# jjery2243542/semi-supervised-ASR

Measured on AMD Instinct MI355X. Metric: utterances/sec (train step), higher is better.
Workload: dtype f32 (fp32-equivalent bf16x6 products)

## Files before the change

include/asr_hip.h:

```cpp
#ifndef ASR_HIP_H
#define ASR_HIP_H

#include <stdint.h>

#ifdef __cplusplus
extern "C" {
#endif

#define ASR_ABI_VERSION 6

#define ASR_E_ARG    (-1)
#define ASR_E_SHAPE  (-2)
#define ASR_E_ALIGN  (-3)

typedef void* asr_stream_t;

int asr_abi_version(void);

#define ASR_ARITH_F32        0
#define ASR_ARITH_BF16X6     1
#define ASR_ARITH_BF16X3     2
#define ASR_ARITH_MASK       0xff
#define ASR_GEMM_TILE_NARROW 0x100
#define ASR_GEMM_TILE_WIDE   0x200
#define ASR_GEMM_TILE_SP     0x800
#define ASR_GEMM_TILE_SMALL  0x1000
#define ASR_GEMM_C_ZEROED    0x2000
#define ASR_LSTM_BWD_GATHER  0x400
#define ASR_DEBUG_FAULT      0x10000

void* asr_graphs_create(int max_entries);
void asr_graphs_destroy(void* graphs);
int asr_graphs_stats(void* graphs, int64_t* hits, int64_t* captures, int64_t* eager);

int asr_gemm_f32(int transA, int transB, int64_t M, int64_t N, int64_t K,
                 const float* A, int64_t lda, const float* B, int64_t ldb,
                 float* C, int64_t ldc, const float* bias, int relu, int accumulate,
                 int batch, int64_t sA, int64_t sB, int64_t sC, int split_k, int arith,
                 asr_stream_t stream);
int asr_gemm_drop_f32(int transA, int transB, int64_t M, int64_t N, int64_t K, const float* A, int64_t lda,
                      const float* B, int64_t ldb, float* C, int64_t ldc, const float* bias, int relu, int split_k,
                      int arith, uint64_t seed, float p, asr_stream_t stream);

int asr_gemm_side_f32(int transA, int transB, int64_t M, int64_t N, int64_t K, const float* A, int64_t lda,
                      const float* B, int64_t ldb, float* C, int64_t ldc, int batch, int64_t sA, int64_t sB, int64_t sC,
                      int arith, unsigned xcd_mask, unsigned* queue, asr_stream_t stream);

int asr_gemm_skinny_f32(int64_t M, int64_t N, int64_t K,
                        const float* A, int64_t lda, const float* Bt, int64_t ldb,
                        float* C, int64_t ldc, const float* bias, int accumulate,
                        const float* mask, int64_t ldmask, int64_t mask_from,
                        asr_stream_t stream);

int asr_colsum_f32(int64_t M, int64_t N, const float* X, int64_t ldx, float* out,
                   int accumulate, asr_stream_t stream);

int asr_lstm_seq_fwd(int T, int B, int nb, int H, int ndir, float* gates, const float* w_hh,
                     const int32_t* lens, const int32_t* rowbase, const int32_t* rowext, float* y, float* c,
                     void* graphs, asr_stream_t stream);

int asr_persist_scratch_bytes(int64_t* xch_bytes, int64_t* ctrl_bytes);
int asr_lstm_seq_fwd_persist(int T, int B, int nb, int H, int ndir, float* gates, const float* w_hh,
                             const int32_t* lens, const int32_t* rowbase, const int32_t* rowext,
                             const int32_t* lens_host, float* y, float* c, void* xch, void* ctrl, int arith,
                             asr_stream_t stream);

int asr_lstm_seq_bwd(int T, int B, int nb, int H, int ndir, float* gates, const float* w_hhT,
                     const int32_t* lens, const int32_t* rowbase, const int32_t* rowext, const float* dy, const float* c,
                     float* dcarry, void* graphs, asr_stream_t stream);
int asr_lstm_seq_bwd_persist(int T, int B, int nb, int H, int ndir, float* gates, const float* w_hhT,
                             const int32_t* lens, const int32_t* rowbase, const int32_t* rowext,
                             const int32_t* lens_host, const float* dy, const float* c, const float* y,
                             float* dw_hh, float* db, void* xch, void* ctrl, int arith, asr_stream_t stream);
int asr_lstm_bwd_persist_fuses_dw(int H, int arith);
int asr_lstm_seq_bwd_persist_w(int T, int B, int nb, int H, int ndir, float* gates, const float* w_hh_il,
                               const int32_t* lens, const int32_t* rowbase, const int32_t* rowext,
                               const int32_t* lens_host, const float* dy, const float* c, const float* y, float* dw_hh,
                               float* db, void* xch, void* ctrl, int arith, asr_stream_t stream);

int asr_rows_pack_f32(int B, int T, int C, const float* x, const int32_t* lens, const int32_t* rowbase,
                      const int32_t* rowext, int ext_max, float* rows, asr_stream_t stream);
int asr_rows_unpack_fwd_f32(int B, int T, int C, const float* rows, const int32_t* lens, const int32_t* rowbase,
                            const float* fill, int fill_relu, const float* mask, uint64_t seed, float p, float* out,
                            asr_stream_t stream);
int asr_rows_unpack_bwd_f32(int B, int T, int C, const float* dout, const int32_t* lens, const int32_t* rowbase,
                            const int32_t* rowext, int ext_max, const float* mask, uint64_t seed, float p, float* drows,
                            float* dfill, const float* relu_of, asr_stream_t stream);

int asr_pyramid_concat_fwd(int T, int B, int C, const float* in, const float* mask,
                           float* out, asr_stream_t stream);
int asr_pyramid_concat_bwd(int T, int B, int C, const float* dout, const float* mask,
                           float* din, asr_stream_t stream);

int asr_dropout_seeded_f32(int64_t n, float* x, uint64_t seed, float p, asr_stream_t stream);
int asr_relu_dropout_bwd_f32(int64_t n, const float* grad, const float* y, uint64_t seed, float p, float* out,
                             asr_stream_t stream);
int asr_dropout_mask_f32(int64_t n, float* mask, uint64_t seed, float p, asr_stream_t stream);
int asr_pyramid_concat_fwd_seeded(int T, int B, int C, const float* in, uint64_t seed, float p, float* out,
                                  asr_stream_t stream);
int asr_pyramid_concat_bwd_seeded(int T, int B, int C, const float* dout, uint64_t seed, float p, float* din,
                                  asr_stream_t stream);

typedef struct {
  int B, nb, Tp, A, D, O, E, C, K;
  int L;
  float scaling;
  const float* P;
  const float* Q;
  const float* bo;
  const float* wcat;
  const float* bcat;
  const float* wdec;
  const float* convw;
  const float* watt;
  const float* wattT;
  const float* gvec;
  const float* w0;
  const float* xmask;
  float* X;
  float* Xd;
  float* gates;
  float* cstate;
  float* Dproj;
  float* fconv;
  float* S;
  float* energy;
  float* ws;
} asr_dec_fwd_t;

int asr_dec_step_fwd(const asr_dec_fwd_t* p, int s, asr_stream_t stream);
int asr_att_step_fwd(const asr_dec_fwd_t* p, int s, asr_stream_t stream);
int asr_dec_seq_fwd(const asr_dec_fwd_t* p, int s_begin, int s_end, void* graphs, asr_stream_t stream);
int asr_dec_seq_fwd_persist(const asr_dec_fwd_t* p, void* xch, void* ctrl, asr_stream_t stream);
int asr_dec_seq_fwd_persist_fault(const asr_dec_fwd_t* p, void* xch, void* ctrl, asr_stream_t stream);
typedef struct {
  int mode;
  int V;
  int eos;
  float scaling;
  const float* w_out;
  const float* b_out;
  const float* emb;
  float* logits;
  float* probs;
  int64_t* pred;
  int64_t* fed;
  const int64_t* tokens;
  int64_t ld_tokens;
  const unsigned char* teacher;
} asr_dec_feedback_t;
int asr_dec_seq_fwd_persist_free(const asr_dec_fwd_t* p, const asr_dec_feedback_t* f, void* xch, void* ctrl,
                                 asr_stream_t stream);

typedef struct {
  asr_dec_fwd_t f;
  const float* wcatT;
  const float* wdecT;
  const float* dws;
  float* G;
  float* dwext;
  float* dwraw;
  float* dfpart;
  float* dP;
  float* dgates;
  float* dD;
  float* dcell;
  float* dgvec_part;
  float* dwatt_part;
  float* dconv_part;
} asr_dec_bwd_t;

int asr_dec_step_bwd(const asr_dec_bwd_t* p, int s, asr_stream_t stream);
int asr_dec_seq_bwd(const asr_dec_bwd_t* p, int s_begin, int s_end, void* graphs, asr_stream_t stream);
int asr_dec_seq_bwd_persist(const asr_dec_bwd_t* p, float* mbuf, void* xch, void* ctrl, asr_stream_t stream);

typedef struct {
  int V;
  float scaling;
  const float* w_out;
  const float* emb;
  const float* probs;
  float* dlfb;
} asr_dec_feedback_bwd_t;
int asr_dec_seq_bwd_persist_free(const asr_dec_bwd_t* p, const asr_dec_feedback_bwd_t* fb, float* mbuf, void* xch,
                                 void* ctrl, asr_stream_t stream);

#define ASR_PACK_MAX_LAYERS 4
typedef struct {
  int H, I, ndir;
  const float* w_ih[2];
  const float* w_hh[2];
  const float* b_ih[2];
  const float* b_hh[2];
  float* w_ih_cat;
  float* w_hh_il;
  float* bias;
} asr_lstm_pack_job_t;
typedef struct {
  int H, I, ndir;
// ... 117 lines not shown
```

semi-supervised-asr_amd/csrc/gemm.hip:

```cpp
#include <cstdlib>
#include <type_traits>
#include "common.h"

#ifndef ASR_GEMM_BF3_TOUCH
#define ASR_GEMM_BF3_TOUCH 2
#endif
#ifndef ASR_GB_ABL
#define ASR_GB_ABL 0
#endif
#ifndef ASR_GLDS_CLOBBER_M0
#define ASR_GLDS_CLOBBER_M0 0
#endif
#ifndef ASR_GEMM_SETPRIO
#define ASR_GEMM_SETPRIO 1
#endif
namespace {

constexpr int BM = 128, BN = 128, BK = 32;
#ifndef ASR_GEMM_SMALL_OCC
#define ASR_GEMM_SMALL_OCC 1
#endif
#ifndef ASR_GEMM_TOUCH
#define ASR_GEMM_TOUCH 2
#endif

struct MatView {
  const float* p;
  int64_t ld, R, Cn;
  bool vec;
};

__device__ __forceinline__ float4 load4_guard(const MatView& m, int64_t r, int64_t c) {
  float4 v = make_float4(0.f, 0.f, 0.f, 0.f);
  if (r >= m.R) return v;
  const float* q = m.p + r * m.ld + c;
  if (m.vec && c + 3 < m.Cn) return *reinterpret_cast<const float4*>(q);
  if (c < m.Cn) v.x = q[0];
  if (c + 1 < m.Cn) v.y = q[1];
  if (c + 2 < m.Cn) v.z = q[2];
  if (c + 3 < m.Cn) v.w = q[3];
  return v;
}

template <bool KC>
struct TileCfg {
  static constexpr int S = KC ? 129 : 128;
};

template <bool KC>
__device__ __forceinline__ void tile_fetch(const MatView& m, int64_t row0, int64_t k0, float4 (&v)[4]) {
  const int t = threadIdx.x;
#pragma unroll
  for (int i = 0; i < 4; ++i) {
    const int f = t + 256 * i;
    if (KC) {
      const int row = f >> 3, kc4 = f & 7;
      v[i] = load4_guard(m, row0 + row, k0 + 4 * kc4);
    } else {
      const int k = f >> 5, m4 = f & 31;
      v[i] = load4_guard(m, k0 + k, row0 + 4 * m4);
    }
  }
}

template <bool KC>
__device__ __forceinline__ void tile_store(float* lds, const float4 (&v)[4]) {
  constexpr int S = TileCfg<KC>::S;
  const int t = threadIdx.x;
#pragma unroll
  for (int i = 0; i < 4; ++i) {
    const int f = t + 256 * i;
    if (KC) {
      const int row = f >> 3, kc4 = f & 7;
      float* d = lds + (4 * kc4) * S + row;
      d[0] = v[i].x; d[S] = v[i].y; d[2 * S] = v[i].z; d[3 * S] = v[i].w;
    } else {
      const int k = f >> 5, m4 = f & 31;
      *reinterpret_cast<float4*>(lds + k * S + 4 * m4) = v[i];
    }
  }
}

struct GemmArgs {
  MatView A, B;
  float* C;
  int64_t ldc, M, N, K;
  const float* bias;
  int relu, accumulate, split_k;
  int64_t sA, sB, sC;
  int tiles_m, tiles_n;
  unsigned* queue;
  unsigned xcd_mask;
};


#ifndef ASR_GEMM_GM
#define ASR_GEMM_GM 4
#endif
__device__ __forceinline__ void tile_coords(int tid, int tiles_m, int tiles_n, int gm_, int& tm, int& tn) {
  const int per = gm_ * tiles_n;
  const int grp = tid / per, in = tid - grp * per;
  const int first = grp * gm_;
  const int rows = tiles_m - first < gm_ ? tiles_m - first : gm_;
  tm = first + in % rows;
  tn = in / rows;
}

template <bool AKC, bool BKC>
__global__ __launch_bounds__(256) void gemm_f32_kernel(GemmArgs g) {
  constexpr int SA = TileCfg<AKC>::S, SB = TileCfg<BKC>::S;
  __shared__ __attribute__((aligned(16))) float smem[BK * SA + BK * SB];
  float* As = smem;
  float* Bs = smem + BK * SA;

  const int ntile = g.tiles_m * g.tiles_n;
  int tid = blockIdx.x;
  {
    const int q = ntile >> 3, rmd = ntile & 7, xcd = tid & 7, idx = tid >> 3;
    tid = (xcd < rmd ? xcd * (q + 1) : rmd * (q + 1) + (xcd - rmd) * q) + idx;
  }
  const int tm = tid / g.tiles_n, tn = tid % g.tiles_n;
  const int z = blockIdx.y;
  const int bz = z / g.split_k, kz = z % g.split_k;

  MatView A = g.A, B = g.B;
  A.p += bz * g.sA;
  B.p += bz * g.sB;
  float* C = g.C + bz * g.sC;

  const int64_t m0 = (int64_t)tm * BM, n0 = (int64_t)tn * BN;
  const int64_t ktiles = (g.K + BK - 1) / BK;
  const int64_t per = (ktiles + g.split_k - 1) / g.split_k;
  const int64_t kt_begin = kz * per;
  const int64_t kt_end = kt_begin + per < ktiles ? kt_begin + per : ktiles;

  const int lane = threadIdx.x & 63, wave = threadIdx.x >> 6;
  const int wm = wave >> 1, wn = wave & 1;
  const int l31 = lane & 31, kh = lane >> 5;

  f32x16 acc[2][2];
#pragma unroll
  for (int i = 0; i < 2; ++i)
#pragma unroll
    for (int j = 0; j < 2; ++j)
#pragma unroll
      for (int e = 0; e < 16; ++e) acc[i][j][e] = 0.f;

  const bool fast_a = A.vec && (AKC ? (m0 + BM <= A.R) : (m0 + BM <= A.Cn)) && A.R * A.ld < (int64_t)1 << 30;
  const bool fast_b = B.vec && (BKC ? (n0 + BN <= B.R) : (n0 + BN <= B.Cn)) && B.R * B.ld < (int64_t)1 << 30;
  const bool fast = fast_a && fast_b;
  unsigned offa[4], offb[4];
#pragma unroll
  for (int i = 0; i < 4; ++i) {
    const int f = threadIdx.x + 256 * i;
    offa[i] = AKC ? (unsigned)((f >> 3) * A.ld + 4 * (f & 7)) : (unsigned)((f >> 5) * A.ld + 4 * (f & 31));
    offb[i] = BKC ? (unsigned)((f >> 3) * B.ld + 4 * (f & 7)) : (unsigned)((f >> 5) * B.ld + 4 * (f & 31));
  }
  const float* basea = AKC ? A.p + m0 * A.ld : A.p + m0;
  const float* baseb = BKC ? B.p + n0 * B.ld : B.p + n0;
  float4 ra[4], rb[4];
  auto fetch = [&](int64_t kt2) {
    const int64_t k0 = kt2 * BK;
    if (fast && k0 + BK <= g.K) {
      const float* pa = basea + (AKC ? k0 : k0 * A.ld);
      const float* pb = baseb + (BKC ? k0 : k0 * B.ld);
#pragma unroll
      for (int i = 0; i < 4; ++i) ra[i] = *reinterpret_cast<const float4*>(pa + offa[i]);
#pragma unroll
      for (int i = 0; i < 4; ++i) rb[i] = *reinterpret_cast<const float4*>(pb + offb[i]);
    } else {
      tile_fetch<AKC>(A, m0, k0, ra);
      tile_fetch<BKC>(B, n0, k0, rb);
    }
  };
  if (kt_begin < kt_end) fetch(kt_begin);
  const int tt = threadIdx.x & 127;
  const bool touch_a = threadIdx.x < 128;
  float touched = 0.f;
  const bool do_touch = kt_end - kt_begin > 16;
  auto touch_tile = [&](int64_t ktt) {
    const MatView& m = touch_a ? A : B;
    const bool kc = touch_a ? AKC : BKC;
    const int64_t r0t = touch_a ? m0 : n0;
    int64_t rr, cc;
    if (kc) { rr = r0t + tt; cc = ktt * BK; }
    else { rr = ktt * BK + (tt >> 2); cc = r0t + 32 * (tt & 3); }
    rr = rr < m.R ? rr : m.R - 1;
    cc = cc < m.Cn ? cc : m.Cn - 1;
    touched = m.p[rr * m.ld + cc];
  };
  for (int64_t kt = kt_begin; kt < kt_end; ++kt) {
    tile_store<AKC>(As, ra);
    tile_store<BKC>(Bs, rb);
    __syncthreads();
    if (kt + 1 < kt_end) fetch(kt + 1);
#if ASR_GEMM_TOUCH
    asm volatile("" ::"v"(touched));
    if (do_touch && kt + ASR_GEMM_TOUCH < kt_end) touch_tile(kt + ASR_GEMM_TOUCH);
#endif
    const float* ap = As + kh * SA + wm * 64 + l31;
    const float* bp = Bs + kh * SB + wn * 64 + l31;
    if (ASR_GEMM_SETPRIO && !AKC) __builtin_amdgcn_s_setprio(1);
#pragma unroll
    for (int kk = 0; kk < BK / 2; ++kk) {
      const float a0 = ap[(2 * kk) * SA], a1 = ap[(2 * kk) * SA + 32];
      const float b0 = bp[(2 * kk) * SB], b1 = bp[(2 * kk) * SB + 32];
      acc[0][0] = __builtin_amdgcn_mfma_f32_32x32x2f32(a0, b0, acc[0][0], 0, 0, 0);
      acc[0][1] = __builtin_amdgcn_mfma_f32_32x32x2f32(a0, b1, acc[0][1], 0, 0, 0);
      acc[1][0] = __builtin_amdgcn_mfma_f32_32x32x2f32(a1, b0, acc[1][0], 0, 0, 0);
      acc[1][1] = __builtin_amdgcn_mfma_f32_32x32x2f32(a1, b1, acc[1][1], 0, 0, 0);
    }
    if (ASR_GEMM_SETPRIO && !AKC) __builtin_amdgcn_s_setprio(0);
    __syncthreads();
  }

  if (m0 + BM <= g.M && n0 + BN <= g.N) {
    const unsigned ldc = (unsigned)g.ldc;
    const bool split = g.split_k > 1, accum = g.accumulate != 0, relu = g.relu != 0;
#pragma unroll
    for (int j = 0; j < 2; ++j) {
      const int64_t n = n0 + wn * 64 + j * 32 + l31;
      const float bv = g.bias ? g.bias[n] : 0.f;
#pragma unroll
      for (int i = 0; i < 2; ++i) {
        float* base = C + (m0 + wm * 64 + i * 32 + 4 * kh) * g.ldc + n;
        if (split) {
#pragma unroll
          for (int e = 0; e < 16; ++e) atomicAdd(base + (unsigned)((e & 3) + 8 * (e >> 2)) * ldc, acc[i][j][e]);
        } else if (accum) {
          float old[16];
#pragma unroll
          for (int e = 0; e < 16; ++e) old[e] = base[(unsigned)((e & 3) + 8 * (e >> 2)) * ldc];
#pragma unroll
          for (int e = 0; e < 16; ++e) {
            float v = acc[i][j][e] + bv + old[e];
            if (relu) v = fmaxf(v, 0.f);
            base[(unsigned)((e & 3) + 8 * (e >> 2)) * ldc] = v;
          }
        } else {
#pragma unroll
          for (int e = 0; e < 16; ++e) {
            float v = acc[i][j][e] + bv;
            if (relu) v = fmaxf(v, 0.f);
            base[(unsigned)((e & 3) + 8 * (e >> 2)) * ldc] = v;
          }
        }
      }
    }
    return;
  }
#pragma unroll
  for (int j = 0; j < 2; ++j) {
    const int64_t n = n0 + wn * 64 + j * 32 + l31;
    if (n >= g.N) continue;
    const float bv = g.bias ? g.bias[n] : 0.f;
#pragma unroll
    for (int i = 0; i < 2; ++i) {
#pragma unroll
      for (int e = 0; e < 16; ++e) {
        const int64_t m = m0 + wm * 64 + i * 32 + (e & 3) + 8 * (e >> 2) + 4 * kh;
        if (m >= g.M) continue;
        float v = acc[i][j][e];
        float* dst = C + m * g.ldc + n;
        if (g.split_k > 1) {
          atomicAdd(dst, v);
        } else {
          v += bv;
          if (g.accumulate) v += *dst;
          if (g.relu) v = fmaxf(v, 0.f);
          *dst = v;
        }
      }
    }
  }
}

typedef __bf16 gbf16x8 __attribute__((ext_vector_type(8)));
typedef __bf16 gbf16x2 __attribute__((ext_vector_type(2)));
typedef unsigned gu32x4 __attribute__((ext_vector_type(4)));
constexpr int BS = 40;

__device__ __forceinline__ unsigned bf3g_hi2(float a, float b) {
  return __builtin_amdgcn_perm(__float_as_uint(b), __float_as_uint(a), 0x07060302u);
}
__device__ __forceinline__ unsigned bf3g_lo2(float a, float b) {
  const float la = a - __uint_as_float(__float_as_uint(a) & 0xffff0000u);
  const float lb = b - __uint_as_float(__float_as_uint(b) & 0xffff0000u);
  const gbf16x2 p = {(__bf16)la, (__bf16)lb};
  return __builtin_bit_cast(unsigned, p);
}

template <int NT>
__device__ __forceinline__ void bfn_split2(float x, float y, unsigned (&t)[NT]) {
  if constexpr (NT == 2) {
    t[0] = bf3g_hi2(x, y);
    t[1] = bf3g_lo2(x, y);
  } else {
    const gbf16x2 pa = {(__bf16)x, (__bf16)y};
    const unsigned ua = __builtin_bit_cast(unsigned, pa);
    const float rx = x - __uint_as_float(ua << 16), ry = y - __uint_as_float(ua & 0xffff0000u);
    const gbf16x2 pb = {(__bf16)rx, (__bf16)ry};
    const unsigned ub = __builtin_bit_cast(unsigned, pb);
    const float sx = rx - __uint_as_float(ub << 16), sy = ry - __uint_as_float(ub & 0xffff0000u);
    t[0] = ua;
    t[1] = ub;
    t[2] = bf3g_hi2(sx, sy);
  }
}

template <bool KC, int TS>
__device__ __forceinline__ void tile_fetch_bf3(const MatView& m, int64_t row0, int64_t k0, float4 (&v)[TS / 32]) {
  const int t = threadIdx.x;
#pragma unroll
  for (int i = 0; i < TS / 32; ++i) {
    if (KC) {
      const int f = t + 256 * i;
      v[i] = load4_guard(m, row0 + (f >> 3), k0 + 4 * (f & 7));
    } else if (TS == 128) {
      v[i] = load4_guard(m, k0 + 4 * (t & 7) + i, row0 + 4 * (t >> 3));
    } else {
      v[i] = load4_guard(m, k0 + 4 * (t & 7) + 2 * (t >> 7) + i, row0 + 4 * ((t >> 3) & 15));
    }
  }
}

template <bool KC, int NT, int TS>
__device__ __forceinline__ void tile_store_bf3(unsigned short* img, const float4 (&v)[TS / 32]) {
  const int t = threadIdx.x;
  if (KC) {
#pragma unroll
    for (int i = 0; i < TS / 32; ++i) {
      const int f = t + 256 * i;
      const int o = (f >> 3) * BS + 4 * (f & 7);
      unsigned p0[NT], p1[NT];
      bfn_split2<NT>(v[i].x, v[i].y, p0);
      bfn_split2<NT>(v[i].z, v[i].w, p1);
#pragma unroll
      for (int k = 0; k < NT; ++k) *reinterpret_cast<uint2*>(img + k * TS * BS + o) = make_uint2(p0[k], p1[k]);
    }
  } else if constexpr (TS == 64) {
    const int o = 4 * ((t >> 3) & 15) * BS + 4 * (t & 7) + 2 * (t >> 7);
    const float r[4][2] = {{v[0].x, v[1].x}, {v[0].y, v[1].y}, {v[0].z, v[1].z}, {v[0].w, v[1].w}};
#pragma unroll
    for (int j = 0; j < 4; ++j) {
      unsigned p0[NT];
      bfn_split2<NT>(r[j][0], r[j][1], p0);
#pragma unroll
      for (int k = 0; k < NT; ++k) *reinterpret_cast<unsigned*>(img + k * TS * BS + o + j * BS) = p0[k];
    }
  } else {
    const int o = 4 * (t >> 3) * BS + 4 * (t & 7);
    const float r[4][4] = {{v[0].x, v[1].x, v[2].x, v[3].x}, {v[0].y, v[1].y, v[2].y, v[3].y},
                           {v[0].z, v[1].z, v[2].z, v[3].z}, {v[0].w, v[1].w, v[2].w, v[3].w}};
#pragma unroll
    for (int j = 0; j < 4; ++j) {
      unsigned p0[NT], p1[NT];
      bfn_split2<NT>(r[j][0], r[j][1], p0);
      bfn_split2<NT>(r[j][2], r[j][3], p1);
#pragma unroll
      for (int k = 0; k < NT; ++k) *reinterpret_cast<uint2*>(img + k * TS * BS + o + j * BS) = make_uint2(p0[k], p1[k]);
    }
  }
}

template <bool AKC, bool BKC, int NT, int TS = 128, bool QUEUE = false>
__global__ __launch_bounds__(256, QUEUE ? 4 : (TS == 64 ? ASR_GEMM_SMALL_OCC : 1)) void gemm_bf3_kernel(GemmArgs g) {
  static_assert(!QUEUE || TS == 64, "the queue instantiation is the 64 x 64 tile");
  constexpr int BM = TS, BN = TS, NP = TS / 32, NB = TS / 64;
  __shared__ __attribute__((aligned(16))) unsigned short smem[2 * NT * BM * BS];
  unsigned short* Ai = smem;
  unsigned short* Bi = smem + NT * BM * BS;

  const int ntile = g.tiles_m * g.tiles_n;
  int tid = blockIdx.x;
  int z = blockIdx.y;
  if constexpr (QUEUE) {
    const unsigned xcc = __builtin_amdgcn_s_getreg(20 | (0 << 6) | (3 << 11)) & 7u;
    if (!((g.xcd_mask >> xcc) & 1u)) return;
    __shared__ unsigned ticket;
    if (threadIdx.x == 0) ticket = atomicAdd(g.queue, 1u);
    __syncthreads();
    const unsigned tk = ticket;
    if (tk >= (unsigned)ntile * gridDim.y) return;
    tid = (int)(tk % (unsigned)ntile);
    z = (int)(tk / (unsigned)ntile);
  } else {
    const int q = ntile >> 3, rmd = ntile & 7, xcd = tid & 7, idx = tid >> 3;
    tid = (xcd < rmd ? xcd * (q + 1) : rmd * (q + 1) + (xcd - rmd) * q) + idx;
  }
  const int tm = tid / g.tiles_n, tn = tid % g.tiles_n;
  const int bz = z / g.split_k, kz = z % g.split_k;

  MatView A = g.A, B = g.B;
  A.p += bz * g.sA;
  B.p += bz * g.sB;
  float* C = g.C + bz * g.sC;

  const int64_t m0 = (int64_t)tm * BM, n0 = (int64_t)tn * BN;
  const int64_t ktiles = (g.K + BK - 1) / BK;
  const int64_t per = (ktiles + g.split_k - 1) / g.split_k;
  const int64_t kt_begin = kz * per;
  const int64_t kt_end = kt_begin + per < ktiles ? kt_begin + per : ktiles;

  const int lane = threadIdx.x & 63, wave = threadIdx.x >> 6;
  const int wm = wave >> 1, wn = wave & 1;
  const int l31 = lane & 31, kh = lane >> 5;

  f32x16 acc[NB][NB];
#pragma unroll
  for (int i = 0; i < NB; ++i)
#pragma unroll
    for (int j = 0; j < NB; ++j)
#pragma unroll
      for (int e = 0; e < 16; ++e) acc[i][j][e] = 0.f;

  const bool fast_a = A.vec && (AKC ? (m0 + BM <= A.R) : (m0 + BM <= A.Cn)) && A.R * A.ld < (int64_t)1 << 30;
  const bool fast_b = B.vec && (BKC ? (n0 + BN <= B.R) : (n0 + BN <= B.Cn)) && B.R * B.ld < (int64_t)1 << 30;
  const bool fast = fast_a && fast_b;
  unsigned offa[NP], offb[NP];
#pragma unroll
  for (int i = 0; i < NP; ++i) {
    const int f = threadIdx.x + 256 * i;
    const int t = threadIdx.x;
    const int krow = TS == 128 ? 4 * (t & 7) + i : 4 * (t & 7) + 2 * (t >> 7) + i, rq = TS == 128 ? (t >> 3) : ((t >> 3) & 15);
    offa[i] = AKC ? (unsigned)((f >> 3) * A.ld + 4 * (f & 7)) : (unsigned)(krow * A.ld + 4 * rq);
    offb[i] = BKC ? (unsigned)((f >> 3) * B.ld + 4 * (f & 7)) : (unsigned)(krow * B.ld + 4 * rq);
  }
  const float* basea = AKC ? A.p + m0 * A.ld : A.p + m0;
  const float* baseb = BKC ? B.p + n0 * B.ld : B.p + n0;
  float4 ra[NP], rb[NP];
  auto fetch_fast = [&](int64_t kt2) {
    const int64_t k0 = kt2 * BK;
    const float* pa = basea + (AKC ? k0 : k0 * A.ld);
    const float* pb = baseb + (BKC ? k0 : k0 * B.ld);
#pragma unroll
    for (int i = 0; i < NP; ++i) ra[i] = *reinterpret_cast<const float4*>(pa + offa[i]);
#pragma unroll
    for (int i = 0; i < NP; ++i) rb[i] = *reinterpret_cast<const float4*>(pb + offb[i]);
  };
  auto fetch_guard = [&](int64_t kt2) {
    const int64_t k0 = kt2 * BK;
    tile_fetch_bf3<AKC, TS>(A, m0, k0, ra);
    tile_fetch_bf3<BKC, TS>(B, n0, k0, rb);
  };
  const int tt = threadIdx.x & 127;
  const bool touch_a = threadIdx.x < 128;
  float touched = 0.f;
  const bool do_touch = TS == 128 && kt_end - kt_begin > 2 * ASR_GEMM_BF3_TOUCH;
  auto touch_tile = [&](int64_t ktt) {
    const MatView& m = touch_a ? A : B;
    const bool kc = touch_a ? AKC : BKC;
    const int64_t r0t = touch_a ? m0 : n0;
    int64_t rr, cc;
    if (kc) { rr = r0t + tt; cc = ktt * BK; }
    else { rr = ktt * BK + (tt >> 2); cc = r0t + 32 * (tt & 3); }
    rr = rr < m.R ? rr : m.R - 1;
    cc = cc < m.Cn ? cc : m.Cn - 1;
    touched = m.p[rr * m.ld + cc];
  };
  const int ao = (wm * (TS / 2) + l31) * BS + 8 * kh, bo = (wn * (TS / 2) + l31) * BS + 8 * kh;
  auto multiply = [&]() {
#pragma unroll
    for (int ks = 0; ks < ((ASR_GB_ABL & 1) ? 0 : BK / 16); ++ks) {
      gu32x4 af[NB][NT], bf[NB][NT];
#pragma unroll
      for (int i = 0; i < NB; ++i)
#pragma unroll
        for (int k = 0; k < NT; ++k) {
          af[i][k] = *reinterpret_cast<const gu32x4*>(Ai + k * BM * BS + ao + 32 * i * BS + 16 * ks);
          bf[i][k] = *reinterpret_cast<const gu32x4*>(Bi + k * BM * BS + bo + 32 * i * BS + 16 * ks);
        }
#define BF3G(a_, b_, c_) c_ = __builtin_amdgcn_mfma_f32_32x32x16_bf16(__builtin_bit_cast(gbf16x8, a_), __builtin_bit_cast(gbf16x8, b_), c_, 0, 0, 0)
#pragma unroll
      for (int o = 0; o < NT; ++o)
#pragma unroll
        for (int p = 0; p <= o; ++p)
#pragma unroll
          for (int i = 0; i < NB; ++i)
#pragma unroll
            for (int j = 0; j < NB; ++j) BF3G(af[i][p], bf[j][o - p], acc[i][j]);
#undef BF3G
    }
  };
  const int64_t kt_full = g.K / BK < kt_end ? g.K / BK : kt_end;
  const int64_t kt_fast_end = (fast && kt_full > kt_begin) ? kt_full : kt_begin;
  if constexpr (TS == 64) {
    constexpr int PD = QUEUE ? 1 : 3;
    float4 qa[PD][NP], qb[PD][NP];
    auto fetch_set = [&](int64_t kt2, float4 (&xa)[NP], float4 (&xb)[NP]) __attribute__((always_inline)) {
      const int64_t k0 = kt2 * BK;
      const float* pa = basea + (AKC ? k0 : k0 * A.ld);
      const float* pb = baseb + (BKC ? k0 : k0 * B.ld);
#pragma unroll
      for (int i = 0; i < NP; ++i) xa[i] = *reinterpret_cast<const float4*>(pa + offa[i]);
#pragma unroll
      for (int i = 0; i < NP; ++i) xb[i] = *reinterpret_cast<const float4*>(pb + offb[i]);
    };
    int64_t kt = kt_begin;
    if (kt < kt_fast_end) {
#pragma unroll
      for (int d = 0; d < PD; ++d)
        if (kt + d < kt_fast_end) fetch_set(kt + d, qa[d], qb[d]);
      for (; kt + 2 * PD <= kt_fast_end; kt += PD) {
#pragma unroll
        for (int d = 0; d < PD; ++d) {
          __builtin_amdgcn_sched_barrier(0);
          tile_store_bf3<AKC, NT, TS>(Ai, qa[d]);
          tile_store_bf3<BKC, NT, TS>(Bi, qb[d]);
          __syncthreads();
          fetch_set(kt + d + PD, qa[d], qb[d]);
          multiply();
          __syncthreads();
          __builtin_amdgcn_sched_barrier(0);
        }
      }
#pragma unroll
      for (int d = 0; d < 2 * PD - 1; ++d) {
        if (kt + d < kt_fast_end) {
          tile_store_bf3<AKC, NT, TS>(Ai, qa[d % PD]);
          tile_store_bf3<BKC, NT, TS>(Bi, qb[d % PD]);
          __syncthreads();
          if (kt + d + PD < kt_fast_end) fetch_set(kt + d + PD, qa[d % PD], qb[d % PD]);
          multiply();
          __syncthreads();
        }
      }
    }
  } else if (kt_begin < kt_fast_end) {
    fetch_fast(kt_begin);
    for (int64_t kt = kt_begin; kt < kt_fast_end; ++kt) {
#if ASR_GB_ABL & 4
      if (kt == kt_begin) {
        tile_store_bf3<AKC, NT, TS>(Ai, ra);
        tile_store_bf3<BKC, NT, TS>(Bi, rb);
      } else {
#pragma unroll
        for (int i = 0; i < NP; ++i) asm volatile("" ::"v"(ra[i].x), "v"(ra[i].y), "v"(ra[i].z), "v"(ra[i].w), "v"(rb[i].x), "v"(rb[i].y), "v"(rb[i].z), "v"(rb[i].w));
      }
#else
      tile_store_bf3<AKC, NT, TS>(Ai, ra);
      tile_store_bf3<BKC, NT, TS>(Bi, rb);
#endif
      __syncthreads();
      if (kt + 1 < kt_fast_end && !(ASR_GB_ABL & 2)) fetch_fast(kt + 1);
#if ASR_GEMM_TOUCH
      asm volatile("" ::"v"(touched));
      if (do_touch && kt + ASR_GEMM_BF3_TOUCH < kt_end) touch_tile(kt + ASR_GEMM_BF3_TOUCH);
#endif
      multiply();
      __syncthreads();
    }
  }
  if (kt_fast_end < kt_end) {
    fetch_guard(kt_fast_end);
    for (int64_t kt = kt_fast_end; kt < kt_end; ++kt) {
      tile_store_bf3<AKC, NT, TS>(Ai, ra);
      tile_store_bf3<BKC, NT, TS>(Bi, rb);
      __syncthreads();
      if (kt + 1 < kt_end) fetch_guard(kt + 1);
#if ASR_GEMM_TOUCH
      asm volatile("" ::"v"(touched));
      if (do_touch && kt + ASR_GEMM_BF3_TOUCH < kt_end) touch_tile(kt + ASR_GEMM_BF3_TOUCH);
#endif
      multiply();
      __syncthreads();
    }
  }

#if ASR_GB_ABL & 8
  if (threadIdx.x + blockIdx.x + blockIdx.y != 0 || g.M != 1) {
#pragma unroll
    for (int i = 0; i < NB; ++i)
#pragma unroll
      for (int j = 0; j < NB; ++j)
#pragma unroll
        for (int e = 0; e < 16; ++e) asm volatile("" ::"v"(acc[i][j][e]));
    return;
  }
#endif
  if (m0 + BM <= g.M && n0 + BN <= g.N) {
    const unsigned ldc = (unsigned)g.ldc;
    const bool split = QUEUE || g.split_k > 1, accum = g.accumulate != 0, relu = g.relu != 0;
#pragma unroll
    for (int j = 0; j < NB; ++j) {
      const int64_t n = n0 + wn * (TS / 2) + j * 32 + l31;
      const float bv = g.bias ? g.bias[n] : 0.f;
#pragma unroll
      for (int i = 0; i < NB; ++i) {
        float* base = C + (m0 + wm * (TS / 2) + i * 32 + 4 * kh) * g.ldc + n;
        if (split) {
#pragma unroll
          for (int e = 0; e < 16; ++e) atomicAdd(base + (unsigned)((e & 3) + 8 * (e >> 2)) * ldc, acc[i][j][e]);
        } else if (accum) {
          float old[16];
#pragma unroll
          for (int e = 0; e < 16; ++e) old[e] = base[(unsigned)((e & 3) + 8 * (e >> 2)) * ldc];
#pragma unroll
          for (int e = 0; e < 16; ++e) {
            float v = acc[i][j][e] + bv + old[e];
            if (relu) v = fmaxf(v, 0.f);
            base[(unsigned)((e & 3) + 8 * (e >> 2)) * ldc] = v;
          }
        } else {
#pragma unroll
          for (int e = 0; e < 16; ++e) {
            float v = acc[i][j][e] + bv;
            if (relu) v = fmaxf(v, 0.f);
            base[(unsigned)((e & 3) + 8 * (e >> 2)) * ldc] = v;
          }
        }
      }
    }
    return;
  }
#pragma unroll
  for (int j = 0; j < NB; ++j) {
    const int64_t n = n0 + wn * (TS / 2) + j * 32 + l31;
    if (n >= g.N) continue;
    const float bv = g.bias ? g.bias[n] : 0.f;
#pragma unroll
    for (int i = 0; i < NB; ++i) {
#pragma unroll
      for (int e = 0; e < 16; ++e) {
        const int64_t m = m0 + wm * (TS / 2) + i * 32 + (e & 3) + 8 * (e >> 2) + 4 * kh;
        if (m >= g.M) continue;
        float v = acc[i][j][e];
        float* dst = C + m * g.ldc + n;
        if (QUEUE || g.split_k > 1) {
          atomicAdd(dst, v);
        } else {
          v += bv;
          if (g.accumulate) v += *dst;
          if (g.relu) v = fmaxf(v, 0.f);
          *dst = v;
        }
      }
    }
  }
}

constexpr int WM = 256, WN = 128, WK = 32;
constexpr int W_A_FLOATS = WM * WK, W_B_FLOATS = WN * WK, W_STAGE_FLOATS = W_A_FLOATS + W_B_FLOATS, W_STAGES = 3;
typedef __attribute__((address_space(3))) void* lds_vptr;

__device__ __forceinline__ void glds16(const float* src, float* lds_dst) {
  const unsigned dst = (unsigned)(uintptr_t)(lds_vptr)lds_dst;
#if ASR_GLDS_CLOBBER_M0
  asm volatile("s_mov_b32 m0, %1\n\ts_nop 0\n\tglobal_load_lds_dwordx4 %0, off" ::"v"(src), "s"(dst) : "memory", "m0");
#else
  unsigned keep;
  asm volatile("s_mov_b32 %0, m0\n\ts_mov_b32 m0, %2\n\ts_nop 0\n\tglobal_load_lds_dwordx4 %1, off\n\ts_mov_b32 m0, %0"
               : "=&s"(keep) : "v"(src), "s"(dst) : "memory");
#endif
}

#ifndef ASR_GW_ABL
#define ASR_GW_ABL 0
#endif
__device__ __forceinline__ void bf3w_split(const float (&v)[8], gu32x4& hi, gu32x4& lo) {
#if ASR_GW_ABL & 2
#pragma unroll
  for (int p = 0; p < 4; ++p) { hi[p] = __float_as_uint(v[p]); lo[p] = __float_as_uint(v[4 + p]); }
  return;
#endif
#pragma unroll
  for (int p = 0; p < 4; ++p) {
    hi[p] = bf3g_hi2(v[2 * p], v[2 * p + 1]);
    lo[p] = bf3g_lo2(v[2 * p], v[2 * p + 1]);
  }
}

template <bool KC, int ROWS>
__device__ __forceinline__ void bf3w_frag(const float* st, int row, int kq0s, int kq1s, int k0, gu32x4& hi, gu32x4& lo) {
  float v[8];
  if (KC) {
    const float4 x = *reinterpret_cast<const float4*>(st + row * WK + kq0s);
    const float4 y = *reinterpret_cast<const float4*>(st + row * WK + kq1s);
    v[0] = x.x; v[1] = x.y; v[2] = x.z; v[3] = x.w; v[4] = y.x; v[5] = y.y; v[6] = y.z; v[7] = y.w;
  } else {
#pragma unroll
    for (int e = 0; e < 8; ++e) v[e] = st[(k0 + e) * ROWS + row];
  }
  bf3w_split(v, hi, lo);
}

template <int I0>
__device__ __forceinline__ void bf3w_send(float* xs, const f32x16 (&acc)[4][2], int lane) {
#pragma unroll
  for (int b = 0; b < 2; ++b)
#pragma unroll
    for (int j = 0; j < 2; ++j)
#pragma unroll
      for (int e = 0; e < 16; ++e) xs[((b * 2 + j) * 16 + e) * 64 + lane] = acc[I0 + b][j][e];
}

template <int I0, bool EDGE>
__device__ __forceinline__ void bf3w_finish(const float* xr, f32x16 (&acc)[4][2], const GemmArgs& g, float* C, int64_t mrow0,
                                            int64_t ncol0, int lane) {
  const int l31 = lane & 31, kh = lane >> 5;
  const unsigned ldc = (unsigned)g.ldc;
  const bool split = g.split_k > 1, accum = g.accumulate != 0, relu = g.relu != 0;
#pragma unroll
  for (int b = 0; b < 2; ++b)
#pragma unroll
    for (int j = 0; j < 2; ++j) {
      const int64_t n = ncol0 + j * 32 + l31;
      const int64_t mb = mrow0 + (I0 + b) * 32 + 4 * kh;
      const bool nok = !EDGE || n < g.N;
      const float bv = (g.bias && nok) ? g.bias[n] : 0.f;
      float* base = C + mb * g.ldc + n;
      float v[16];
#pragma unroll
      for (int e = 0; e < 16; ++e) v[e] = acc[I0 + b][j][e] + xr[((b * 2 + j) * 16 + e) * 64 + lane];
#pragma unroll
      for (int e = 0; e < 16; ++e) {
        const int r = (e & 3) + 8 * (e >> 2);
        if (EDGE && !(nok && mb + r < g.M)) continue;
        float* dst = base + (unsigned)r * ldc;
        if (split) {
          atomicAdd(dst, v[e]);
        } else {
          float o = v[e] + bv;
          if (accum) o += *dst;
          if (relu) o = fmaxf(o, 0.f);
          *dst = o;
        }
      }
    }
}

#ifdef ASR_GW_TRACE
__device__ unsigned long long asr_gw_trace_buf[2 * 64 * 8];
#define GW_MARK(m) do { if (blockIdx.x == 0 && blockIdx.y == 0 && lane == 0 && (wave & 3) == 0 && st < 63) \
    asr_gw_trace_buf[((wave >> 2) * 64 + st) * 8 + (m)] = clock64(); } while (0)
#define GW_COARSE(m) do { if (blockIdx.x == 0 && blockIdx.y == 0 && threadIdx.x == 0) asr_gw_trace_buf[63 * 8 + (m)] = clock64(); } while (0)
#else
#define GW_MARK(m) do {} while (0)
#define GW_COARSE(m) do {} while (0)
#endif

template <bool AKC, bool BKC>
__global__ __launch_bounds__(512) void gemm_bf3w_kernel(GemmArgs g) {
  __shared__ __attribute__((aligned(1024))) float smem[W_STAGES * W_STAGE_FLOATS];

  const int ntile = g.tiles_m * g.tiles_n;
  int tid = blockIdx.x;
  {
    const int q = ntile >> 3, rmd = ntile & 7, xcd = tid & 7, idx = tid >> 3;
    tid = (xcd < rmd ? xcd * (q + 1) : rmd * (q + 1) + (xcd - rmd) * q) + idx;
  }
  const int tm = tid / g.tiles_n, tn = tid % g.tiles_n;
  const int z = blockIdx.y;
  const int bz = z / g.split_k, kz = z % g.split_k;
  const float* Ap = g.A.p + bz * g.sA;
  const float* Bp = g.B.p + bz * g.sB;
  float* C = g.C + bz * g.sC;
  const int64_t m0 = (int64_t)tm * WM, n0 = (int64_t)tn * WN;
  const int64_t ktiles = g.K / WK;
  const int64_t per = (ktiles + g.split_k - 1) / g.split_k;
  const int64_t kt_begin = kz * per;
  const int64_t kt_end = kt_begin + per < ktiles ? kt_begin + per : ktiles;
  const int S = (int)(kt_end - kt_begin);
  if (S <= 0) return;

  const int lane = threadIdx.x & 63;
  const int wave = __builtin_amdgcn_readfirstlane(threadIdx.x >> 6);
  const int kg = wave >> 2, wm = (wave >> 1) & 1, wn = wave & 1;
  const int l31 = lane & 31, kh = lane >> 5;

  const int64_t lda = g.A.ld, ldb = g.B.ld;
  unsigned offa[4], offb[2];
#pragma unroll
  for (int q = 0; q < 4; ++q) {
    const int p = 4 * wave + q;
    if (AKC) {
      const int r = 8 * p + (lane >> 3);
      const int64_t row = m0 + r < g.M ? m0 + r : g.M - 1;
      offa[q] = (unsigned)(row * lda + 4 * ((lane & 7) ^ ((r >> 1) & 7)));
    } else {
      const int64_t col = m0 + 4 * lane + 4 <= g.M ? m0 + 4 * lane : g.M - 4;
      offa[q] = (unsigned)(p * lda + col);
    }
  }
#pragma unroll
  for (int q = 0; q < 2; ++q) {
    const int p = 2 * wave + q;
    if (BKC) {
      const int r = 8 * p + (lane >> 3);
      const int64_t row = n0 + r < g.N ? n0 + r : g.N - 1;
      offb[q] = (unsigned)(row * ldb + 4 * ((lane & 7) ^ ((r >> 1) & 7)));
    } else {
// ... 885 lines not shown
#define X_LDA0(u_) load_a(I0(), std::integral_constant<int, u_>(), grp)
  BFK_FOR_PIECES(X_LDA0);
#undef X_LDA0
  barrier();
  {
    const unsigned bbase = lds0 + BUFB + (wn * 32 + l31) * ROWB + 16 * kh;
#pragma unroll
    for (int ks = 0; ks < KS; ++ks) {
      const unsigned a = bbase + 32 * ks;
      FB[ks][0] = *lds_at<lds_q4ptr>(a);
      FB[ks][1] = *lds_at<lds_q4ptr>(a + PLANE);
      if constexpr (NT > 2) FB[ks][2] = *lds_at<lds_q4ptr>(a + 2 * PLANE);
    }
  }
#define X_UNA0(u_) unit(I0(), std::integral_constant<int, u_>(), I0())
  BFK_FOR_PIECES(X_UNA0);
#undef X_UNA0
  if (ntile > 1) {
#define X_LDA1(u_) load_a(I1(), std::integral_constant<int, u_>(), grp + groups)
    BFK_FOR_PIECES(X_LDA1);
#undef X_LDA1
  }
  barrier();
  read_fa(I0(), I0(), I0());
#pragma unroll
  for (int p = 0; p < 2; ++p)
#pragma unroll
    for (int i = 0; i < 2; ++i)
#pragma unroll
      for (int e = 0; e < 16; ++e) acc[p][i][e] = 0.f;

  auto mtile = [&](int k, auto ptag) __attribute__((always_inline)) {
    constexpr int P = decltype(ptag)::value;
    typedef std::integral_constant<int, P> PT;
    typedef std::integral_constant<int, 1 - P> PN;
    const int mt = grp + k * groups;
    const bool has_prev = k > 0, has_next = k + 1 < ntile, has_next2 = k + 2 < ntile;
    if (has_next2 && !(ASR_GK_ABL & 2)) {
#define X_LDA2(u_) load_a(PT(), std::integral_constant<int, u_>(), mt + 2 * groups)
      BFK_FOR_PIECES(X_LDA2);
#undef X_LDA2
    }
#define BFK_UNIT(u_) { unit(PN(), std::integral_constant<int, u_>(), PN()); }
#define BFK_STEP(ks_)                                                                                                   \
    {                                                                                                                   \
      typedef std::integral_constant<int, ((ks_) + P * KS) & 1> SL;       \
      typedef std::integral_constant<int, ((ks_) + 1 + P * KS) & 1> SN;                                                 \
      if ((ks_) == KS - 1 && has_next) barrier();                                                                       \
      products(SL(), std::integral_constant<int, ks_>(), PT());                                                         \
      if ((ks_) + 1 < KS) read_fa(SN(), std::integral_constant<int, ((ks_) + 1 < KS ? (ks_) + 1 : 0)>(), PT());        \
      else if (has_next) read_fa(SN(), I0(), PN());                                                                     \
      if constexpr ((ks_) < KS - 1) {                   \
        if (has_next && !(ASR_GK_ABL & 2)) {                                                                            \
          constexpr int u0 = (ks_) * HP / (KS - 1), u1 = ((ks_) + 1) * HP / (KS - 1);                                   \
          if constexpr (u0 < u1) BFK_UNIT(u0)                                                                           \
          if constexpr (u0 + 1 < u1) BFK_UNIT(u0 + 1)                                                                   \
          if constexpr (u0 + 2 < u1) BFK_UNIT(u0 + 2)                                                                   \
        }                                                                                                               \
      }                                                                                                                 \
      if constexpr ((ks_) < 4) {                                                                                        \
        if (has_prev) store_half(PN(), std::integral_constant<int, ((ks_) / 2)>(), std::integral_constant<int, (ks_) & 1>(), mt - groups); \
      }                                                                                                                 \
      __builtin_amdgcn_sched_barrier(0);                                                                                \
    }
    BFK_STEP(0) BFK_STEP(1) BFK_STEP(2) BFK_STEP(3)
    if constexpr (KS > 4) BFK_STEP(4)
    if constexpr (KS > 5) BFK_STEP(5)
#undef BFK_STEP
#undef BFK_UNIT
  };
  int k = 0;
  for (; k + 1 < ntile; k += 2) {
    mtile(k, I0());
    mtile(k + 1, I1());
  }
  if (k < ntile) mtile(k, I0());
  {
    const int klast = ntile - 1, mt = grp + klast * groups;
    if (klast & 1) {
      store_half(I1(), I0(), I0(), mt); store_half(I1(), I0(), I1(), mt); store_half(I1(), I1(), I0(), mt); store_half(I1(), I1(), I1(), mt);
    } else {
      store_half(I0(), I0(), I0(), mt); store_half(I0(), I0(), I1(), mt); store_half(I0(), I1(), I0(), mt); store_half(I0(), I1(), I1(), mt);
    }
  }
#undef BFK_FOR_PIECES
}

struct DropEpi {
  unsigned long long seed;
  unsigned thresh;
  float scale;
};
__global__ void bias_act_kernel(float* C, int64_t ldc, int64_t M, int64_t N, int64_t sC, const float* __restrict__ bias,
                                int relu, DropEpi drop) {
  float* p = C + blockIdx.z * sC;
  for (int64_t i = blockIdx.x * (int64_t)blockDim.x + threadIdx.x; i < M * N; i += (int64_t)gridDim.x * blockDim.x) {
    const int64_t m = i / N, n = i % N;
    float v = p[m * ldc + n] + (bias ? bias[n] : 0.f);
    if (relu) v = fmaxf(v, 0.f);
    if (drop.thresh) v = asr_drop_keep(drop.seed, i, drop.thresh) ? v * drop.scale : 0.f;
    p[m * ldc + n] = v;
  }
}

__global__ void zero_rows_kernel(float* C, int64_t ldc, int64_t M, int64_t N, int64_t sC) {
  float* p = C + blockIdx.z * sC;
  for (int64_t i = blockIdx.x * (int64_t)blockDim.x + threadIdx.x; i < M * N; i += (int64_t)gridDim.x * blockDim.x) {
    const int64_t m = i / N, n = i % N;
    p[m * ldc + n] = 0.f;
  }
}

template <int MT>
__global__ __launch_bounds__(256) void skinny_kernel(int64_t M, int64_t N, int K, const float* A, int64_t lda,
                                                     const float* Bt, int64_t ldb, float* C, int64_t ldc,
                                                     const float* bias, int accumulate, const float* mask,
                                                     int64_t ldmask, int64_t mask_from, int ksplit) {
  __shared__ float red[4 * MT * 16 * SK_LDS_STRIDE];
  const int64_t n0 = (int64_t)blockIdx.x * 16;
  const int64_t row0 = (int64_t)blockIdx.y * (MT * 16);
  const int kper = K / ksplit;
  A += (int64_t)blockIdx.z * kper;
  Bt += (int64_t)blockIdx.z * kper;
  K = kper;
  constexpr int NE = MT;
  float bv[NE], mv[NE], cv[NE];
#pragma unroll
  for (int i = 0; i < NE; ++i) {
    const int e = threadIdx.x + 256 * i;
    const int row = e >> 4, col = e & 15;
    const int64_t m = row0 + row, n = n0 + col;
    const bool ok = m < M && n < N;
    const int64_t mc = ok ? m : 0, nc = ok ? n : 0;
    bv[i] = bias ? bias[nc] : 0.f;
    mv[i] = (mask && nc >= mask_from) ? mask[mc * ldmask + (nc - mask_from)] : 1.f;
    cv[i] = (accumulate && ksplit == 1) ? C[mc * ldc + nc] : 0.f;
  }
  skinny_partial<MT>(A, lda, row0, M, Bt, ldb, n0, N, K, red);
  __syncthreads();
#pragma unroll
  for (int i = 0; i < NE; ++i) {
    const int e = threadIdx.x + 256 * i;
    const int row = e >> 4, col = e & 15;
    const int64_t m = row0 + row, n = n0 + col;
    if (m >= M || n >= N) continue;
    const float v = (skinny_reduced<MT>(red, row, col) + bv[i]) * mv[i];
    if (ksplit > 1) atomicAdd(C + m * ldc + n, v);
    else C[m * ldc + n] = v + cv[i];
  }
}

__global__ void colsum_kernel(int64_t M, int64_t N, const float* X, int64_t ldx, float* out) {
  __shared__ float part[4][64];
  const int cx = threadIdx.x & 63, ry = threadIdx.x >> 6;
  const int64_t n = (int64_t)blockIdx.x * 64 + cx;
  const int64_t mbeg = (int64_t)blockIdx.y * 512;
  const int64_t mend = mbeg + 512 < M ? mbeg + 512 : M;
  float s = 0.f;
  if (n < N)
    for (int64_t m = mbeg + ry; m < mend; m += 4) s += X[m * ldx + n];
  part[ry][cx] = s;
  __syncthreads();
  if (ry == 0 && n < N) atomicAdd(out + n, (part[0][cx] + part[1][cx]) + (part[2][cx] + part[3][cx]));
}

__global__ __launch_bounds__(256) void colsum4_kernel(int64_t M, int64_t N, const float* __restrict__ X, int64_t ldx,
                                                      float* out) {
  __shared__ float4 part[16][16];
  const int cq = threadIdx.x & 15, ry = threadIdx.x >> 4;
  const int64_t n = (int64_t)blockIdx.x * 64 + 4 * cq;
  const int64_t mbeg = (int64_t)blockIdx.y * 256;
  const int64_t mend = mbeg + 256 < M ? mbeg + 256 : M;
  float4 s = make_float4(0.f, 0.f, 0.f, 0.f);
  if (n < N) {
    const float* p = X + n;
#pragma unroll 4
    for (int64_t m = mbeg + ry; m < mend; m += 16) {
      const float4 v = *reinterpret_cast<const float4*>(p + m * ldx);
      s.x += v.x; s.y += v.y; s.z += v.z; s.w += v.w;
    }
  }
  part[ry][cq] = s;
  __syncthreads();
  if (threadIdx.x < 64) {
    const int q = threadIdx.x >> 2, e = threadIdx.x & 3;
    float t = 0.f;
#pragma unroll
    for (int r = 0; r < 16; ++r) t += reinterpret_cast<const float*>(&part[r][q])[e];
    const int64_t col = (int64_t)blockIdx.x * 64 + threadIdx.x;
    if (col < N) atomicAdd(out + col, t);
  }
}

}

extern "C" int asr_abi_version(void) { return ASR_ABI_VERSION; }

#ifdef ASR_GW_TRACE
extern "C" int asr_gw_trace_read(void* dst) {
  return (int)hipMemcpyFromSymbol(dst, HIP_SYMBOL(asr_gw_trace_buf), sizeof(unsigned long long) * 2 * 64 * 8);
}
#endif

static int narrow_split_k(int64_t M, int64_t N, int64_t K, int batch, bool epilogue, int ts = 128) {
  const int64_t tiles = ((M + ts - 1) / ts) * ((N + ts - 1) / ts) * batch;
  const int64_t target = 512;
  if (tiles >= target || K < 512) return 1;
  int64_t sk = tiles <= 32 ? 16 : 8;
  if (target / tiles < sk) sk = target / tiles;
  if (K / 256 < sk) sk = K / 256;
  if (sk < 1) sk = 1;
  if (epilogue && sk > 1 && tiles > 64 && K < 2048) return 1;
  return (int)sk;
}

template <int NT, int TS = 128>
static void launch_narrow_split(bool akc, bool bkc, dim3 grid, hipStream_t stream, const GemmArgs& g) {
  const dim3 block(256);
  if (akc && bkc) hipLaunchKernelGGL((gemm_bf3_kernel<true, true, NT, TS>), grid, block, 0, stream, g);
  else if (akc && !bkc) hipLaunchKernelGGL((gemm_bf3_kernel<true, false, NT, TS>), grid, block, 0, stream, g);
  else if (!akc && bkc) hipLaunchKernelGGL((gemm_bf3_kernel<false, true, NT, TS>), grid, block, 0, stream, g);
  else hipLaunchKernelGGL((gemm_bf3_kernel<false, false, NT, TS>), grid, block, 0, stream, g);
}

static int gemm_impl(int transA, int transB, int64_t M, int64_t N, int64_t K, const float* A, int64_t lda,
                     const float* B, int64_t ldb, float* C, int64_t ldc, const float* bias, int relu,
                     int accumulate, int batch, int64_t sA, int64_t sB, int64_t sC, int split_k, int arith,
                     DropEpi drop, hipStream_t stream) {
  if (!A || !B || !C || M <= 0 || N <= 0 || K <= 0 || batch <= 0) return ASR_E_ARG;
  if (drop.thresh && (batch != 1 || accumulate)) return ASR_E_ARG;
  const DropEpi no_drop = {0ull, 0u, 1.f};
  auto pass_behind = [&](bool late) {
    if (!late && !drop.thresh) return;
    dim3 eg((unsigned)((M * N + 255) / 256 > 2048 ? 2048 : (M * N + 255) / 256), 1, batch);
    hipLaunchKernelGGL(bias_act_kernel, eg, dim3(256), 0, stream, C, ldc, M, N, sC, late ? bias : nullptr, late ? relu : 0,
                       drop.thresh ? drop : no_drop);
  };
  const int ar = arith & ASR_ARITH_MASK;
  if (ar != ASR_ARITH_F32 && ar != ASR_ARITH_BF16X6 && ar != ASR_ARITH_BF16X3) return ASR_E_ARG;
  const bool auto_split = split_k <= 0;
  GemmArgs g;
  const bool akc = !transA, bkc = transB != 0;
  g.A.p = A; g.A.ld = lda;
  if (akc) { g.A.R = M; g.A.Cn = K; } else { g.A.R = K; g.A.Cn = M; }
  g.A.vec = (lda % 4 == 0) && asr_aligned16(A) && (sA % 4 == 0);
  g.B.p = B; g.B.ld = ldb;
  if (bkc) { g.B.R = N; g.B.Cn = K; } else { g.B.R = K; g.B.Cn = N; }
  g.B.vec = (ldb % 4 == 0) && asr_aligned16(B) && (sB % 4 == 0);
  g.C = C; g.ldc = ldc; g.M = M; g.N = N; g.K = K;
  g.accumulate = accumulate;
  g.sA = sA; g.sB = sB; g.sC = sC;
  g.queue = nullptr; g.xcd_mask = 0xffu;
  const bool epi = bias || relu;
  const bool base_shape = g.A.vec && g.B.vec && (akc ? M : K) * lda < ((int64_t)1 << 31) &&
                          (bkc ? N : K) * ldb < ((int64_t)1 << 31) && (akc || (M % 4 == 0 && M >= 4)) &&
                          (bkc || (N % 4 == 0 && N >= 4)) && M >= 64 && N >= 64;
  const bool wide_shape = K % WK == 0 && base_shape;
  const int64_t wtiles = ((M + WM - 1) / WM) * ((N + WN - 1) / WN) * batch;
  const bool may_split = auto_split && !(epi && accumulate);
  const bool wide_pays = (!akc && !bkc && K >= 1024) || (K >= 2048 && ((may_split && !epi) || wtiles >= 150));
  if (ar != ASR_ARITH_F32 && akc && bkc && K == 80 && g.A.vec && g.B.vec && M * lda < ((int64_t)1 << 29) && N * ldb < ((int64_t)1 << 29) &&
      M >= 1024 && N >= 128 && (auto_split || split_k == 1) && !(arith & (ASR_GEMM_TILE_NARROW | ASR_GEMM_TILE_WIDE | ASR_GEMM_TILE_SP | ASR_GEMM_TILE_SMALL))) {
    const int tiles_n = (int)((N + 127) / 128);
    if (tiles_n <= 256) {
      const int groups = 8 * (tiles_n >= 32 ? 1 : 32 / tiles_n);
      g.bias = bias; g.relu = relu; g.split_k = 1;
      dim3 grid(tiles_n * groups, batch, 1), b4(512);
      const bool plain = M % 128 == 0 && N % 128 == 0 && !relu && !accumulate && M * ldc < ((int64_t)1 << 29);
      if (ar == ASR_ARITH_BF16X6) {
        if (plain) hipLaunchKernelGGL((gemm_bfk_kernel<3, 5, true>), grid, b4, 0, stream, g, groups);
        else hipLaunchKernelGGL((gemm_bfk_kernel<3, 5, false>), grid, b4, 0, stream, g, groups);
      } else {
        if (plain) hipLaunchKernelGGL((gemm_bfk_kernel<2, 5, true>), grid, b4, 0, stream, g, groups);
        else hipLaunchKernelGGL((gemm_bfk_kernel<2, 5, false>), grid, b4, 0, stream, g, groups);
      }
      pass_behind(false);
      ASR_CHECK_LAUNCH();
      return 0;
    }
  }
  static const int64_t small_max = [] { const char* f = getenv("ASR_GEMM_SMALL_MAX"); return f ? (int64_t)atoll(f) : (int64_t)256; }();
  const int64_t tiles128 = ((M + BM - 1) / BM) * ((N + BN - 1) / BN) * batch;
  const int64_t wgs128 = tiles128 * (auto_split ? ((epi && accumulate) ? 1 : narrow_split_k(M, N, K, batch, epi, 128)) : (split_k > 0 ? split_k : 1));
  const bool small = ar != ASR_ARITH_F32 && ((arith & ASR_GEMM_TILE_SMALL) || (wgs128 <= small_max && !(arith & ASR_GEMM_TILE_NARROW)));
  const bool sp_shape = base_shape && (K % WK == 0 || (K % 4 == 0 && K > WK)) &&
                        (akc ? M : K) * lda < ((int64_t)1 << 29) && (bkc ? N : K) * ldb < ((int64_t)1 << 29);
  static const int64_t sp_min_units = [] { const char* f = getenv("ASR_GEMM_SP_MIN"); return f ? (int64_t)atoll(f) : (int64_t)5000; }();
  const bool sp_pays = (K % WK == 0 || K >= 64 * WK) && wtiles * (K / WK) >= sp_min_units;
  const bool use_sp = ar != ASR_ARITH_F32 && sp_shape && (auto_split || split_k == 1) && (!small || (arith & ASR_GEMM_TILE_SP)) &&
                      ((arith & ASR_GEMM_TILE_SP) || (sp_pays && !(arith & (ASR_GEMM_TILE_NARROW | ASR_GEMM_TILE_WIDE | ASR_GEMM_TILE_SMALL))));
  const bool wide = use_sp || (ar != ASR_ARITH_F32 && !(arith & (ASR_GEMM_TILE_NARROW | ASR_GEMM_TILE_SP | ASR_GEMM_TILE_SMALL)) && wide_shape &&
                               ((wide_pays && !small) || (arith & ASR_GEMM_TILE_WIDE)) && (auto_split || split_k == 1));
  if (wide) {
    const int64_t tiles = wtiles, stages = (K + WK - 1) / WK;
    int best = 1;
    if (may_split) {
      double best_cost = 1e30;
      for (int sk = 1; sk <= 16 && stages / sk >= 8; ++sk) {
        const int64_t wgs = tiles * sk, rounds = (wgs + 255) / 256;
        const double out_mb = (double)M * N * batch * 4.0 / 1048576.0;
        const double cost = (double)rounds * ((double)((stages + sk - 1) / sk) + 6.0) +
                            (sk > 1 ? 0.47 * sk * out_mb + (epi ? 3.0 + 0.6 * out_mb : 0.0) : 0.0);
        if (cost < best_cost) { best_cost = cost; best = sk; }
      }
    }
    static const int forced_sk = [] { const char* f = getenv("ASR_GEMM_WIDE_SK"); return f ? atoi(f) : 0; }();
    if (forced_sk >= 1 && forced_sk <= stages && may_split) best = forced_sk;
    const bool late_epi = best > 1 && epi;
    g.bias = late_epi ? nullptr : bias; g.relu = late_epi ? 0 : relu;
    g.split_k = best;
    g.tiles_m = (int)((M + WM - 1) / WM);
    g.tiles_n = (int)((N + WN - 1) / WN);
    if (best > 1 && !accumulate && !(arith & ASR_GEMM_C_ZEROED)) {
      dim3 zg((unsigned)((M * N + 255) / 256 > 2048 ? 2048 : (M * N + 255) / 256), 1, batch);
      hipLaunchKernelGGL(zero_rows_kernel, zg, dim3(256), 0, stream, C, ldc, M, N, sC);
    }
    dim3 grid(g.tiles_m * g.tiles_n, batch * best, 1), block(512);
    if (use_sp) {
      const dim3 b4(256);
#define SP_LAUNCH(nt_, kt_)                                                                                             \
      do {                                                                                                              \
        if (akc && bkc) hipLaunchKernelGGL((gemm_bfs_kernel<true, true, nt_, kt_>), grid, b4, 0, stream, g);            \
        else if (akc && !bkc) hipLaunchKernelGGL((gemm_bfs_kernel<true, false, nt_, kt_>), grid, b4, 0, stream, g);     \
        else if (!akc && bkc) hipLaunchKernelGGL((gemm_bfs_kernel<false, true, nt_, kt_>), grid, b4, 0, stream, g);     \
        else hipLaunchKernelGGL((gemm_bfs_kernel<false, false, nt_, kt_>), grid, b4, 0, stream, g);                     \
      } while (0)
      if (ar == ASR_ARITH_BF16X6) { if (K % WK) SP_LAUNCH(3, true); else SP_LAUNCH(3, false); }
      else { if (K % WK) SP_LAUNCH(2, true); else SP_LAUNCH(2, false); }
#undef SP_LAUNCH
    } else if (ar == ASR_ARITH_BF16X6) {
      if (akc && bkc) hipLaunchKernelGGL((gemm_bf6w_kernel<true, true>), grid, block, 0, stream, g);
      else if (akc && !bkc) hipLaunchKernelGGL((gemm_bf6w_kernel<true, false>), grid, block, 0, stream, g);
      else if (!akc && bkc) hipLaunchKernelGGL((gemm_bf6w_kernel<false, true>), grid, block, 0, stream, g);
      else hipLaunchKernelGGL((gemm_bf6w_kernel<false, false>), grid, block, 0, stream, g);
    } else {
      if (akc && bkc) hipLaunchKernelGGL((gemm_bf3w_kernel<true, true>), grid, block, 0, stream, g);
      else if (akc && !bkc) hipLaunchKernelGGL((gemm_bf3w_kernel<true, false>), grid, block, 0, stream, g);
      else if (!akc && bkc) hipLaunchKernelGGL((gemm_bf3w_kernel<false, true>), grid, block, 0, stream, g);
      else hipLaunchKernelGGL((gemm_bf3w_kernel<false, false>), grid, block, 0, stream, g);
    }
    pass_behind(late_epi);
    ASR_CHECK_LAUNCH();
    return 0;
  }
  const int ts = small ? 64 : 128;
  if (auto_split) split_k = (epi && accumulate) ? 1 : narrow_split_k(M, N, K, batch, epi, ts);
  const bool late_epilogue = split_k > 1 && epi;
  if (late_epilogue && accumulate) return ASR_E_SHAPE;
  g.bias = late_epilogue ? nullptr : bias;
  g.relu = late_epilogue ? 0 : relu;
  g.tiles_m = (int)((M + ts - 1) / ts);
  g.tiles_n = (int)((N + ts - 1) / ts);
  const int64_t ktiles = (K + BK - 1) / BK;
  if (split_k > ktiles) split_k = (int)ktiles;
  g.split_k = split_k;
  if (split_k > 1 && !accumulate && !(arith & ASR_GEMM_C_ZEROED)) {
    dim3 zg((unsigned)((M * N + 255) / 256 > 2048 ? 2048 : (M * N + 255) / 256), 1, batch);
    hipLaunchKernelGGL(zero_rows_kernel, zg, dim3(256), 0, stream, C, ldc, M, N, sC);
  }
  dim3 grid(g.tiles_m * g.tiles_n, batch * split_k, 1), block(256);
  if (ar == ASR_ARITH_BF16X6 && small) launch_narrow_split<3, 64>(akc, bkc, grid, stream, g);
  else if (ar == ASR_ARITH_BF16X3 && small) launch_narrow_split<2, 64>(akc, bkc, grid, stream, g);
  else if (ar == ASR_ARITH_BF16X6) launch_narrow_split<3>(akc, bkc, grid, stream, g);
  else if (ar == ASR_ARITH_BF16X3) launch_narrow_split<2>(akc, bkc, grid, stream, g);
  else if (akc && bkc) hipLaunchKernelGGL((gemm_f32_kernel<true, true>), grid, block, 0, stream, g);
  else if (akc && !bkc) hipLaunchKernelGGL((gemm_f32_kernel<true, false>), grid, block, 0, stream, g);
  else if (!akc && bkc) hipLaunchKernelGGL((gemm_f32_kernel<false, true>), grid, block, 0, stream, g);
  else hipLaunchKernelGGL((gemm_f32_kernel<false, false>), grid, block, 0, stream, g);
  pass_behind(late_epilogue);
  ASR_CHECK_LAUNCH();
  return 0;
}

extern "C" int asr_gemm_f32(int transA, int transB, int64_t M, int64_t N, int64_t K, const float* A, int64_t lda,
                            const float* B, int64_t ldb, float* C, int64_t ldc, const float* bias, int relu,
                            int accumulate, int batch, int64_t sA, int64_t sB, int64_t sC, int split_k, int arith,
                            asr_stream_t stream) {
  const DropEpi none = {0ull, 0u, 1.f};
  return gemm_impl(transA, transB, M, N, K, A, lda, B, ldb, C, ldc, bias, relu, accumulate, batch, sA, sB, sC, split_k, arith,
                   none, (hipStream_t)stream);
}

extern "C" int asr_gemm_drop_f32(int transA, int transB, int64_t M, int64_t N, int64_t K, const float* A, int64_t lda,
                                 const float* B, int64_t ldb, float* C, int64_t ldc, const float* bias, int relu,
                                 int split_k, int arith, uint64_t seed, float p, asr_stream_t stream) {
  if (p < 0.f || p >= 1.f) return ASR_E_ARG;
  const DropEpi d = {(unsigned long long)seed, asr_drop_thresh(p), 1.0f / (1.0f - p)};
  return gemm_impl(transA, transB, M, N, K, A, lda, B, ldb, C, ldc, bias, relu, 0, 1, 0, 0, 0, split_k, arith, d,
                   (hipStream_t)stream);
}

extern "C" int asr_gemm_side_f32(int transA, int transB, int64_t M, int64_t N, int64_t K, const float* A, int64_t lda,
                                 const float* B, int64_t ldb, float* C, int64_t ldc, int batch, int64_t sA, int64_t sB,
                                 int64_t sC, int arith, unsigned xcd_mask, unsigned* queue, asr_stream_t stream_) {
  if (!A || !B || !C || !queue || M <= 0 || N <= 0 || K <= 0 || batch <= 0 || !(xcd_mask & 0xffu)) return ASR_E_ARG;
  const int ar = arith & ASR_ARITH_MASK;
  if (ar != ASR_ARITH_BF16X6 && ar != ASR_ARITH_BF16X3) return ASR_E_SHAPE;
  hipStream_t stream = (hipStream_t)stream_;
  GemmArgs g;
  const bool akc = !transA, bkc = transB != 0;
  g.A.p = A; g.A.ld = lda;
  if (akc) { g.A.R = M; g.A.Cn = K; } else { g.A.R = K; g.A.Cn = M; }
  g.A.vec = (lda % 4 == 0) && asr_aligned16(A) && (sA % 4 == 0);
  g.B.p = B; g.B.ld = ldb;
  if (bkc) { g.B.R = N; g.B.Cn = K; } else { g.B.R = K; g.B.Cn = N; }
  g.B.vec = (ldb % 4 == 0) && asr_aligned16(B) && (sB % 4 == 0);
  g.C = C; g.ldc = ldc; g.M = M; g.N = N; g.K = K;
  g.bias = nullptr; g.relu = 0; g.accumulate = 1;
  g.sA = sA; g.sB = sB; g.sC = sC;
  g.tiles_m = (int)((M + 63) / 64);
  g.tiles_n = (int)((N + 63) / 64);
  g.queue = queue; g.xcd_mask = xcd_mask & 0xffu;
  const int nx = __builtin_popcount(g.xcd_mask);
  const int64_t tiles = (int64_t)g.tiles_m * g.tiles_n * batch, ktiles = (K + BK - 1) / BK;
  int64_t sk = (4 * 32 * nx + tiles - 1) / tiles;
  if (sk > ktiles / 8) sk = ktiles / 8;
  if (sk < 1) sk = 1;
  if (sk > 64) sk = 64;
  g.split_k = (int)sk;
  const int64_t tickets = (int64_t)g.tiles_m * g.tiles_n * batch * sk;
  if (tickets > 0x3fffffff) return ASR_E_SHAPE;
  const unsigned gy = (unsigned)(batch * sk);
  const int64_t per_y = (int64_t)g.tiles_m * g.tiles_n;
  const unsigned gx = (unsigned)((per_y * 8 + nx - 1) / nx + 8);
  auto launch = [&](dim3 grid) {
    const dim3 block(256);
#define SIDE_LAUNCH(nt_)                                                                                                     \
    do {                                                                                                                     \
      if (akc && bkc) hipLaunchKernelGGL((gemm_bf3_kernel<true, true, nt_, 64, true>), grid, block, 0, stream, g);           \
      else if (akc && !bkc) hipLaunchKernelGGL((gemm_bf3_kernel<true, false, nt_, 64, true>), grid, block, 0, stream, g);    \
      else if (!akc && bkc) hipLaunchKernelGGL((gemm_bf3_kernel<false, true, nt_, 64, true>), grid, block, 0, stream, g);    \
      else hipLaunchKernelGGL((gemm_bf3_kernel<false, false, nt_, 64, true>), grid, block, 0, stream, g);                    \
    } while (0)
    if (ar == ASR_ARITH_BF16X6) SIDE_LAUNCH(3); else SIDE_LAUNCH(2);
#undef SIDE_LAUNCH
  };
  launch(dim3(gx, gy, 1));
  g.xcd_mask = 0xffu;
  launch(dim3((unsigned)per_y, gy, 1));
  ASR_CHECK_LAUNCH();
  return 0;
}

int asr_skinny_launch(int64_t M, int64_t N, int64_t K, const float* A, int64_t lda, const float* Bt, int64_t ldb,
                      float* C, int64_t ldc, const float* bias, int accumulate, const float* mask, int64_t ldmask,
                      int64_t mask_from, hipStream_t stream) {
  if (!A || !Bt || !C || M <= 0 || N <= 0 || K <= 0) return ASR_E_ARG;
  if (K % 16 || lda % 4 || ldb % 4) return ASR_E_SHAPE;
  if (!asr_aligned16(A) || !asr_aligned16(Bt)) return ASR_E_ALIGN;
  const unsigned nb = (unsigned)((N + 15) / 16);
  int ksplit = 1;
  if (accumulate && !bias && K >= 1024 && K % 64 == 0) {
    ksplit = (int)(K / 512);
    while ((K / 16) % ksplit) --ksplit;
  }
  if (M <= 32) {
    hipLaunchKernelGGL((skinny_kernel<1>), dim3(nb, (unsigned)((M + 15) / 16), ksplit), dim3(256), 0, stream, M, N,
                       (int)K, A, lda, Bt, ldb, C, ldc, bias, accumulate, mask, ldmask, mask_from, ksplit);
  } else {
    hipLaunchKernelGGL((skinny_kernel<2>), dim3(nb, (unsigned)((M + 31) / 32), ksplit), dim3(256), 0, stream, M, N,
                       (int)K, A, lda, Bt, ldb, C, ldc, bias, accumulate, mask, ldmask, mask_from, ksplit);
  }
  ASR_CHECK_LAUNCH();
  return 0;
}

extern "C" int asr_gemm_skinny_f32(int64_t M, int64_t N, int64_t K, const float* A, int64_t lda, const float* Bt,
                                   int64_t ldb, float* C, int64_t ldc, const float* bias, int accumulate,
                                   const float* mask, int64_t ldmask, int64_t mask_from, asr_stream_t stream) {
  return asr_skinny_launch(M, N, K, A, lda, Bt, ldb, C, ldc, bias, accumulate, mask, ldmask, mask_from,
                           (hipStream_t)stream);
}

extern "C" int asr_colsum_f32(int64_t M, int64_t N, const float* X, int64_t ldx, float* out, int accumulate,
                              asr_stream_t stream) {
  if (!X || !out || M <= 0 || N <= 0) return ASR_E_ARG;
  if (!accumulate) {
    hipError_t e = hipMemsetAsync(out, 0, (size_t)N * sizeof(float), (hipStream_t)stream);
    if (e != hipSuccess) return (int)e;
  }
  if (N % 4 == 0 && ldx % 4 == 0 && asr_aligned16(X))
    hipLaunchKernelGGL(colsum4_kernel, dim3((unsigned)((N + 63) / 64), (unsigned)((M + 255) / 256)), dim3(256), 0,
                       (hipStream_t)stream, M, N, X, ldx, out);
  else
    hipLaunchKernelGGL(colsum_kernel, dim3((unsigned)((N + 63) / 64), (unsigned)((M + 511) / 512)), dim3(256), 0,
                       (hipStream_t)stream, M, N, X, ldx, out);
  ASR_CHECK_LAUNCH();
  return 0;
}
```

semi-supervised-asr_amd/hip_backend.py:

```python
import ctypes
import os

import torch

_HERE = os.path.dirname(os.path.abspath(__file__))
LIB_PATH = os.path.join(_HERE, "lib", "libasr_hip.so")
ABI_VERSION = 6

EXPORTS = (
    "asr_abi_version", "asr_persist_scratch_bytes", "asr_gemm_f32", "asr_gemm_skinny_f32", "asr_colsum_f32",
    "asr_lstm_seq_fwd", "asr_lstm_seq_fwd_persist", "asr_lstm_seq_bwd", "asr_lstm_seq_bwd_persist", "asr_lstm_seq_bwd_persist_w", "asr_lstm_bwd_persist_fuses_dw", "asr_pyramid_concat_fwd", "asr_pyramid_concat_bwd",
    "asr_pyramid_concat_fwd_seeded", "asr_pyramid_concat_bwd_seeded", "asr_rows_pack_f32", "asr_rows_unpack_fwd_f32", "asr_rows_unpack_bwd_f32", "asr_dropout_seeded_f32", "asr_relu_dropout_bwd_f32",
    "asr_dropout_mask_f32",
    "asr_dec_step_fwd", "asr_att_step_fwd", "asr_dec_seq_fwd", "asr_dec_seq_fwd_persist", "asr_dec_seq_fwd_persist_fault", "asr_dec_seq_fwd_persist_free", "asr_dec_step_bwd", "asr_dec_seq_bwd", "asr_dec_seq_bwd_persist", "asr_dec_seq_bwd_persist_free",
    "asr_lstm_pack_f32", "asr_lstm_unpack_f32", "asr_lstm_unpack2_f32", "asr_dec_prepare_f32", "asr_cell_pack_f32", "asr_cell_unpack_f32",
    "asr_lstm_pack_multi_f32", "asr_lstm_unpack_multi_f32", "asr_dec_pack_f32", "asr_colsum_parts_f32", "asr_gemm_drop_f32", "asr_gemm_side_f32", "asr_embedding_grad_f32",
    "asr_label_logprob_fwd", "asr_label_logprob_bwd", "asr_dec_feedback_fwd", "asr_dec_feedback_bwd",
    "asr_adam_clip_f32", "asr_sumsq_f32", "asr_gather_sumsq_f32", "asr_graphs_create", "asr_graphs_destroy", "asr_graphs_stats",
    "asr_beam_select_f32", "asr_beam_reorder_f32", "asr_beam_backtrack",
    "asr_lm_step_f32", "asr_beam_select_lm_f32", "asr_beam_reorder_lm_f32",
    "asr_edit_distance_i32",
)

_lib = None

c_i, c_i64, c_f, c_p = ctypes.c_int, ctypes.c_int64, ctypes.c_float, ctypes.c_void_p


PACK_MAX_LAYERS = 4


class LstmPackJob(ctypes.Structure):
    _fields_ = [("H", c_i), ("I", c_i), ("ndir", c_i), ("w_ih", c_p * 2), ("w_hh", c_p * 2), ("b_ih", c_p * 2),
                ("b_hh", c_p * 2), ("w_ih_cat", c_p), ("w_hh_il", c_p), ("bias", c_p)]


class LstmUnpackJob(ctypes.Structure):
    _fields_ = [("H", c_i), ("I", c_i), ("ndir", c_i), ("dw_ih_cat", c_p), ("dw_hh_il", c_p), ("db_il", c_p),
                ("dw_ih", c_p * 2), ("dw_hh", c_p * 2), ("db", c_p * 2), ("db2", c_p * 2)]


class DecFeedback(ctypes.Structure):
    _fields_ = [("mode", c_i), ("V", c_i), ("eos", c_i), ("scaling", c_f), ("w_out", c_p), ("b_out", c_p), ("emb", c_p), ("logits", c_p),
                ("probs", c_p), ("pred", c_p), ("fed", c_p), ("tokens", c_p), ("ld_tokens", ctypes.c_int64), ("teacher", c_p)]


class DecFeedbackBwd(ctypes.Structure):
    _fields_ = [("V", c_i), ("scaling", c_f), ("w_out", c_p), ("emb", c_p), ("probs", c_p), ("dlfb", c_p)]


_DEC_DIMS = ("B", "nb", "Tp", "A", "D", "O", "E", "C", "K", "L")
_DEC_FWD_PTRS = ("P", "Q", "bo", "wcat", "bcat", "wdec", "convw", "watt", "wattT", "gvec", "w0", "xmask",
                 "X", "Xd", "gates", "cstate", "Dproj", "fconv", "S", "energy", "ws")
_DEC_BWD_PTRS = ("wcatT", "wdecT", "dws", "G", "dwext", "dwraw", "dfpart", "dP", "dgates", "dD",
                 "dcell", "dgvec_part", "dwatt_part", "dconv_part")


class DecFwd(ctypes.Structure):
    _fields_ = [(n, c_i) for n in _DEC_DIMS] + [("scaling", c_f)] + [(n, c_p) for n in _DEC_FWD_PTRS]


class Beam(ctypes.Structure):
    _fields_ = [(n, c_i) for n in ("B", "K", "V", "L", "eos")] + \
               [(n, c_p) for n in ("logits", "scores", "tok_hist", "bp_hist", "fin", "fin_score", "nfin", "done", "ndone")]


class BeamState(ctypes.Structure):
    _fields_ = [(n, c_i) for n in ("D", "O", "E", "Tp")] + [("ldx", ctypes.c_int64)] + \
               [(n, c_p) for n in ("x_src", "x_dst", "c_src", "c_dst", "w_src", "w_dst", "emb")]


BEAM_KMAX, BEAM_FCAP = 16, 48
LM_MAX_LAYERS, LM_MAX_ROWS, LM_MAX_WIDTH = 4, 512, 1024


class BeamLmState(ctypes.Structure):
    _fields_ = [("n_layers", c_i), ("H", c_i), ("in_dim", c_i * LM_MAX_LAYERS)] + \
               [(n, c_p * LM_MAX_LAYERS) for n in ("x_src", "x_dst", "c_src", "c_dst")] + [("emb", c_p)]


class DecBwd(ctypes.Structure):
    _fields_ = [("f", DecFwd)] + [(n, c_p) for n in _DEC_BWD_PTRS]


def _fptr(t, off=0):
    return None if t is None else c_p(t.data_ptr() + 4 * int(off))


class DecBuffers(object):

    _ACC = ("G", "dwext", "dP", "dcell", "dgvec_part", "dwatt_part", "dconv_part")

    def __init__(self, B, Tp, A, D, O, E, C, K, L, drop, dev, with_bwd):
        f32 = dict(device=dev, dtype=torch.float32)
        KX = D + O + E
        self.dims = dict(B=B, Tp=Tp, A=A, D=D, O=O, E=E, C=C, K=K, L=L)
        self.B, self.L, self.KX, self.scaling = B, L, KX, 2.0
        self.bo = self.wdec = self.watt = None
        self.P, self.Q, self.w0 = torch.empty(B, Tp, A, **f32), torch.empty(B, Tp, O, **f32), torch.empty(B, Tp, **f32)
        self.wcat, self.bcat, self.wattT = torch.empty(4 * D, KX, **f32), torch.empty(4 * D, **f32), torch.empty(C, A, **f32)
        self.convw, self.gvec = torch.empty(C, 2 * K + 1, **f32), torch.empty(A, **f32)
        self.X = torch.empty(L + 1, B, KX, **f32)
        self.Xd = torch.empty(L + 1, B, KX, **f32) if drop else None
        self.xmask = torch.empty(L, B, O + E, **f32) if drop else None
        self.gates, self.cstate = torch.empty(L, B, 4 * D, **f32), torch.empty(L, B, D, **f32)
        self.Dproj, self.fconv = torch.empty(L, B, A, **f32), torch.empty(L, B, C, Tp, **f32)
        self.S, self.energy, self.ws = torch.empty(L, B, Tp, A, **f32), torch.empty(L, B, Tp, **f32), torch.empty(L, B, Tp, **f32)
        self._row = dict(P=Tp * A, Q=Tp * O, w0=Tp, xmask=O + E, X=KX, Xd=KX, gates=4 * D, cstate=D, Dproj=A, fconv=C * Tp,
                         S=Tp * A, energy=Tp, ws=Tp, dws=Tp, G=KX, dwext=Tp, dwraw=Tp, dfpart=C * Tp, dP=Tp * A, dgates=4 * D,
                         dD=A, dcell=D, dgvec_part=A, dwatt_part=A * C, dconv_part=C * (2 * K + 1))
        self.zbuf = self.acc = None
        if with_bwd:
            ntile = (A + 63) // 64
            shapes = dict(G=(L + 1, B, KX), dwext=(C, B, Tp), dP=(B, Tp, A), dcell=(B, D), dgvec_part=(B, A),
                          dwatt_part=(B, A, C), dconv_part=(B, C, 2 * K + 1))
            self._acc_layout, off = [], 0
            for name in self._ACC:
                strides = torch.empty(shapes[name], device="meta").stride()
                self._acc_layout.append((name, shapes[name], strides, off))
                off += (strides[0] * shapes[name][0] + 3) // 4 * 4
            self.zbuf = torch.empty(off, **f32)
            self.acc = self.accumulators(self.zbuf)
            self.wcatT, self.wdecT = torch.empty(KX, 4 * D, **f32), torch.empty(D, A, **f32)
            self.dwraw, self.dfpart = torch.empty(B, Tp, **f32), torch.empty(ntile, B, C, Tp, **f32)
            self.dgates, self.dD = torch.empty(L, B, 4 * D, **f32), torch.empty(L, B, A, **f32)
            self.dws, self.Mf = torch.empty(L, B, Tp, **f32), torch.empty(L, B, C, Tp, **f32)
        else:
            self.wcatT = self.wdecT = None

    def bind(self, P=None, Q=None, w0=None, convw=None, gvec=None, bo=None, wdec=None, watt=None, xmask=None, scaling=None):
        given = dict(P=P, Q=Q, w0=w0, bo=bo, wdec=wdec, watt=watt, xmask=xmask,
                     convw=None if convw is None else convw.reshape(self.convw.shape),
                     gvec=None if gvec is None else gvec.reshape(self.gvec.shape))
        for name, t in given.items():
            if t is not None:
                setattr(self, name, t.contiguous())
        if scaling is not None:
            self.scaling = float(scaling)

    def accumulators(self, base):
        first = base.storage_offset()
        return {name: base.as_strided(shape, strides, first + off) for name, shape, strides, off in self._acc_layout}

    def fwd_struct(self, b0=0, nb=None):
        row = self._row
        return DecFwd(nb=self.B if nb is None else nb, scaling=self.scaling,
                      **{n: _fptr(getattr(self, n), b0 * row.get(n, 0)) for n in _DEC_FWD_PTRS}, **self.dims)

    def bwd_struct(self, b0=0, nb=None, acc=None, with_dws=True):
        acc, own, row = self.acc if acc is None else acc, self.__dict__, self._row
        ptrs = {n: _fptr(acc[n] if n in acc else own[n], b0 * row.get(n, 0)) for n in _DEC_BWD_PTRS}
        if not with_dws:
            ptrs["dws"] = None
        return DecBwd(f=self.fwd_struct(b0, nb), **ptrs)


def load():
    global _lib
    if _lib is not None:
        return _lib
    if not os.path.exists(LIB_PATH):
        raise RuntimeError(
            "libasr_hip.so not found at %s — build it with `python -c 'import __graft_entry__ as g; g.build()'` "
            "(hipcc --offload-arch=gfx950). This package has no CPU fallback." % LIB_PATH)
    lib = ctypes.CDLL(LIB_PATH)
    for name in EXPORTS:
        getattr(lib, name).restype = c_i
    lib.asr_graphs_create.restype = c_p
    lib.asr_graphs_create.argtypes = [c_i]
    lib.asr_graphs_destroy.restype = None
    lib.asr_graphs_destroy.argtypes = [c_p]
    lib.asr_graphs_stats.argtypes = [c_p, ctypes.POINTER(c_i64), ctypes.POINTER(c_i64), ctypes.POINTER(c_i64)]
    lib.asr_persist_scratch_bytes.argtypes = [ctypes.POINTER(c_i64), ctypes.POINTER(c_i64)]
    lib.asr_gemm_f32.argtypes = [c_i, c_i, c_i64, c_i64, c_i64, c_p, c_i64, c_p, c_i64, c_p, c_i64, c_p, c_i, c_i,
                                 c_i, c_i64, c_i64, c_i64, c_i, c_i, c_p]
    lib.asr_gemm_skinny_f32.argtypes = [c_i64, c_i64, c_i64, c_p, c_i64, c_p, c_i64, c_p, c_i64, c_p, c_i, c_p,
                                        c_i64, c_i64, c_p]
    lib.asr_colsum_f32.argtypes = [c_i64, c_i64, c_p, c_i64, c_p, c_i, c_p]
    lib.asr_lstm_seq_fwd.argtypes = [c_i, c_i, c_i, c_i, c_i, c_p, c_p, c_p, c_p, c_p, c_p, c_p, c_p, c_p]
    lib.asr_lstm_seq_fwd_persist.argtypes = [c_i, c_i, c_i, c_i, c_i, c_p, c_p, c_p, c_p, c_p, c_p, c_p, c_p, c_p, c_p, c_i, c_p]
    lib.asr_lstm_seq_bwd_persist.argtypes = [c_i, c_i, c_i, c_i, c_i, c_p, c_p, c_p, c_p, c_p, c_p, c_p, c_p, c_p, c_p, c_p, c_p, c_p,
                                             c_i, c_p]
    lib.asr_lstm_seq_bwd_persist_w.argtypes = lib.asr_lstm_seq_bwd_persist.argtypes
    lib.asr_lstm_bwd_persist_fuses_dw.argtypes = [c_i, c_i]
    lib.asr_lstm_seq_bwd.argtypes = [c_i, c_i, c_i, c_i, c_i, c_p, c_p, c_p, c_p, c_p, c_p, c_p, c_p, c_p, c_p]
    lib.asr_rows_pack_f32.argtypes = [c_i, c_i, c_i, c_p, c_p, c_p, c_p, c_i, c_p, c_p]
    lib.asr_rows_unpack_fwd_f32.argtypes = [c_i, c_i, c_i, c_p, c_p, c_p, c_p, c_i, c_p, ctypes.c_uint64, c_f, c_p, c_p]
    lib.asr_rows_unpack_bwd_f32.argtypes = [c_i, c_i, c_i, c_p, c_p, c_p, c_p, c_i, c_p, ctypes.c_uint64, c_f, c_p, c_p, c_p, c_p]
    lib.asr_pyramid_concat_fwd.argtypes = [c_i, c_i, c_i, c_p, c_p, c_p, c_p]
    lib.asr_pyramid_concat_bwd.argtypes = [c_i, c_i, c_i, c_p, c_p, c_p, c_p]
    c_u64 = ctypes.c_uint64
    lib.asr_pyramid_concat_fwd_seeded.argtypes = [c_i, c_i, c_i, c_p, c_u64, c_f, c_p, c_p]
    lib.asr_pyramid_concat_bwd_seeded.argtypes = [c_i, c_i, c_i, c_p, c_u64, c_f, c_p, c_p]
    lib.asr_dropout_seeded_f32.argtypes = [c_i64, c_p, c_u64, c_f, c_p]
    lib.asr_relu_dropout_bwd_f32.argtypes = [c_i64, c_p, c_p, c_u64, c_f, c_p, c_p]
    lib.asr_dropout_mask_f32.argtypes = [c_i64, c_p, c_u64, c_f, c_p]
    lib.asr_dec_step_fwd.argtypes = [ctypes.POINTER(DecFwd), c_i, c_p]
    lib.asr_beam_select_f32.argtypes = [ctypes.POINTER(Beam), c_i, c_p]
    lib.asr_beam_reorder_f32.argtypes = [ctypes.POINTER(Beam), c_i, ctypes.POINTER(BeamState), c_p]
    lib.asr_beam_backtrack.argtypes = [ctypes.POINTER(Beam), c_f, c_p, c_p, c_p, c_p]
    lib.asr_lm_step_f32.argtypes = [c_i, c_i, c_i, c_p, c_i64, c_p, c_p, c_p, c_p, c_p, c_i64, c_p, c_i64, c_p]
    lib.asr_beam_select_lm_f32.argtypes = [ctypes.POINTER(Beam), c_p, c_f, c_i, c_p]
    lib.asr_beam_reorder_lm_f32.argtypes = [ctypes.POINTER(Beam), c_i, ctypes.POINTER(BeamState),
                                            ctypes.POINTER(BeamLmState), c_p]
    lib.asr_edit_distance_i32.argtypes = [c_i, c_p, c_i, c_i64, c_i, c_p, c_p, c_i64, c_p, c_p, c_i, c_p, c_i, c_p, c_p, c_p,
                                          c_p, c_p]
    lib.asr_att_step_fwd.argtypes = [ctypes.POINTER(DecFwd), c_i, c_p]
    lib.asr_dec_seq_fwd.argtypes = [ctypes.POINTER(DecFwd), c_i, c_i, c_p, c_p]
    lib.asr_dec_seq_fwd_persist.argtypes = [ctypes.POINTER(DecFwd), c_p, c_p, c_p]
    lib.asr_dec_seq_fwd_persist_fault.argtypes = lib.asr_dec_seq_fwd_persist.argtypes
    lib.asr_dec_seq_fwd_persist_free.argtypes = [ctypes.POINTER(DecFwd), ctypes.POINTER(DecFeedback), c_p, c_p, c_p]
    lib.asr_dec_step_bwd.argtypes = [ctypes.POINTER(DecBwd), c_i, c_p]
    lib.asr_dec_seq_bwd.argtypes = [ctypes.POINTER(DecBwd), c_i, c_i, c_p, c_p]
    lib.asr_dec_seq_bwd_persist.argtypes = [ctypes.POINTER(DecBwd), c_p, c_p, c_p, c_p]
    lib.asr_dec_seq_bwd_persist_free.argtypes = [ctypes.POINTER(DecBwd), ctypes.POINTER(DecFeedbackBwd), c_p, c_p, c_p, c_p]
    lib.asr_adam_clip_f32.argtypes = [c_i64, c_p, c_p, c_p, c_p, c_p, c_p, c_f, c_f, c_f, c_f, c_f, c_f, c_f, c_f, c_p, c_p, c_p]
    lib.asr_sumsq_f32.argtypes = [c_i64, c_p, c_p, c_p]
    lib.asr_gather_sumsq_f32.argtypes = [c_i, ctypes.POINTER(c_p), ctypes.POINTER(c_i64), ctypes.POINTER(c_i64), c_p, c_p, c_p]
    lib.asr_label_logprob_fwd.argtypes = [c_i64, c_i, c_p, c_i64, c_p, c_p, c_f, c_p, c_p, c_f, c_p, c_p]
    lib.asr_label_logprob_bwd.argtypes = [c_i64, c_i, c_p, c_i64, c_p, c_p, c_f, c_p, c_i64, c_f, c_p, c_i64, c_p]
    lib.asr_dec_feedback_fwd.argtypes = [c_i, c_i, c_i, c_i, c_p, c_i64, c_p, c_p, c_p, c_p, c_p, c_i, c_f, c_p, c_i64,
                                         c_p, c_p, c_p, c_p, c_p, c_i64, c_p]
    lib.asr_dec_feedback_bwd.argtypes = [c_i, c_i, c_i, c_i, c_p, c_p, c_i64, c_p, c_p, c_p, c_f, c_p, c_p]
    pp = ctypes.POINTER(c_p)
    lib.asr_lstm_pack_f32.argtypes = [c_i, c_i, c_i, pp, pp, pp, pp, c_p, c_p, c_p, c_p]
    lib.asr_lstm_unpack_f32.argtypes = [c_i, c_i, c_i, c_p, c_p, c_p, pp, pp, pp, c_p]
    lib.asr_lstm_unpack2_f32.argtypes = [c_i, c_i, c_i, c_p, c_p, c_p, pp, pp, pp, pp, c_p]
    lib.asr_dec_prepare_f32.argtypes = [c_i, c_i, c_i, c_i, c_i, c_p, c_i64, c_p, c_p, c_p, c_p, c_p, c_p]
    lib.asr_cell_pack_f32.argtypes = [c_i, c_i, c_i, c_p, c_p, c_p, c_p, c_p, c_p, c_p]
    lib.asr_cell_unpack_f32.argtypes = [c_i, c_i, c_i, c_p, c_p, c_p, c_p, c_p, c_p, c_p]
    lib.asr_lstm_pack_multi_f32.argtypes = [c_i, ctypes.POINTER(LstmPackJob), c_p]
    lib.asr_lstm_unpack_multi_f32.argtypes = [c_i, ctypes.POINTER(LstmUnpackJob), c_p]
    lib.asr_dec_pack_f32.argtypes = [c_i, c_i, c_i, c_i, c_i] + [c_p] * 12
    lib.asr_colsum_parts_f32.argtypes = [c_i, c_i, pp, ctypes.POINTER(ctypes.c_int32), pp, c_p]
    lib.asr_embedding_grad_f32.argtypes = [c_i64, c_i, c_i, c_p, c_p, c_i64, c_p, c_p]
    lib.asr_gemm_drop_f32.argtypes = [c_i, c_i, c_i64, c_i64, c_i64, c_p, c_i64, c_p, c_i64, c_p, c_i64, c_p, c_i, c_i, c_i,
                                      ctypes.c_uint64, c_f, c_p]
    lib.asr_gemm_side_f32.argtypes = [c_i, c_i, c_i64, c_i64, c_i64, c_p, c_i64, c_p, c_i64, c_p, c_i64, c_i, c_i64, c_i64, c_i64,
                                      c_i, ctypes.c_uint, c_p, c_p]
    if lib.asr_abi_version() != ABI_VERSION:
        raise RuntimeError("libasr_hip.so ABI %d != expected %d" % (lib.asr_abi_version(), ABI_VERSION))
    _lib = lib
    return lib


ARITH_F32, ARITH_BF16X6, ARITH_BF16X3 = 0, 1, 2
GEMM_TILE_NARROW, GEMM_TILE_WIDE, LSTM_BWD_GATHER, GEMM_TILE_SP, GEMM_TILE_SMALL = 0x100, 0x200, 0x400, 0x800, 0x1000
DEBUG_FAULT = 0x10000
DEC_FAULT = [False]
ARITH_NAMES = {"f32": ARITH_F32, "bf16x6": ARITH_BF16X6, "bf16x3": ARITH_BF16X3}
ARITH_LABEL = {ARITH_F32: "f32", ARITH_BF16X6: "bf16x6", ARITH_BF16X3: "bf16x3"}


def _arith_code(a):
    if isinstance(a, str):
        code = 0
        for part in a.lower().split("+"):
            code |= {"narrow": GEMM_TILE_NARROW, "wide": GEMM_TILE_WIDE, "gather": LSTM_BWD_GATHER, "sp": GEMM_TILE_SP,
                     "small": GEMM_TILE_SMALL, "fault": DEBUG_FAULT}.get(part, 0) or \
                    ARITH_NAMES[part]
        return code
    return int(a)


ARITH = [_arith_code(os.environ.get("ASR_ARITH", "bf16x6"))]


def current_arith():
    return ARITH[0]


def arith_name(a=None):
    return ARITH_LABEL[(ARITH[0] if a is None else _arith_code(a)) & 0xff]


class arith(object):

    def __init__(self, a):
        self.code = _arith_code(a)

    def __enter__(self):
        self.old = ARITH[0]
        ARITH[0] = self.code
        return self

    def __exit__(self, *exc):
        ARITH[0] = self.old
        return False


def _dev(t, name="tensor"):
    if not t.is_cuda:
        raise RuntimeError("%s must live on the GPU: the HIP path has no CPU fallback" % name)
    if t.dtype not in (torch.float32, torch.int32):
        raise RuntimeError("%s must be float32/int32, got %s" % (name, t.dtype))
    return t


def ptr(t):
    return None if t is None else c_p(_dev(t).data_ptr())


_raw_stream = getattr(torch._C, "_cuda_getCurrentRawStream", None)
_raw_device = getattr(torch._C, "_cuda_getDevice", None)


def stream():
    if _raw_stream is not None and _raw_device is not None:
        return c_p(_raw_stream(_raw_device()))
    return c_p(torch.cuda.current_stream().cuda_stream)


def check(rc, what):
    if rc != 0:
        raise RuntimeError("%s failed with code %d (negative: ASR_E_*; positive: hipError_t)" % (what, rc))


def _rowmajor(t):
    assert t.dim() == 2 and (t.stride(1) == 1 or t.shape[1] == 1), "need row-major 2-D view"
    return t, (t.stride(0) if t.shape[0] > 1 else max(t.shape[1], 1))


C_ZEROED = 0x2000


def gemm(A, B, trans_a=False, trans_b=False, bias=None, relu=False, out=None, accumulate=False, split_k=None, arith=None,
         drop=None, out_zeroed=False):
    A, lda = _rowmajor(_dev(A, "A"))
    B, ldb = _rowmajor(_dev(B, "B"))
    M, K = (A.shape[1], A.shape[0]) if trans_a else A.shape
    K2, N = (B.shape[1], B.shape[0]) if trans_b else B.shape
    assert K == K2, "inner dimensions differ: %d vs %d" % (K, K2)
    if out is None:
        out = torch.empty(M, N, device=A.device, dtype=torch.float32)
    out, ldc = _rowmajor(out)
    assert out.shape == (M, N)
    code = (ARITH[0] if arith is None else _arith_code(arith)) | (C_ZEROED if out_zeroed else 0)
    if drop is not None:
        assert not accumulate and ldc == N
        check(load().asr_gemm_drop_f32(int(trans_a), int(trans_b), M, N, K, ptr(A), lda, ptr(B), ldb, ptr(out), ldc,
                                       ptr(bias), int(relu), 0 if split_k is None else int(split_k), code, drop.seed,
                                       float(drop.p), stream()), "asr_gemm_drop_f32")
        return out
    check(load().asr_gemm_f32(int(trans_a), int(trans_b), M, N, K, ptr(A), lda, ptr(B), ldb, ptr(out), ldc,
                              ptr(bias), int(relu), int(accumulate), 1, 0, 0, 0, 0 if split_k is None else int(split_k),
                              code, stream()), "asr_gemm_f32")
    return out


def gemm_batched(A, B, out, trans_a, trans_b, M, N, K, lda, ldb, ldc, batch, sA, sB, sC, accumulate=False, arith=None,
                 split_k=None, a_off=0, b_off=0):
    check(load().asr_gemm_f32(int(trans_a), int(trans_b), M, N, K, _off(A, a_off), lda, _off(B, b_off), ldb, ptr(out), ldc,
                              None, 0, int(accumulate), batch, sA, sB, sC, 0 if split_k is None else int(split_k),
                              ARITH[0] if arith is None else _arith_code(arith), stream()), "asr_gemm_f32(batched)")
    return out


def gemm_side(A, B, out, queue, xcd_mask, trans_a=False, trans_b=False, arith=None):
    code = ARITH[0] if arith is None else _arith_code(arith)
    if (code & 0xff) == ARITH_F32:
        return False
    A, lda = _rowmajor(_dev(A, "A"))
    B, ldb = _rowmajor(_dev(B, "B"))
    M, K = (A.shape[1], A.shape[0]) if trans_a else A.shape
    K2, N = (B.shape[1], B.shape[0]) if trans_b else B.shape
    assert K == K2 and out.shape == (M, N)
    out, ldc = _rowmajor(out)
    check(load().asr_gemm_side_f32(int(trans_a), int(trans_b), M, N, K, ptr(A), lda, ptr(B), ldb, ptr(out), ldc, 1, 0, 0, 0,
                                   code, int(xcd_mask) & 0xff, c_p(queue.data_ptr()), stream()), "asr_gemm_side_f32")
    return True


def gemm_side_batched(A, B, out, queue, xcd_mask, trans_a, trans_b, M, N, K, lda, ldb, ldc, batch, sA, sB, sC, arith=None,
                      a_off=0, b_off=0):
    code = ARITH[0] if arith is None else _arith_code(arith)
    if (code & 0xff) == ARITH_F32:
        return False
    check(load().asr_gemm_side_f32(int(trans_a), int(trans_b), M, N, K, _off(A, a_off), lda, _off(B, b_off), ldb, ptr(out), ldc,
                                   batch, sA, sB, sC, code, int(xcd_mask) & 0xff, c_p(queue.data_ptr()), stream()),
          "asr_gemm_side_f32(batched)")
    return True


def gemm_skinny(A, Bt, bias=None, out=None, accumulate=False):
    A, lda = _rowmajor(_dev(A, "A"))
    Bt, ldb = _rowmajor(_dev(Bt, "Bt"))
    M, K = A.shape
    N = Bt.shape[0]
    if out is None:
        out = torch.empty(M, N, device=A.device, dtype=torch.float32)
    out, ldc = _rowmajor(out)
    check(load().asr_gemm_skinny_f32(M, N, K, ptr(A), lda, ptr(Bt), ldb, ptr(out), ldc, ptr(bias), int(accumulate),
                                     None, 0, 0, stream()), "asr_gemm_skinny_f32")
    return out


class BeamSearch:

    def __init__(self, B, K, V, L, eos, device):
        if not 1 <= K <= BEAM_KMAX:
            raise ValueError("beam width %d outside 1..%d" % (K, BEAM_KMAX))
        i32 = dict(dtype=torch.int32, device=device)
        self.B, self.K, self.V, self.L, self.eos = B, K, V, L, eos
        self.scores = torch.full((B, K), float("-inf"), dtype=torch.float32, device=device)
        self.scores[:, 0] = 0.0
        self.tok_hist = torch.empty(L, B, K, **i32)
        self.bp_hist = torch.empty(L, B, K, **i32)
        self.fin = torch.empty(B, BEAM_FCAP, 4, **i32)
        self.fin_score = torch.empty(B, BEAM_FCAP, dtype=torch.float32, device=device)
        counters = torch.zeros(2 * B + 1, **i32)
        self.nfin, self.done, self.ndone = counters[:B], counters[B:2 * B], counters[2 * B:]
        self._counters = counters
        self.struct = Beam(B=B, K=K, V=V, L=L, eos=eos, logits=None, scores=ptr(self.scores),
                           tok_hist=ptr(self.tok_hist), bp_hist=ptr(self.bp_hist), fin=ptr(self.fin),
                           fin_score=ptr(self.fin_score), nfin=ptr(self.nfin), done=ptr(self.done), ndone=ptr(self.ndone))

    def select(self, logits, t):
        assert logits.is_contiguous() and tuple(logits.shape) == (self.B * self.K, self.V)
        self.struct.logits = ptr(logits)
        check(load().asr_beam_select_f32(ctypes.byref(self.struct), int(t), stream()), "asr_beam_select_f32")

    def select_lm(self, logits, lm_logits, lm_weight, t):
        assert logits.is_contiguous() and tuple(logits.shape) == (self.B * self.K, self.V)
        assert lm_logits.is_contiguous() and lm_logits.shape == logits.shape
        self.struct.logits = ptr(logits)
        check(load().asr_beam_select_lm_f32(ctypes.byref(self.struct), ptr(lm_logits), float(lm_weight), int(t), stream()),
              "asr_beam_select_lm_f32")

    @staticmethod
    def _state(x_src, x_dst, c_src, c_dst, w_src, w_dst, emb, D, O):
        assert x_dst.stride(0) == x_src.stride(0) and emb.is_contiguous()
        return BeamState(D=D, O=O, E=emb.shape[1], Tp=w_src.shape[1], ldx=x_src.stride(0), x_src=ptr(x_src),
                         x_dst=ptr(x_dst), c_src=ptr(c_src), c_dst=ptr(c_dst), w_src=ptr(w_src), w_dst=ptr(w_dst),
                         emb=ptr(emb))

    def reorder(self, t, x_src, x_dst, c_src, c_dst, w_src, w_dst, emb, D, O):
        st = self._state(x_src, x_dst, c_src, c_dst, w_src, w_dst, emb, D, O)
        check(load().asr_beam_reorder_f32(ctypes.byref(self.struct), int(t), ctypes.byref(st), stream()),
              "asr_beam_reorder_f32")

    def reorder_lm(self, t, lm_state, dec=None):
        st = self._state(*dec) if dec is not None else None
        check(load().asr_beam_reorder_lm_f32(ctypes.byref(self.struct), int(t), ctypes.byref(st) if st is not None else None,
                                             ctypes.byref(lm_state.reorder_struct()), stream()), "asr_beam_reorder_lm_f32")

    def backtrack(self, length_penalty=0.0):
        dev = self.scores.device
        tokens = torch.empty(self.B, self.K, self.L, dtype=torch.int32, device=dev)
        scores = torch.empty(self.B, self.K, dtype=torch.float32, device=dev)
        lengths = torch.empty(self.B, self.K, dtype=torch.int32, device=dev)
        check(load().asr_beam_backtrack(ctypes.byref(self.struct), float(length_penalty), ptr(tokens), ptr(scores),
                                        ptr(lengths), stream()), "asr_beam_backtrack")
        return tokens, scores, lengths


ED_MAX_COLS = 4096


class UnsupportedShape(RuntimeError):
    """A launcher answered ASR_E_SHAPE: its kernel does not cover these sizes (the caller may have another route)."""


def _ints(t, name, dtypes, dim):
    if t is None:
        return None
    if not t.is_cuda:
        raise RuntimeError("%s must live on the GPU: the HIP path has no CPU fallback" % name)
    if t.dtype not in dtypes:
        raise RuntimeError("%s must be %s, got %s" % (name, " or ".join(str(d) for d in dtypes), t.dtype))
    if t.dim() != dim or (t.shape[-1] > 1 and t.stride(-1) != 1):
        raise RuntimeError("%s must be %d-D with unit stride in its last dimension" % (name, dim))
    return c_p(t.data_ptr())


def edit_distance(hyp, ref, ref_len, *, hyp_len=None, ref_index=None, eos=-1, skip=None, totals=None, out=None):
    N = hyp.shape[0]
    hp = _ints(hyp, "hyp", (torch.int32, torch.int64), 2)
    rp, rlp = _ints(ref, "ref", (torch.int32,), 2), _ints(ref_len, "ref_len", (torch.int32,), 1)
    hlp, rip = _ints(hyp_len, "hyp_len", (torch.int32,), 1), _ints(ref_index, "ref_index", (torch.int32,), 1)
    sp, tp = _ints(skip, "skip", (torch.uint8,), 1), _ints(totals, "totals", (torch.int64,), 1)
    if ref_len.shape[0] != ref.shape[0] or (ref_index is None and ref.shape[0] < N):
        raise RuntimeError("ref has %d rows, ref_len %d, for %d pairs" % (ref.shape[0], ref_len.shape[0], N))
    for t, n, name in ((hyp_len, N, "hyp_len"), (ref_index, N, "ref_index"), (totals, 2, "totals")):
        if t is not None and t.shape[0] != n:
            raise RuntimeError("%s must have %d entries, got %d" % (name, n, t.shape[0]))
    if out is None:
        out = torch.empty(3, N, dtype=torch.int32, device=hyp.device)
    op = _ints(out, "out", (torch.int32,), 2)
    if tuple(out.shape) != (3, N) or not out.is_contiguous():
        raise RuntimeError("out must be a contiguous int32 [3, %d]" % N)
    rc = load().asr_edit_distance_i32(
        N, hp, hyp.element_size(), hyp.stride(0) if N > 1 else max(hyp.shape[1], 1), hyp.shape[1], hlp, rp,
        ref.stride(0) if ref.shape[0] > 1 else max(ref.shape[1], 1), rlp, rip, int(eos), sp,
        0 if skip is None else skip.shape[0], op, c_p(out[1].data_ptr()), c_p(out[2].data_ptr()), tp, stream())
    if rc == ASR_E_SHAPE:
        raise UnsupportedShape("asr_edit_distance_i32: more than %d columns (hyp %d, ref %d)"
                               % (ED_MAX_COLS, hyp.shape[1], ref.shape[1]))
    check(rc, "asr_edit_distance_i32")
    return out[0], out[1], out[2]


def lm_step(R, H, In, xin, wcat, bcat, c_prev, c_out, h_out, h_out2=None):
    check(load().asr_lm_step_f32(int(R), int(H), int(In), ptr(xin), xin.stride(0), ptr(wcat), ptr(bcat), ptr(c_prev),
                                 ptr(c_out), ptr(h_out), h_out.stride(0), ptr(h_out2),
                                 0 if h_out2 is None else h_out2.stride(0), stream()), "asr_lm_step_f32")


class LmStepState:

    def __init__(self, R, emb, layers, device=None):
        device = emb.device if device is None else device
        n = len(layers)
        if not 1 <= n <= LM_MAX_LAYERS:
            raise ValueError("%d LM layers outside 1..%d" % (n, LM_MAX_LAYERS))
        if not 1 <= R <= LM_MAX_ROWS:
            raise ValueError("%d beam rows outside 1..%d: the LM step kernel does not serve them" % (R, LM_MAX_ROWS))
        f32 = dict(device=device, dtype=torch.float32)
        self.R, self.n, self.H = R, n, layers[0][1].shape[1]
        self.emb = emb.detach().contiguous()
        self.in_dim, self.xin, self.cell, self.wcat, self.bcat = [], [], [], [], []
        with torch.no_grad():
            for l, (w_ih, w_hh, b_ih, b_hh) in enumerate(layers):
                H, In = self.H, w_ih.shape[1]
                want = self.emb.shape[1] if l == 0 else H
                if tuple(w_hh.shape) != (4 * H, H) or w_ih.shape[0] != 4 * H or In != want:
                    raise ValueError("LM layer %d: weights %s / %s do not stack on input width %d, hidden width %d"
                                     % (l, tuple(w_ih.shape), tuple(w_hh.shape), want, H))
                self.in_dim.append(In)
                self.xin.append(torch.zeros(2, R, In + H, **f32))
                self.cell.append(torch.zeros(2, R, H, **f32))
                w = torch.cat([w_ih.detach(), w_hh.detach()], dim=1).view(4, H, In + H)
                self.wcat.append(w.transpose(0, 1).reshape(4 * H, In + H).contiguous())
                self.bcat.append((b_ih.detach() + b_hh.detach()).view(4, H).t().contiguous().view(-1))
        self._reorder = None

    def prime(self, token):
# ... 805 lines not shown
```

semi-supervised-asr_amd/ops.py:

```python
import ctypes
import os
import weakref

import torch

import hip_backend as hb


def gate_perm(H, device):
    return torch.arange(4 * H, device=device).view(4, H).t().reshape(-1)


def gate_unperm(H, device):
    return torch.arange(4 * H, device=device).view(H, 4).t().reshape(-1)


class _Lease(object):

    def __init__(self, free_list, ws):
        self._free, self.ws = free_list, ws

    def release(self):
        if self.ws is not None:
            self._free.append(self.ws)
# ... 18 lines not shown

    def __init__(self):
        self.buf, self.cursor, self.want, self.active = None, 0, 0, False

    def begin(self, device):
        device = torch.device(device)
        if self.buf is None or self.buf.device != device or self.buf.numel() < self.want:
            self.buf = torch.zeros(int(self.want * 1.25) + 4096, device=device, dtype=torch.float32) if self.want > 0 else None
        elif self.cursor > 0:
            self.buf[:self.cursor].zero_()
        if _ARENA_DEBUG and self.buf is not None:
            assert float(self.buf.abs().max()) == 0.0, "step arena: a value survived behind the cursor"
        self.cursor, self.want, self.active = 0, 0, True

    def end(self):
        self.active = False

    def take(self, shape, device):
        if not self.active:
            return None
        n = 1
        for v in shape:
            n *= int(v)
        n4 = (n + 63) // 64 * 64
        self.want += n4
        if self.buf is None or self.buf.device != torch.device(device) or self.cursor + n4 > self.buf.numel():
            return None
        shape = tuple(int(v) for v in shape)
        strides, acc = [], 1
        for v in reversed(shape):
            strides.append(acc)
            acc *= v
        out = torch.empty(0, device=self.buf.device, dtype=torch.float32).set_(
            self.buf.untyped_storage(), self.buf.storage_offset() + self.cursor, shape, tuple(reversed(strides)))
        self.cursor += n4
        return out


_ARENA_DEBUG = os.environ.get("ASR_ARENA_DEBUG", "0") == "1"
_ARENA = _Arena()
_LINEAR_ARENA = os.environ.get("ASR_LINEAR_ARENA", "1") != "0"


class step_arena(object):

    def __init__(self, device):
        self.device = device

    def __enter__(self):
        if torch.device(self.device).type == "cuda":
            _ARENA.begin(self.device)
        return _ARENA

    def __exit__(self, *exc):
        _ARENA.end()
        return False


def zeros_acc(shape, device):
    t = _ARENA.take(shape, device)
    return t if t is not None else torch.zeros(*shape, device=device, dtype=torch.float32)


class _SideStream(object):

    def __init__(self):
        self.enabled = os.environ.get("ASR_SIDE_GEMM", "1") != "0"
        self.streams, self.active, self.mask_hint = {}, None, 0
        self.uses = {}
        self.deferred = []
        self.task = -1
        self.launches = 0

    def mask_for(self, nbatch):
        return hb.idle_xcd_mask(nbatch) if self.enabled else 0

    def usable(self, mask):
        return bool(mask) and self.enabled and (hb.current_arith() & 0xff) != hb.ARITH_F32

    def count_use(self, ctx, weight):
        key = weight.data_ptr()
        self.uses[key] = self.uses.get(key, 0) + 1
        weakref.finalize(ctx, self._drop_use, key)

    def _drop_use(self, key):
        n = self.uses.get(key, 0) - 1
        if n > 0:
            self.uses[key] = n
        else:
            self.uses.pop(key, None)

    def may_defer(self, ctx, weight):
        return (ctx.side_mask and ctx.needs_input_grad[0] and weight.is_leaf and weight.grad is None
                and not weight._backward_hooks and not getattr(weight, "_post_accumulate_grad_hooks", None)
                and self.uses.get(weight.data_ptr(), 0) == 1 and self.usable(ctx.side_mask))

    def defer(self, dev, launch, keep):
        main = torch.cuda.current_stream(dev)
        st = self.streams.get(dev.index)
        if st is None:
            st = self.streams[dev.index] = torch.cuda.Stream(device=dev)
        task = torch._C._current_graph_task_id()
        if self.active is not None and task != self.task:
            self.active[0].wait_stream(self.active[1])
            del self.deferred[:]
            self.active = None
        if self.active is None:
            self.active, self.task = (main, st), task
            torch.autograd.Variable._execution_engine.queue_callback(self.join)
        self.deferred.append((launch, keep))
        self.launches += 1

    def flush(self):
        if self.active is None or not self.deferred:
            return
        if self.task != torch._C._current_graph_task_id() and torch._C._current_graph_task_id() != -1:
            return
        main, st = self.active
        ev = torch.cuda.Event()
        ev.record(main)
        st.wait_event(ev)
        with torch.cuda.stream(st):
            for launch, keep in self.deferred:
                launch()
                for t in keep:
                    t.record_stream(st)
        del self.deferred[:]

    def join_now(self):
        if self.active is not None:
            self.flush()
            self.active[0].wait_stream(self.active[1])

    def join(self):
        self.join_now()
        self.active = None


_SIDE = _SideStream()


def _side_product(a, b, out, queue, mask):
    code = hb.current_arith()
    return lambda: hb.gemm_side(a, b, out, queue, mask, trans_a=True, arith=code)


def _gemm_acc(A, B, trans_a=False, trans_b=False, shape=None):
    out = _ARENA.take(shape, A.device) if shape is not None else None
    if out is None:
        return hb.gemm(A, B, trans_a=trans_a, trans_b=trans_b)
    return hb.gemm(A, B, trans_a=trans_a, trans_b=trans_b, out=out, accumulate=True)


def _colsum_acc(X):
    out = _ARENA.take((X.shape[1],), X.device)
    return hb.colsum(X) if out is None else hb.colsum(X, out=out, accumulate=True)


def _with_saved_arith(bwd):
    import functools

    @functools.wraps(bwd)
    def wrapped(ctx, *grads):
        with hb.arith(ctx.arith):
            return bwd(ctx, *grads)
    return wrapped


class _Linear(torch.autograd.Function):
    @staticmethod
    def forward(ctx, x, weight, bias, relu, drop):
        ctx.arith = hb.current_arith()
        x2 = x.reshape(-1, x.shape[-1])
        seeded = isinstance(drop, hb.SeededMask)
        if seeded:
            assert relu and (x2.shape[0] * weight.shape[0]) % 4 == 0
        out = _ARENA.take((x2.shape[0], weight.shape[0]), x2.device) if _LINEAR_ARENA else None
        y = hb.gemm(x2, weight, trans_b=True, bias=bias, relu=relu, drop=drop if seeded else None, out=out,
                    out_zeroed=out is not None)
        ctx.save_for_backward(x2, weight, y if relu else None)
        ctx.side_mask = 0
        if ctx.needs_input_grad[1]:
            _SIDE.count_use(ctx, weight)
            ctx.side_mask = _SIDE.mask_hint if x2.shape[0] >= 512 else 0
        ctx.relu = relu
        ctx.drop = (drop.seed, drop.p) if seeded else None
        ctx.has_bias = bias is not None
        ctx.in_shape = x.shape
        return y.view(*x.shape[:-1], weight.shape[0])

    @staticmethod
    @_with_saved_arith
    def backward(ctx, dy):
        x2, weight, y = ctx.saved_tensors
        dy2 = dy.reshape(-1, dy.shape[-1])
        if not dy2.is_contiguous():
            dy2 = dy2.contiguous()
        if ctx.relu and y.numel() % 4 == 0:
            seed, p = ctx.drop if ctx.drop is not None else (0, 0.0)
            dy2 = hb.relu_dropout_bwd(dy2, y, seed, p)
        elif ctx.relu:
            dy2 = dy2 * (y > 0).to(dy2.dtype)
        dx = hb.gemm(dy2, weight).view(ctx.in_shape) if ctx.needs_input_grad[0] else None
        if _SIDE.may_defer(ctx, weight):
            dw = zeros_acc((dy2.shape[1], x2.shape[1]), dy2.device)
            queue = zeros_acc((1,), dy2.device)
            _SIDE.defer(dy2.device, _side_product(dy2, x2, dw.detach(), queue, ctx.side_mask), (dy2, x2, queue))
        else:
            dw = _gemm_acc(dy2, x2, trans_a=True, shape=(dy2.shape[1], x2.shape[1]))
        db = _colsum_acc(dy2) if ctx.has_bias else None
        return dx, dw, db, None, None


def linear(x, weight, bias=None, relu=False, drop=None):
    return _Linear.apply(x, weight, bias, relu, drop)


def _row_capacity(n):
    n = max(int(n), 1)
    q = max(256, 1 << max(n.bit_length() - 3, 0))
    return (n + q - 1) // q * q


def _lstm_workspace(rows, nbatch, H, ndir, dev, with_bwd):
    f32 = dict(device=dev, dtype=torch.float32)
    alloc = torch.zeros if with_bwd else torch.empty
    ws = dict(gates_buf=alloc(rows + 1, ndir, 4 * H, **f32), y_buf=alloc(rows + 1, ndir * H, **f32),
              c_buf=torch.empty(rows, ndir * H, **f32))
    if with_bwd:
        n1, n2, n3 = nbatch * ndir * H, ndir * 4 * H * H, ndir * 4 * H
        zbuf = torch.empty(n1 + n2 + n3, **f32)
        ws.update(w_hhT=torch.empty(ndir, H, 4 * H, **f32), dy_buf=torch.empty(rows, ndir * H, **f32), zbuf=zbuf,
                  dcarry=zbuf[:n1].view(nbatch, ndir * H), dw_hh=zbuf[n1:n1 + n2].view(ndir, 4 * H, H),
                  db=zbuf[n1 + n2:].view(ndir * 4 * H))
    return ws


def _lstm_views(ws, T, B, H, ndir):
    n = T * B
    ws["gates"] = ws["gates_buf"][:n].view(T, B, ndir, 4 * H)
    ws["y"] = ws["y_buf"][:n].view(T, B, ndir * H)
    ws["c"] = ws["c_buf"][:n].view(T, B, ndir * H)
    if "dy_buf" in ws:
        ws["dy"] = ws["dy_buf"][:n].view(T, B, ndir * H)
    return ws


class _LstmPack(torch.autograd.Function):

    @staticmethod
    def forward(ctx, ndir, nlayers, *params):
        per = 4 * ndir
        layers = [params[per * j:per * (j + 1)] for j in range(nlayers)]
        ctx.ndir, ctx.dims = ndir, [(lp[1].shape[1], lp[0].shape[1]) for lp in layers]
        ctx.set_materialize_grads(False)
        outs = hb.lstm_pack_multi(layers, ndir)
        return tuple(t for out in outs for t in out)

    @staticmethod
    def backward(ctx, *grads):
        _SIDE.join_now()
        n = len(ctx.dims)
        per_layer = [grads[3 * j:3 * j + 3] for j in range(n)]
        for j, g in enumerate(per_layer):
            if any(t is None for t in g) and not all(t is None for t in g):
                H, I = ctx.dims[j]
                ref = next(t for t in g if t is not None)
                shp = ((ctx.ndir * 4 * H, I), (ctx.ndir, 4 * H, H), (ctx.ndir * 4 * H,))
                per_layer[j] = [t if t is not None else torch.zeros(shp[k], device=ref.device) for k, t in enumerate(g)]
        outs = hb.lstm_unpack_multi(per_layer, ctx.dims, ctx.ndir)
        flat = []
        for j in range(n):
            flat += outs[j] if outs[j] is not None else [None] * (4 * ctx.ndir)
        return (None, None) + tuple(flat)


def lstm_pack(layers, ndir):
    flat = [p for lp in layers for p in lp]
    out = _LstmPack.apply(ndir, len(layers), *flat)
    return [out[3 * j:3 * j + 3] for j in range(len(layers))]


class _LstmLayer(torch.autograd.Function):

    @staticmethod
    def forward(ctx, x, lens, ndir, pooled, rows, w_ih, w_hh, bias):
        ctx.arith = hb.current_arith()
        T, B, I = x.shape
        H = w_hh.shape[2]
        dev = x.device
        x2 = x.reshape(T * B, I)
        nbatch = rows.B if rows is not None else B
        if pooled:
            cap = _row_capacity(T * B)
            lease = _POOL.acquire(("lstm", dev.index, cap, nbatch, H, ndir),
                                  lambda: _lstm_workspace(cap, nbatch, H, ndir, dev, True))
            ws = lease.ws
        else:
            lease, ws = None, _lstm_workspace(T * B, nbatch, H, ndir, dev, False)
        _lstm_views(ws, T, B, H, ndir)
        ws["rows_written"] = max(ws.get("rows_written", 0), T * B)
        ctx.side_mask = _SIDE.mask_hint = _SIDE.mask_for(nbatch) if pooled else 0
        ws["lens"] = lens
        hb.gemm(x2, w_ih, trans_b=True, bias=bias, out=ws["gates"].view(T * B, ndir * 4 * H))
        hb.lstm_seq_fwd(ws["gates"], w_hh, ws["lens"], ws["y"], ws["c"], use_graphs=pooled, rows=rows)
        ctx.save_for_backward(x2, w_ih, w_hh)
        ctx.lease = lease
        ctx.rows = rows
        ctx.dims = (T, B, I, H, ndir)
        return ws["y"].detach()

    @staticmethod
    @_with_saved_arith
    def backward(ctx, dy):
        x2, w_ih, w_hh = ctx.saved_tensors
        T, B, I, H, ndir = ctx.dims
        lease = ctx.lease
        assert lease is not None and lease.ws is not None, "lstm_layer backward needs the leased workspace " \
            "(autograd was off in forward, or backward ran twice)"
        ws = _lstm_views(lease.ws, T, B, H, ndir)
        dev = dy.device
        dyc = dy if dy.is_contiguous() else ws["dy"].copy_(dy)
        zb = _ARENA.take((ws["zbuf"].numel(),), dev)
        if zb is None:
            ws["zbuf"].zero_()
        else:
            nb_, n2 = ws["dcarry"].numel(), ws["dw_hh"].numel()
            ws = dict(ws, dcarry=zb[:nb_].view_as(ws["dcarry"]), dw_hh=zb[nb_:nb_ + n2].view_as(ws["dw_hh"]),
                      db=zb[nb_ + n2:].view_as(ws["db"]))
        gates, y = ws["gates"], ws["y"]
        _SIDE.flush()
        fused_dw, fused_db = hb.lstm_seq_bwd(gates, lambda: ws["w_hhT"].copy_(w_hh.transpose(1, 2)), ws["lens"], dyc,
                                             ws["c"], ws["dcarry"], y=y, dw_hh=ws["dw_hh"], db=ws["db"],
                                             w_hh=w_hh, rows=ctx.rows)
        dG = gates.view(T * B, ndir * 4 * H)
        with_hh = not fused_dw and T > 1
        ldg, ldy = ndir * 4 * H, ndir * H
        kk = T * B if ctx.rows is not None else (T - 1) * B
        hh_shape = (True, False, 4 * H, H, kk, ldg, ldy, H, ndir, 4 * H - B * ldg, B * ldy + H, 4 * H * H)
        side = bool(ctx.side_mask and ctx.needs_input_grad[0] and _SIDE.usable(ctx.side_mask))
        if side:
            dw_ih = zeros_acc((ndir * 4 * H, I), dev)
            queue = zeros_acc((2,), dev)
            dw_hh_side = ws["dw_hh"] if zb is not None else torch.zeros_like(ws["dw_hh"])
        if with_hh and ctx.rows is not None and ws.get("rows_written", 0) > T * B:
            ws["gates_buf"][T * B].zero_()
            ws["y_buf"][T * B].zero_()
        dx = hb.gemm(dG, w_ih).view(T, B, I) if ctx.needs_input_grad[0] else None
        if side:
            mask, code = ctx.side_mask, hb.current_arith()

            def launch():
                hb.gemm_side(dG, x2, dw_ih, queue[0:1], mask, trans_a=True, arith=code)
                if with_hh:
                    hb.gemm_side_batched(dG, y, dw_hh_side, queue[1:2], mask, *hh_shape, arith=code, a_off=B * ldg)
            _SIDE.defer(dev, launch, (x2, queue))
        else:
            dw_ih = _gemm_acc(dG, x2, trans_a=True, shape=(ndir * 4 * H, I))
        db = ws["db"] if fused_db else _colsum_acc(dG)
        if with_hh and not side:
            hb.gemm_batched(dG, y, ws["dw_hh"], *hh_shape, accumulate=True, a_off=B * ldg)
        dw_hh, db = (ws["dw_hh"], db) if zb is not None else (ws["dw_hh"].clone(), db.clone() if fused_db else db)
        if side and with_hh:
# ... 80 lines not shown
        hb.dec_prepare(tokens, emb_w.contiguous(), xmask, X, Xd, fed, L, B, D, O, E)
    else:
        fed = _dec_clear(buf)
        fed.copy_(tokens.t())
        X[:L, :, D + O:] = emb_w[fed]
        if Xd is not None:
            Xd[:L, :, D + O:] = X[:L, :, D + O:] * xmask[:, :, O:]
    hb.dec_seq_fwd(buf, use_graphs)
    logits = hb.gemm(X[1:].view(L * B, buf.KX)[:, :D + O], w_out, trans_b=True, bias=b_out).view(L, B, w_out.shape[0])
    return fed, logits, (None if skip_pred else logits.argmax(-1))


def _dec_free_kernels(buf, emb_w, tokens, tf_flags, smooth, opts, w_out, b_out):
    B, L, D, O = (buf.dims[k] for k in "BLDO")
    X, Xd, dev, V = buf.X, buf.Xd, buf.X.device, w_out.shape[0]
    fed = _dec_clear(buf)
    logits = torch.empty(L, B, V, device=dev, dtype=torch.float32)
    pred = torch.empty(L, B, dtype=torch.long, device=dev)
    emb_c = emb_w.contiguous()
    probs_saved = torch.empty(max(L - 1, 1), B, V, device=dev, dtype=torch.float32) if smooth and tokens is None else []
    tok_c = tokens.contiguous() if tokens is not None else None
    fed[0] = tok_c[:, 0] if tok_c is not None else opts["bos"]
    X[0, :, D + O:] = emb_c[fed[0]]
    if Xd is not None:
        Xd[0, :, D + O:] = X[0, :, D + O:] * buf.xmask[0, :, O:]
    done = hb.dec_free_fwd(buf, w_out, b_out, emb_c, logits, pred, fed, probs_saved, tok_c, tf_flags, smooth,
                           float(opts.get("smooth_scaling", 1.0)), int(opts.get("eos", -1)))
    return fed, logits, pred, probs_saved, done


def _dec_free_torch(buf, emb_w, tokens, tf_flags, smooth, sample, opts, w_out, b_out):
    B, L, D, O = (buf.dims[k] for k in "BLDO")
    X, Xd, dev, V = buf.X, buf.Xd, buf.X.device, w_out.shape[0]
    fed = _dec_clear(buf)
    fs = buf.fwd_struct()
    logits = torch.empty(L, B, V, device=dev, dtype=torch.float32)
    pred = torch.empty(L, B, dtype=torch.long, device=dev)
    probs_saved = []
    for s in range(L):
        if s == 0:
            tok = tokens[:, 0] if tokens is not None else torch.full((B,), opts["bos"], dtype=torch.long, device=dev)
            fed[0] = tok
            X[0, :, D + O:] = emb_w[tok]
        elif tokens is not None:
            tok = tokens[:, s] if tf_flags[s] else pred[s - 1]
            fed[s] = tok
            X[s, :, D + O:] = emb_w[tok]
        elif not smooth:
            fed[s] = pred[s - 1]
            X[s, :, D + O:] = emb_w[pred[s - 1]]
        else:
            pr = torch.softmax(logits[s - 1] * opts["smooth_scaling"], dim=-1)
            probs_saved.append(pr)
            fed[s] = -1
            hb.gemm(pr, emb_w, out=X[s][:, D + O:])
        if Xd is not None:
            Xd[s, :, D + O:] = X[s, :, D + O:] * buf.xmask[s, :, O:]
        hb.dec_step_fwd(fs, s)
        hb.gemm_skinny(X[s + 1][:, :D + O], w_out, bias=b_out, out=logits[s])
        pred[s] = torch.distributions.Categorical(logits=logits[s]).sample() if sample else logits[s].argmax(-1)
    return fed, logits, pred, probs_saved


def _dec_smooth_bwd_torch(buf, acc, with_dws, w_out, emb_w, probs_saved, k, dw_out, db_out, demb_w):
    D, O = buf.dims["D"], buf.dims["O"]
    hb.count_path("dec_bwd", False, "free-running smooth: %s L=%d fused-feedback=False" % (hb.dec_shape(buf), buf.L))
    bs = buf.bwd_struct(0, None, acc, with_dws)
    G, X = acc["G"], buf.X
    for s in range(buf.L - 1, -1, -1):
        hb.dec_step_bwd(bs, s)
        if s >= 1:
            demb = G[s][:, D + O:]
            pr = probs_saved[s - 1]
            hb.gemm(pr, demb, trans_a=True, out=demb_w, accumulate=True, split_k=1)
            dp = hb.gemm(demb, emb_w, trans_b=True)
            dl = (k * pr * (dp - (pr * dp).sum(-1, keepdim=True))).contiguous()
            hb.gemm(dl, w_out, out=G[s][:, :D + O], accumulate=True, split_k=1)
            hb.gemm(dl, X[s][:, :D + O], trans_a=True, out=dw_out, accumulate=True, split_k=1)
            hb.colsum(dl, out=db_out, accumulate=True)


class _DecoderSeq(torch.autograd.Function):

    @staticmethod
    def forward(ctx, P, Q, emb_w, w_ih, w_hh, b_ih, b_hh, wdec, convw, watt, gvec, bo, w_out, b_out, w0, opts):
        ctx.arith = hb.current_arith()
        dev = P.device
        B, Tp, A = P.shape
        O = Q.shape[2]
        D = w_hh.shape[1]
        E = emb_w.shape[1]
        V = w_out.shape[0]
        C = convw.shape[0]
        K = (convw.shape[-1] - 1) // 2
        L = int(opts["L"])
        KX = D + O + E
        xmask_in = opts.get("xmask")
        drop = xmask_in is not None
        pooled = bool(opts.get("pooled", False))
        if pooled:
            lease = _POOL.acquire(("dec", dev.index, B, Tp, A, D, O, E, C, K, L, drop),
                                  lambda: hb.DecBuffers(B, Tp, A, D, O, E, C, K, L, drop, dev, True))
            buf = lease.ws
        else:
            lease, buf = None, hb.DecBuffers(B, Tp, A, D, O, E, C, K, L, drop, dev, False)
        hb.dec_pack(w_ih, w_hh, b_ih, b_hh, wdec, watt, D, O, E, A, C, buf.wcat, buf.bcat, buf.wcatT, buf.wdecT, buf.wattT)
        buf.bind(P, Q, w0, convw, gvec, bo, wdec, watt, xmask_in, opts.get("scaling", 2.0))
        w_out_c = w_out.contiguous()
        tokens = opts.get("tokens")
        tf_flags = opts.get("tf_flags")
        smooth = bool(opts.get("smooth", False))
        sample = bool(opts.get("sample", False))
        all_teacher = tokens is not None and (tf_flags is None or all(tf_flags)) and not sample
        probs_saved, done = [], False
        if all_teacher:
            fed, logits, pred = _dec_teacher_forced(buf, emb_w, tokens, w_out_c, b_out, pooled, opts.get("skip_pred"))
        elif hb.USE_FEEDBACK_KERNEL and not sample and V <= 128:
            fed, logits, pred, probs_saved, done = _dec_free_kernels(buf, emb_w, tokens, tf_flags, smooth, opts, w_out_c, b_out)
        else:
            fed, logits, pred, probs_saved = _dec_free_torch(buf, emb_w, tokens, tf_flags, smooth, sample, opts, w_out_c, b_out)
        ctx.lease = lease
        ctx.keep = (fed, probs_saved, w_out_c, emb_w)
        ctx.dims = (B, Tp, A, O, D, E, V, C, K, L, KX)
        ctx.smooth = smooth and tokens is None
        ctx.all_teacher = all_teacher
        ctx.free_persist = (not all_teacher) and done and not ctx.smooth
        ctx.smooth_scaling = float(opts.get("smooth_scaling", 1.0))
        if pred is not None:
            ctx.mark_non_differentiable(pred)
        ctx.set_materialize_grads(False)
        return logits, (buf.ws.detach() if pooled else buf.ws.clone()), pred

    @staticmethod
    @_with_saved_arith
    def backward(ctx, dlogits, dws, _dpred):
        fed, probs_saved, w_out, emb_w = ctx.keep
        B, Tp, A, O, D, E, V, C, K, L, KX = ctx.dims
        lease = ctx.lease
        assert lease is not None and lease.ws is not None, "decoder_sequence backward needs the leased workspace"
        buf = lease.ws
        X, Xd = buf.X, buf.Xd
        dev = X.device
        if dlogits is None:
            dlogits = torch.zeros(L, B, V, device=dev, dtype=torch.float32)
        dlog2 = dlogits.contiguous().view(L * B, V)
        zb = _ARENA.take((buf.zbuf.numel(),), dev)
        if zb is None:
            buf.zbuf.zero_()
            acc = buf.acc
        else:
            acc = buf.accumulators(zb)
        G = acc["G"]
        XO = X[1:].view(L * B, KX)[:, :D + O]
        hb.gemm(dlog2, w_out, out=G[1:].view(L * B, KX)[:, :D + O])
        dw_out = _gemm_acc(dlog2, XO, trans_a=True, shape=(V, D + O))
        db_out = _colsum_acc(dlog2)
        if dws is not None:
            buf.dws.copy_(dws)
        demb_w = zeros_acc(tuple(emb_w.shape), dev)
        if not ctx.smooth:
            hb.dec_seq_bwd(buf, acc, dws is not None, ctx.all_teacher or ctx.free_persist, ctx.all_teacher)
        elif torch.is_tensor(probs_saved):
            dtot = hb.dec_smooth_bwd(buf, acc, dws is not None, w_out.contiguous(), emb_w.contiguous(), probs_saved,
                                     ctx.smooth_scaling, dlog2)
            dw_out = hb.gemm(dtot.view(L * B, V), XO, trans_a=True)
            db_out = hb.colsum(dtot.view(L * B, V))
            if L > 1:
                hb.gemm(probs_saved[:L - 1].view((L - 1) * B, V), G[1:L].view((L - 1) * B, KX)[:, D + O:], trans_a=True,
                        out=demb_w, accumulate=True, split_k=1)
        else:
            _dec_smooth_bwd_torch(buf, acc, dws is not None, w_out, emb_w, probs_saved, ctx.smooth_scaling, dw_out, db_out,
                                  demb_w)
        dg2 = buf.dgates.view(L * B, 4 * D)
        Xin = X[:L] if Xd is None else Xd[:L]
        dwcat = _gemm_acc(dg2, Xin.reshape(L * B, KX), trans_a=True, shape=(4 * D, KX))
        dw_ih, dw_hh, dbias, dbias2 = hb.cell_unpack(dwcat, _colsum_acc(dg2), D, O, E)
        dwdec = _gemm_acc(buf.dD.view(L * B, A), X[1:].view(L * B, KX)[:, :D], trans_a=True, shape=(A, D))
        dgvec, dwatt, dconvw = hb.colsum_parts([acc["dgvec_part"], acc["dwatt_part"], acc["dconv_part"]])
        dgvec, dconvw = dgvec.view(1, A), dconvw.view(C, 1, 1, 2 * K + 1)
        dQ = torch.empty(B, Tp, O, device=dev, dtype=torch.float32)
        dctx_base = G[1:]
        hb.gemm_batched(buf.ws, dctx_base[:, :, D:], dQ, True, False, Tp, O, L, B * Tp, B * KX, O, B, Tp, KX,
                        Tp * O)
        dbo = _colsum_acc(dctx_base.view(L * B, KX)[:, D:D + O])
        demb_all = G[:L, :, D + O:]
        nsteps = 1 if torch.is_tensor(probs_saved) else L
        if not hb.embedding_grad(fed[:nsteps].reshape(-1), G[:nsteps].view(nsteps * B, KX)[:, D + O:], demb_w):
            if torch.is_tensor(probs_saved):
                demb_w.index_add_(0, fed[0], demb_all[0])
            elif not probs_saved:
                demb_w.index_add_(0, fed.view(-1), demb_all.reshape(L * B, E))
            else:
                tokfed = fed >= 0
                demb_w.index_add_(0, fed[tokfed], demb_all[tokfed])
        dP = acc["dP"] if zb is not None else acc["dP"].clone()
        lease.release()
        return (dP, dQ, demb_w, dw_ih, dw_hh, dbias, dbias2, dwdec, dconvw, dwatt, dgvec, dbo, dw_out, db_out,
                None, None)


class _LabelLogProb(torch.autograd.Function):

    @staticmethod
    def forward(ctx, logits, index, labeldist, ls_weight, with_sum, sum_scale, with_argmax):
        lg = logits.contiguous()
        V = lg.shape[-1]
        rows = lg.numel() // V
        idx = index.contiguous()
        out = torch.empty(lg.shape[:-1], device=lg.device, dtype=torch.float32)
        total = zeros_acc((1,), lg.device).view(()) if with_sum else None
        amax = torch.empty(lg.shape[:-1], device=lg.device, dtype=torch.long) if with_argmax else None
        dist = labeldist.contiguous() if labeldist is not None else None
        hb.check(hb.load().asr_label_logprob_fwd(rows, V, hb.ptr(lg), V, ctypes.c_void_p(idx.data_ptr()), hb.ptr(dist),
                                                 float(ls_weight), hb.ptr(out), hb.ptr(total), float(sum_scale),
                                                 None if amax is None else ctypes.c_void_p(amax.data_ptr()), hb.stream()),
                 "asr_label_logprob_fwd")
        ctx.save_for_backward(lg, idx, dist)
        ctx.ls, ctx.sum_scale = float(ls_weight), float(sum_scale)
        ctx.set_materialize_grads(False)
        if amax is not None:
            ctx.mark_non_differentiable(amax)
        return out, total, amax

    @staticmethod
    def backward(ctx, g, gt, _gamax):
        lg, idx, dist = ctx.saved_tensors
        V = lg.shape[-1]
        rows = lg.numel() // V
        if g is None and gt is None:
            return (None,) * 7
        if g is None:
            gc, stride, scale = gt.contiguous(), 0, ctx.sum_scale
        else:
            gc, stride, scale = (g if gt is None else g + gt * ctx.sum_scale).contiguous(), 1, 1.0
        dz = torch.empty_like(lg)
        hb.check(hb.load().asr_label_logprob_bwd(rows, V, hb.ptr(lg), V, ctypes.c_void_p(idx.data_ptr()), hb.ptr(dist),
                                                 ctx.ls, hb.ptr(gc), stride, scale, hb.ptr(dz), V, hb.stream()),
                 "asr_label_logprob_bwd")
        return (dz,) + (None,) * 6


def label_logprob(logits, index, labeldist=None, ls_weight=0.0, with_sum=False, sum_scale=1.0, with_argmax=False):
    out, total, amax = _LabelLogProb.apply(logits, index, labeldist, ls_weight, with_sum, sum_scale, with_argmax)
    res = (out,) + ((total,) if with_sum else ()) + ((amax,) if with_argmax else ())
    return res if len(res) > 1 else out


def decoder_sequence(P, Q, emb_w, w_ih, w_hh, b_ih, b_hh, wdec, convw, watt, gvec, bo, w_out, b_out, w0, opts):
    opts = dict(opts)
    opts["pooled"] = torch.is_grad_enabled() and (P.requires_grad or w_hh.requires_grad)
    return _DecoderSeq.apply(P, Q, emb_w, w_ih, w_hh, b_ih, b_hh, wdec, convw, watt, gvec, bo, w_out, b_out, w0, opts)


def attention_step(enc_pad, P, Q, wdec, convw, watt, gvec, bo, dec_z, att_prev, scaling):
    dev = P.device
    B, Tp, A = P.shape
    O, D, C = Q.shape[2], wdec.shape[1], convw.shape[0]
    K = (convw.shape[-1] - 1) // 2
    E = 16
    buf = hb.DecBuffers(B, Tp, A, D, O, E, C, K, 1, False, dev, False)
    with torch.no_grad():
        buf.P.copy_(P); buf.Q.copy_(Q); buf.w0.copy_(att_prev)
        buf.convw.copy_(convw.reshape(C, 2 * K + 1)); buf.gvec.copy_(gvec.reshape(A)); buf.wattT.copy_(watt.t())
        buf.wcat.zero_(); buf.bcat.zero_(); buf.X.zero_()
        buf.X[1, :, :D] = dec_z
        buf.bind(bo=bo, wdec=wdec, watt=watt, scaling=scaling)
        hb.att_step_fwd(buf.fwd_struct(), 0)
        return buf.X[1, :, D:D + O].clone(), buf.ws[0].clone()


BEAM_POLL_STEPS = 8


def beam_search(P, Q, emb_w, w_ih, w_hh, b_ih, b_hh, wdec, convw, watt, gvec, bo, w_out, b_out, w0, beam, L, bos, eos,
                length_penalty=0.0, scaling=2.0, lm=None, lm_weight=0.0):
    dev = P.device
    B, Tp, A = P.shape
    O = Q.shape[2]
    D = w_hh.shape[1]
    E = emb_w.shape[1]
    V = w_out.shape[0]
    C = convw.shape[0]
    Kc = (convw.shape[-1] - 1) // 2
    R = B * beam
    f32 = dict(device=dev, dtype=torch.float32)
    fused = lm is not None and float(lm_weight) != 0.0
    if fused and (tuple(lm["w_out"].shape) != (V, lm["layers"][-1][1].shape[1]) or lm["emb"].shape[0] != V):
        raise ValueError("the LM's vocabulary (%d outputs, %d embeddings) is not the decoder's (%d)"
                         % (lm["w_out"].shape[0], lm["emb"].shape[0], V))
    with torch.no_grad():
        search = hb.BeamSearch(B, beam, V, L, eos, dev)
        if fused:
            lms = hb.LmStepState(R, lm["emb"], lm["layers"], dev)
            lms.prime(bos)
            lm_w_out, lm_b_out = lm["w_out"].detach().contiguous(), lm["b_out"].detach().contiguous()
            lm_logits = torch.empty(R, V, **f32)
        buf = hb.DecBuffers(R, Tp, A, D, O, E, C, Kc, 2, False, dev, False)
        buf.bind(P.repeat_interleave(beam, 0), Q.repeat_interleave(beam, 0), w0.repeat_interleave(beam, 0), convw, gvec, bo,
                 wdec, watt, None, scaling)
        X, cst, wts = buf.X.zero_(), buf.cstate.zero_(), buf.ws
        hb.dec_pack(w_ih, w_hh, b_ih, b_hh, wdec, watt, D, O, E, A, C, buf.wcat, buf.bcat, None, None, buf.wattT)
        fs = buf.fwd_struct()
        emb_c, w_out_c = emb_w.contiguous(), w_out.contiguous()
        X[1, :, D + O:] = emb_c[bos]
        wts[0].copy_(buf.w0)
        logits = torch.empty(R, V, **f32)
        landing = torch.zeros(1, dtype=torch.int32).pin_memory()
        polled = None
        steps = launches = 0
        for t in range(L):
            hb.dec_step_fwd(fs, 1)
            hb.gemm_skinny(X[2][:, :D + O], w_out_c, bias=b_out, out=logits)
            if fused:
                lms.step()
                hb.gemm_skinny(lms.top(), lm_w_out, bias=lm_b_out, out=lm_logits)
                search.select_lm(logits, lm_logits, lm_weight, t)
                launches += lms.n + 1
            else:
                search.select(logits, t)
            steps += 1
            launches += 6
            if t == L - 1:
                break
            if fused:
                search.reorder_lm(t, lms, (X[2], X[1], cst[1], cst[0], wts[1], wts[0], emb_c, D, O))
            else:
                search.reorder(t, X[2], X[1], cst[1], cst[0], wts[1], wts[0], emb_c, D, O)
            launches += 1
            if (t + 1) % BEAM_POLL_STEPS == 0:
                if polled is not None:
                    polled.synchronize()
                    if int(landing[0]) == B:
                        break
                landing.copy_(search.ndone, non_blocking=True)
                polled = torch.cuda.Event()
                polled.record()
# ... 5 lines not shown
```

Before: 2754.

## Group independent backward GEMMs into one launch with fused column sums

After: 2766, median of 6. Within noise of the previous version (+0.4%).

```diff
diff --git a/include/asr_hip.h b/include/asr_hip.h
--- a/include/asr_hip.h
+++ b/include/asr_hip.h
@@ -45,6 +45,22 @@
 int asr_gemm_side_f32(int transA, int transB, int64_t M, int64_t N, int64_t K, const float* A, int64_t lda,
                       const float* B, int64_t ldb, float* C, int64_t ldc, int batch, int64_t sA, int64_t sB, int64_t sC,
                       int arith, unsigned xcd_mask, unsigned* queue, asr_stream_t stream);
+
+#define ASR_GEMM_GROUP_MAX 8
+typedef struct {
+  int transA, transB;
+  int64_t M, N, K;
+  const float* A; int64_t lda;
+  const float* B; int64_t ldb;
+  float* C; int64_t ldc;
+  const float* bias;
+  int relu, accumulate, batch, split_k;
+  int64_t sA, sB, sC;
+  int flags, colsum, colsum_accumulate, reserved;
+  float* colsum_out;
+} AsrGemmJob;
+int asr_gemm_group_f32(const AsrGemmJob* jobs, int njobs, int arith, asr_stream_t stream);
+int asr_gemm_group_plan(const AsrGemmJob* jobs, int njobs, int arith, int* first, int* kinds, int cap);
 
 int asr_gemm_skinny_f32(int64_t M, int64_t N, int64_t K,
                         const float* A, int64_t lda, const float* Bt, int64_t ldb,
diff --git a/semi-supervised-asr_amd/csrc/gemm.hip b/semi-supervised-asr_amd/csrc/gemm.hip
--- a/semi-supervised-asr_amd/csrc/gemm.hip
+++ b/semi-supervised-asr_amd/csrc/gemm.hip
@@ -1,13 +1,8 @@
 #include <cstdlib>
 #include <type_traits>
 #include "common.h"
-
-#ifndef ASR_GEMM_BF3_TOUCH
-#define ASR_GEMM_BF3_TOUCH 2
-#endif
-#ifndef ASR_GB_ABL
-#define ASR_GB_ABL 0
-#endif
+#include "gemm_bf3.h"
+
 #ifndef ASR_GLDS_CLOBBER_M0
 #define ASR_GLDS_CLOBBER_M0 0
 #endif
@@ -16,32 +11,7 @@
 #endif
 namespace {
 
-constexpr int BM = 128, BN = 128, BK = 32;
-#ifndef ASR_GEMM_SMALL_OCC
-#define ASR_GEMM_SMALL_OCC 1
-#endif
-#ifndef ASR_GEMM_TOUCH
-#define ASR_GEMM_TOUCH 2
-#endif
-
-struct MatView {
-  const float* p;
-  int64_t ld, R, Cn;
-  bool vec;
-};
-
-__device__ __forceinline__ float4 load4_guard(const MatView& m, int64_t r, int64_t c) {
-  float4 v = make_float4(0.f, 0.f, 0.f, 0.f);
-  if (r >= m.R) return v;
-  const float* q = m.p + r * m.ld + c;
-  if (m.vec && c + 3 < m.Cn) return *reinterpret_cast<const float4*>(q);
-  if (c < m.Cn) v.x = q[0];
-  if (c + 1 < m.Cn) v.y = q[1];
-  if (c + 2 < m.Cn) v.z = q[2];
-  if (c + 3 < m.Cn) v.w = q[3];
-  return v;
-}
-
+constexpr int BM = 128, BN = 128;
 template <bool KC>
 struct TileCfg {
   static constexpr int S = KC ? 129 : 128;
@@ -81,17 +51,6 @@
   }
 }
 
-struct GemmArgs {
-  MatView A, B;
-  float* C;
-  int64_t ldc, M, N, K;
-  const float* bias;
-  int relu, accumulate, split_k;
-  int64_t sA, sB, sC;
-  int tiles_m, tiles_n;
-  unsigned* queue;
-  unsigned xcd_mask;
-};
 
 
 #ifndef ASR_GEMM_GM
@@ -275,101 +234,10 @@
   }
 }
 
-typedef __bf16 gbf16x8 __attribute__((ext_vector_type(8)));
-typedef __bf16 gbf16x2 __attribute__((ext_vector_type(2)));
-typedef unsigned gu32x4 __attribute__((ext_vector_type(4)));
-constexpr int BS = 40;
-
-__device__ __forceinline__ unsigned bf3g_hi2(float a, float b) {
-  return __builtin_amdgcn_perm(__float_as_uint(b), __float_as_uint(a), 0x07060302u);
-}
-__device__ __forceinline__ unsigned bf3g_lo2(float a, float b) {
-  const float la = a - __uint_as_float(__float_as_uint(a) & 0xffff0000u);
-  const float lb = b - __uint_as_float(__float_as_uint(b) & 0xffff0000u);
-  const gbf16x2 p = {(__bf16)la, (__bf16)lb};
-  return __builtin_bit_cast(unsigned, p);
-}
-
-template <int NT>
-__device__ __forceinline__ void bfn_split2(float x, float y, unsigned (&t)[NT]) {
-  if constexpr (NT == 2) {
-    t[0] = bf3g_hi2(x, y);
-    t[1] = bf3g_lo2(x, y);
-  } else {
-    const gbf16x2 pa = {(__bf16)x, (__bf16)y};
-    const unsigned ua = __builtin_bit_cast(unsigned, pa);
-    const float rx = x - __uint_as_float(ua << 16), ry = y - __uint_as_float(ua & 0xffff0000u);
-    const gbf16x2 pb = {(__bf16)rx, (__bf16)ry};
-    const unsigned ub = __builtin_bit_cast(unsigned, pb);
-    const float sx = rx - __uint_as_float(ub << 16), sy = ry - __uint_as_float(ub & 0xffff0000u);
-    t[0] = ua;
-    t[1] = ub;
-    t[2] = bf3g_hi2(sx, sy);
-  }
-}
-
-template <bool KC, int TS>
-__device__ __forceinline__ void tile_fetch_bf3(const MatView& m, int64_t row0, int64_t k0, float4 (&v)[TS / 32]) {
-  const int t = threadIdx.x;
-#pragma unroll
-  for (int i = 0; i < TS / 32; ++i) {
-    if (KC) {
-      const int f = t + 256 * i;
-      v[i] = load4_guard(m, row0 + (f >> 3), k0 + 4 * (f & 7));
-    } else if (TS == 128) {
-      v[i] = load4_guard(m, k0 + 4 * (t & 7) + i, row0 + 4 * (t >> 3));
-    } else {
-      v[i] = load4_guard(m, k0 + 4 * (t & 7) + 2 * (t >> 7) + i, row0 + 4 * ((t >> 3) & 15));
-    }
-  }
-}
-
-template <bool KC, int NT, int TS>
-__device__ __forceinline__ void tile_store_bf3(unsigned short* img, const float4 (&v)[TS / 32]) {
-  const int t = threadIdx.x;
-  if (KC) {
-#pragma unroll
-    for (int i = 0; i < TS / 32; ++i) {
-      const int f = t + 256 * i;
-      const int o = (f >> 3) * BS + 4 * (f & 7);
-      unsigned p0[NT], p1[NT];
-      bfn_split2<NT>(v[i].x, v[i].y, p0);
-      bfn_split2<NT>(v[i].z, v[i].w, p1);
-#pragma unroll
-      for (int k = 0; k < NT; ++k) *reinterpret_cast<uint2*>(img + k * TS * BS + o) = make_uint2(p0[k], p1[k]);
-    }
-  } else if constexpr (TS == 64) {
-    const int o = 4 * ((t >> 3) & 15) * BS + 4 * (t & 7) + 2 * (t >> 7);
-    const float r[4][2] = {{v[0].x, v[1].x}, {v[0].y, v[1].y}, {v[0].z, v[1].z}, {v[0].w, v[1].w}};
-#pragma unroll
-    for (int j = 0; j < 4; ++j) {
-      unsigned p0[NT];
-      bfn_split2<NT>(r[j][0], r[j][1], p0);
-#pragma unroll
-      for (int k = 0; k < NT; ++k) *reinterpret_cast<unsigned*>(img + k * TS * BS + o + j * BS) = p0[k];
-    }
-  } else {
-    const int o = 4 * (t >> 3) * BS + 4 * (t & 7);
-    const float r[4][4] = {{v[0].x, v[1].x, v[2].x, v[3].x}, {v[0].y, v[1].y, v[2].y, v[3].y},
-                           {v[0].z, v[1].z, v[2].z, v[3].z}, {v[0].w, v[1].w, v[2].w, v[3].w}};
-#pragma unroll
-    for (int j = 0; j < 4; ++j) {
-      unsigned p0[NT], p1[NT];
-      bfn_split2<NT>(r[j][0], r[j][1], p0);
-      bfn_split2<NT>(r[j][2], r[j][3], p1);
-#pragma unroll
-      for (int k = 0; k < NT; ++k) *reinterpret_cast<uint2*>(img + k * TS * BS + o + j * BS) = make_uint2(p0[k], p1[k]);
-    }
-  }
-}
-
 template <bool AKC, bool BKC, int NT, int TS = 128, bool QUEUE = false>
 __global__ __launch_bounds__(256, QUEUE ? 4 : (TS == 64 ? ASR_GEMM_SMALL_OCC : 1)) void gemm_bf3_kernel(GemmArgs g) {
   static_assert(!QUEUE || TS == 64, "the queue instantiation is the 64 x 64 tile");
-  constexpr int BM = TS, BN = TS, NP = TS / 32, NB = TS / 64;
-  __shared__ __attribute__((aligned(16))) unsigned short smem[2 * NT * BM * BS];
-  unsigned short* Ai = smem;
-  unsigned short* Bi = smem + NT * BM * BS;
+  __shared__ __attribute__((aligned(16))) unsigned short smem[2 * NT * TS * BS];
 
   const int ntile = g.tiles_m * g.tiles_n;
   int tid = blockIdx.x;
@@ -388,255 +256,7 @@
     const int q = ntile >> 3, rmd = ntile & 7, xcd = tid & 7, idx = tid >> 3;
     tid = (xcd < rmd ? xcd * (q + 1) : rmd * (q + 1) + (xcd - rmd) * q) + idx;
   }
-  const int tm = tid / g.tiles_n, tn = tid % g.tiles_n;
-  const int bz = z / g.split_k, kz = z % g.split_k;
-
-  MatView A = g.A, B = g.B;
-  A.p += bz * g.sA;
-  B.p += bz * g.sB;
-  float* C = g.C + bz * g.sC;
-
-  const int64_t m0 = (int64_t)tm * BM, n0 = (int64_t)tn * BN;
-  const int64_t ktiles = (g.K + BK - 1) / BK;
-  const int64_t per = (ktiles + g.split_k - 1) / g.split_k;
-  const int64_t kt_begin = kz * per;
-  const int64_t kt_end = kt_begin + per < ktiles ? kt_begin + per : ktiles;
-
-  const int lane = threadIdx.x & 63, wave = threadIdx.x >> 6;
-  const int wm = wave >> 1, wn = wave & 1;
-  const int l31 = lane & 31, kh = lane >> 5;
-
-  f32x16 acc[NB][NB];
-#pragma unroll
-  for (int i = 0; i < NB; ++i)
-#pragma unroll
-    for (int j = 0; j < NB; ++j)
-#pragma unroll
-      for (int e = 0; e < 16; ++e) acc[i][j][e] = 0.f;
-
-  const bool fast_a = A.vec && (AKC ? (m0 + BM <= A.R) : (m0 + BM <= A.Cn)) && A.R * A.ld < (int64_t)1 << 30;
-  const bool fast_b = B.vec && (BKC ? (n0 + BN <= B.R) : (n0 + BN <= B.Cn)) && B.R * B.ld < (int64_t)1 << 30;
-  const bool fast = fast_a && fast_b;
-  unsigned offa[NP], offb[NP];
-#pragma unroll
-  for (int i = 0; i < NP; ++i) {
-    const int f = threadIdx.x + 256 * i;
-    const int t = threadIdx.x;
-    const int krow = TS == 128 ? 4 * (t & 7) + i : 4 * (t & 7) + 2 * (t >> 7) + i, rq = TS == 128 ? (t >> 3) : ((t >> 3) & 15);
-    offa[i] = AKC ? (unsigned)((f >> 3) * A.ld + 4 * (f & 7)) : (unsigned)(krow * A.ld + 4 * rq);
-    offb[i] = BKC ? (unsigned)((f >> 3) * B.ld + 4 * (f & 7)) : (unsigned)(krow * B.ld + 4 * rq);
-  }
-  const float* basea = AKC ? A.p + m0 * A.ld : A.p + m0;
-  const float* baseb = BKC ? B.p + n0 * B.ld : B.p + n0;
-  float4 ra[NP], rb[NP];
-  auto fetch_fast = [&](int64_t kt2) {
-    const int64_t k0 = kt2 * BK;
-    const float* pa = basea + (AKC ? k0 : k0 * A.ld);
-    const float* pb = baseb + (BKC ? k0 : k0 * B.ld);
-#pragma unroll
-    for (int i = 0; i < NP; ++i) ra[i] = *reinterpret_cast<const float4*>(pa + offa[i]);
-#pragma unroll
-    for (int i = 0; i < NP; ++i) rb[i] = *reinterpret_cast<const float4*>(pb + offb[i]);
-  };
-  auto fetch_guard = [&](int64_t kt2) {
-    const int64_t k0 = kt2 * BK;
-    tile_fetch_bf3<AKC, TS>(A, m0, k0, ra);
-    tile_fetch_bf3<BKC, TS>(B, n0, k0, rb);
-  };
-  const int tt = threadIdx.x & 127;
-  const bool touch_a = threadIdx.x < 128;
-  float touched = 0.f;
-  const bool do_touch = TS == 128 && kt_end - kt_begin > 2 * ASR_GEMM_BF3_TOUCH;
-  auto touch_tile = [&](int64_t ktt) {
-    const MatView& m = touch_a ? A : B;
-    const bool kc = touch_a ? AKC : BKC;
-    const int64_t r0t = touch_a ? m0 : n0;
-    int64_t rr, cc;
-    if (kc) { rr = r0t + tt; cc = ktt * BK; }
-    else { rr = ktt * BK + (tt >> 2); cc = r0t + 32 * (tt & 3); }
-    rr = rr < m.R ? rr : m.R - 1;
-    cc = cc < m.Cn ? cc : m.Cn - 1;
-    touched = m.p[rr * m.ld + cc];
-  };
-  const int ao = (wm * (TS / 2) + l31) * BS + 8 * kh, bo = (wn * (TS / 2) + l31) * BS + 8 * kh;
-  auto multiply = [&]() {
-#pragma unroll
-    for (int ks = 0; ks < ((ASR_GB_ABL & 1) ? 0 : BK / 16); ++ks) {
-      gu32x4 af[NB][NT], bf[NB][NT];
-#pragma unroll
-      for (int i = 0; i < NB; ++i)
-#pragma unroll
-        for (int k = 0; k < NT; ++k) {
-          af[i][k] = *reinterpret_cast<const gu32x4*>(Ai + k * BM * BS + ao + 32 * i * BS + 16 * ks);
-          bf[i][k] = *reinterpret_cast<const gu32x4*>(Bi + k * BM * BS + bo + 32 * i * BS + 16 * ks);
-        }
-#define BF3G(a_, b_, c_) c_ = __builtin_amdgcn_mfma_f32_32x32x16_bf16(__builtin_bit_cast(gbf16x8, a_), __builtin_bit_cast(gbf16x8, b_), c_, 0, 0, 0)
-#pragma unroll
-      for (int o = 0; o < NT; ++o)
-#pragma unroll
-        for (int p = 0; p <= o; ++p)
-#pragma unroll
-          for (int i = 0; i < NB; ++i)
-#pragma unroll
-            for (int j = 0; j < NB; ++j) BF3G(af[i][p], bf[j][o - p], acc[i][j]);
-#undef BF3G
-    }
-  };
-  const int64_t kt_full = g.K / BK < kt_end ? g.K / BK : kt_end;
-  const int64_t kt_fast_end = (fast && kt_full > kt_begin) ? kt_full : kt_begin;
-  if constexpr (TS == 64) {
-    constexpr int PD = QUEUE ? 1 : 3;
-    float4 qa[PD][NP], qb[PD][NP];
-    auto fetch_set = [&](int64_t kt2, float4 (&xa)[NP], float4 (&xb)[NP]) __attribute__((always_inline)) {
-      const int64_t k0 = kt2 * BK;
-      const float* pa = basea + (AKC ? k0 : k0 * A.ld);
-      const float* pb = baseb + (BKC ? k0 : k0 * B.ld);
-#pragma unroll
-      for (int i = 0; i < NP; ++i) xa[i] = *reinterpret_cast<const float4*>(pa + offa[i]);
-#pragma unroll
-      for (int i = 0; i < NP; ++i) xb[i] = *reinterpret_cast<const float4*>(pb + offb[i]);
-    };
-    int64_t kt = kt_begin;
-    if (kt < kt_fast_end) {
-#pragma unroll
-      for (int d = 0; d < PD; ++d)
-        if (kt + d < kt_fast_end) fetch_set(kt + d, qa[d], qb[d]);
-      for (; kt + 2 * PD <= kt_fast_end; kt += PD) {
-#pragma unroll
-        for (int d = 0; d < PD; ++d) {
-          __builtin_amdgcn_sched_barrier(0);
-          tile_store_bf3<AKC, NT, TS>(Ai, qa[d]);
-          tile_store_bf3<BKC, NT, TS>(Bi, qb[d]);
-          __syncthreads();
-          fetch_set(kt + d + PD, qa[d], qb[d]);
-          multiply();
-          __syncthreads();
-          __builtin_amdgcn_sched_barrier(0);
-        }
-      }
-#pragma unroll
-      for (int d = 0; d < 2 * PD - 1; ++d) {
-        if (kt + d < kt_fast_end) {
-          tile_store_bf3<AKC, NT, TS>(Ai, qa[d % PD]);
-          tile_store_bf3<BKC, NT, TS>(Bi, qb[d % PD]);
-          __syncthreads();
-          if (kt + d + PD < kt_fast_end) fetch_set(kt + d + PD, qa[d % PD], qb[d % PD]);
-          multiply();
-          __syncthreads();
-        }
-      }
-    }
-  } else if (kt_begin < kt_fast_end) {
-    fetch_fast(kt_begin);
-    for (int64_t kt = kt_begin; kt < kt_fast_end; ++kt) {
-#if ASR_GB_ABL & 4
-      if (kt == kt_begin) {
-        tile_store_bf3<AKC, NT, TS>(Ai, ra);
-        tile_store_bf3<BKC, NT, TS>(Bi, rb);
-      } else {
-#pragma unroll
-        for (int i = 0; i < NP; ++i) asm volatile("" ::"v"(ra[i].x), "v"(ra[i].y), "v"(ra[i].z), "v"(ra[i].w), "v"(rb[i].x), "v"(rb[i].y), "v"(rb[i].z), "v"(rb[i].w));
-      }
-#else
-      tile_store_bf3<AKC, NT, TS>(Ai, ra);
-      tile_store_bf3<BKC, NT, TS>(Bi, rb);
-#endif
-      __syncthreads();
-      if (kt + 1 < kt_fast_end && !(ASR_GB_ABL & 2)) fetch_fast(kt + 1);
-#if ASR_GEMM_TOUCH
-      asm volatile("" ::"v"(touched));
-      if (do_touch && kt + ASR_GEMM_BF3_TOUCH < kt_end) touch_tile(kt + ASR_GEMM_BF3_TOUCH);
-#endif
-      multiply();
-      __syncthreads();
-    }
-  }
-  if (kt_fast_end < kt_end) {
-    fetch_guard(kt_fast_end);
-    for (int64_t kt = kt_fast_end; kt < kt_end; ++kt) {
-      tile_store_bf3<AKC, NT, TS>(Ai, ra);
-      tile_store_bf3<BKC, NT, TS>(Bi, rb);
-      __syncthreads();
-      if (kt + 1 < kt_end) fetch_guard(kt + 1);
-#if ASR_GEMM_TOUCH
-      asm volatile("" ::"v"(touched));
-      if (do_touch && kt + ASR_GEMM_BF3_TOUCH < kt_end) touch_tile(kt + ASR_GEMM_BF3_TOUCH);
-#endif
-      multiply();
-      __syncthreads();
-    }
-  }
-
-#if ASR_GB_ABL & 8
-  if (threadIdx.x + blockIdx.x + blockIdx.y != 0 || g.M != 1) {
-#pragma unroll
-    for (int i = 0; i < NB; ++i)
-#pragma unroll
-      for (int j = 0; j < NB; ++j)
-#pragma unroll
-        for (int e = 0; e < 16; ++e) asm volatile("" ::"v"(acc[i][j][e]));
-    return;
-  }
-#endif
-  if (m0 + BM <= g.M && n0 + BN <= g.N) {
-    const unsigned ldc = (unsigned)g.ldc;
-    const bool split = QUEUE || g.split_k > 1, accum = g.accumulate != 0, relu = g.relu != 0;
-#pragma unroll
-    for (int j = 0; j < NB; ++j) {
-      const int64_t n = n0 + wn * (TS / 2) + j * 32 + l31;
-      const float bv = g.bias ? g.bias[n] : 0.f;
-#pragma unroll
-      for (int i = 0; i < NB; ++i) {
-        float* base = C + (m0 + wm * (TS / 2) + i * 32 + 4 * kh) * g.ldc + n;
-        if (split) {
-#pragma unroll
-          for (int e = 0; e < 16; ++e) atomicAdd(base + (unsigned)((e & 3) + 8 * (e >> 2)) * ldc, acc[i][j][e]);
-        } else if (accum) {
-          float old[16];
-#pragma unroll
-          for (int e = 0; e < 16; ++e) old[e] = base[(unsigned)((e & 3) + 8 * (e >> 2)) * ldc];
-#pragma unroll
-          for (int e = 0; e < 16; ++e) {
-            float v = acc[i][j][e] + bv + old[e];
-            if (relu) v = fmaxf(v, 0.f);
-            base[(unsigned)((e & 3) + 8 * (e >> 2)) * ldc] = v;
-          }
-        } else {
-#pragma unroll
-          for (int e = 0; e < 16; ++e) {
-            float v = acc[i][j][e] + bv;
-            if (relu) v = fmaxf(v, 0.f);
-            base[(unsigned)((e & 3) + 8 * (e >> 2)) * ldc] = v;
-          }
-        }
-      }
-    }
-    return;
-  }
-#pragma unroll
-  for (int j = 0; j < NB; ++j) {
-    const int64_t n = n0 + wn * (TS / 2) + j * 32 + l31;
-    if (n >= g.N) continue;
-    const float bv = g.bias ? g.bias[n] : 0.f;
-#pragma unroll
-    for (int i = 0; i < NB; ++i) {
-#pragma unroll
-      for (int e = 0; e < 16; ++e) {
-        const int64_t m = m0 + wm * (TS / 2) + i * 32 + (e & 3) + 8 * (e >> 2) + 4 * kh;
-        if (m >= g.M) continue;
-        float v = acc[i][j][e];
-        float* dst = C + m * g.ldc + n;
-        if (QUEUE || g.split_k > 1) {
-          atomicAdd(dst, v);
-        } else {
-          v += bv;
-          if (g.accumulate) v += *dst;
-          if (g.relu) v = fmaxf(v, 0.f);
-          *dst = v;
-        }
-      }
-    }
-  }
+  gemm_bf3_tile<AKC, BKC, NT, TS, QUEUE>(g, tid, z, smem);
 }
 
 constexpr int WM = 256, WN = 128, WK = 32;
@@ -1828,45 +1448,30 @@
 
 __global__ void colsum_kernel(int64_t M, int64_t N, const float* X, int64_t ldx, float* out) {
   __shared__ float part[4][64];
-  const int cx = threadIdx.x & 63, ry = threadIdx.x >> 6;
-  const int64_t n = (int64_t)blockIdx.x * 64 + cx;
-  const int64_t mbeg = (int64_t)blockIdx.y * 512;
-  const int64_t mend = mbeg + 512 < M ? mbeg + 512 : M;
-  float s = 0.f;
-  if (n < N)
-    for (int64_t m = mbeg + ry; m < mend; m += 4) s += X[m * ldx + n];
-  part[ry][cx] = s;
-  __syncthreads();
-  if (ry == 0 && n < N) atomicAdd(out + n, (part[0][cx] + part[1][cx]) + (part[2][cx] + part[3][cx]));
+  colsum_body(M, N, X, ldx, out, blockIdx.x, blockIdx.y, part);
 }
 
 __global__ __launch_bounds__(256) void colsum4_kernel(int64_t M, int64_t N, const float* __restrict__ X, int64_t ldx,
                                                       float* out) {
   __shared__ float4 part[16][16];
-  const int cq = threadIdx.x & 15, ry = threadIdx.x >> 4;
-  const int64_t n = (int64_t)blockIdx.x * 64 + 4 * cq;
-  const int64_t mbeg = (int64_t)blockIdx.y * 256;
-  const int64_t mend = mbeg + 256 < M ? mbeg + 256 : M;
-  float4 s = make_float4(0.f, 0.f, 0.f, 0.f);
-  if (n < N) {
-    const float* p = X + n;
-#pragma unroll 4
-    for (int64_t m = mbeg + ry; m < mend; m += 16) {
-      const float4 v = *reinterpret_cast<const float4*>(p + m * ldx);
-      s.x += v.x; s.y += v.y; s.z += v.z; s.w += v.w;
-    }
-  }
-  part[ry][cq] = s;
-  __syncthreads();
-  if (threadIdx.x < 64) {
-    const int q = threadIdx.x >> 2, e = threadIdx.x & 3;
-    float t = 0.f;
-#pragma unroll
-    for (int r = 0; r < 16; ++r) t += reinterpret_cast<const float*>(&part[r][q])[e];
-    const int64_t col = (int64_t)blockIdx.x * 64 + threadIdx.x;
-    if (col < N) atomicAdd(out + col, t);
-  }
-}
+  colsum4_body(M, N, X, ldx, out, blockIdx.x, blockIdx.y, part);
+}
+
+constexpr int64_t GROUP_MAX_WGS = (int64_t)1 << 30;
+struct GroupSink {
+  GroupJobs jobs;
+  int64_t wgs;
+  bool plan_only;
+  bool add(const GemmArgs& g, int kind, int64_t count) {
+    if (jobs.n >= GROUP_MAX_SLOTS) return false;
+    jobs.g[jobs.n] = g;
+    jobs.kind[jobs.n] = kind;
+    jobs.first[jobs.n] = (int)wgs;
+    wgs += count;
+    ++jobs.n;
+    return true;
+  }
+};
 
 }
 
@@ -1902,7 +1507,7 @@
 static int gemm_impl(int transA, int transB, int64_t M, int64_t N, int64_t K, const float* A, int64_t lda,
                      const float* B, int64_t ldb, float* C, int64_t ldc, const float* bias, int relu,
                      int accumulate, int batch, int64_t sA, int64_t sB, int64_t sC, int split_k, int arith,
-                     DropEpi drop, hipStream_t stream) {
+                     DropEpi drop, hipStream_t stream, GroupSink* sink = nullptr) {
   if (!A || !B || !C || M <= 0 || N <= 0 || K <= 0 || batch <= 0) return ASR_E_ARG;
   if (drop.thresh && (batch != 1 || accumulate)) return ASR_E_ARG;
   const DropEpi no_drop = {0ull, 0u, 1.f};
@@ -1940,6 +1545,7 @@
     const int tiles_n = (int)((N + 127) / 128);
     if (tiles_n <= 256) {
       const int groups = 8 * (tiles_n >= 32 ? 1 : 32 / tiles_n);
+      if (sink && sink->plan_only) return 0;
       g.bias = bias; g.relu = relu; g.split_k = 1;
       dim3 grid(tiles_n * groups, batch, 1), b4(512);
       const bool plain = M % 128 == 0 && N % 128 == 0 && !relu && !accumulate && M * ldc < ((int64_t)1 << 29);
@@ -1968,6 +1574,7 @@
   const bool wide = use_sp || (ar != ASR_ARITH_F32 && !(arith & (ASR_GEMM_TILE_NARROW | ASR_GEMM_TILE_SP | ASR_GEMM_TILE_SMALL)) && wide_shape &&
                                ((wide_pays && !small) || (arith & ASR_GEMM_TILE_WIDE)) && (auto_split || split_k == 1));
   if (wide) {
+    if (sink && sink->plan_only) return 0;
     const int64_t tiles = wtiles, stages = (K + WK - 1) / WK;
     int best = 1;
     if (may_split) {
@@ -2030,6 +1637,11 @@
   const int64_t ktiles = (K + BK - 1) / BK;
   if (split_k > ktiles) split_k = (int)ktiles;
   g.split_k = split_k;
+  if (sink && small && !drop.thresh && !late_epilogue && !(split_k > 1 && !accumulate && !(arith & ASR_GEMM_C_ZEROED)) &&
+      (int64_t)g.tiles_m * g.tiles_n * batch * split_k + sink->wgs <= GROUP_MAX_WGS &&
+      sink->add(g, (akc ? 1 : 0) | (bkc ? 2 : 0), (int64_t)g.tiles_m * g.tiles_n * batch * split_k))
+    return 0;
+  if (sink && sink->plan_only) return 0;
   if (split_k > 1 && !accumulate && !(arith & ASR_GEMM_C_ZEROED)) {
     dim3 zg((unsigned)((M * N + 255) / 256 > 2048 ? 2048 : (M * N + 255) / 256), 1, batch);
     hipLaunchKernelGGL(zero_rows_kernel, zg, dim3(256), 0, stream, C, ldc, M, N, sC);
@@ -2055,6 +1667,83 @@
   const DropEpi none = {0ull, 0u, 1.f};
   return gemm_impl(transA, transB, M, N, K, A, lda, B, ldb, C, ldc, bias, relu, accumulate, batch, sA, sB, sC, split_k, arith,
                    none, (hipStream_t)stream);
+}
+
+static int group_fill(const AsrGemmJob& q, int arith, GroupSink& sink, hipStream_t stream, bool plan_only) {
+  const DropEpi none = {0ull, 0u, 1.f};
+  const int ar = arith & ASR_ARITH_MASK;
+  if (ar != ASR_ARITH_F32 && ar != ASR_ARITH_BF16X6 && ar != ASR_ARITH_BF16X3) return ASR_E_ARG;
+  sink.plan_only = plan_only;
+  const int rc = gemm_impl(q.transA, q.transB, q.M, q.N, q.K, q.A, q.lda, q.B, q.ldb, q.C, q.ldc, q.bias, q.relu, q.accumulate,
+                           q.batch, q.sA, q.sB, q.sC, q.split_k, arith | (q.flags & ASR_GEMM_C_ZEROED), none, stream, &sink);
+  if (rc) return rc;
+  if (q.colsum) {
+    const bool ofA = q.colsum == 1;
+    const float* X = ofA ? q.A : q.B;
+    const int64_t ld = ofA ? q.lda : q.ldb, cols = ofA ? q.M : q.N, sX = ofA ? q.sA : q.sB;
+    const bool vec = cols % 4 == 0 && ld % 4 == 0 && asr_aligned16(X) && sX % 4 == 0;
+    GemmArgs c = {};
+    c.A.p = X; c.A.ld = ld; c.A.R = q.K; c.A.Cn = cols; c.A.vec = vec;
+    c.C = q.colsum_out; c.sA = sX;
+    c.tiles_m = (int)((cols + 63) / 64);
+    c.tiles_n = (int)((q.K + (vec ? 255 : 511)) / (vec ? 256 : 512));
+    c.split_k = vec ? 1 : 0;
+    const int64_t count = (int64_t)c.tiles_m * c.tiles_n * q.batch;
+    if (count + sink.wgs > GROUP_MAX_WGS) return ASR_E_SHAPE;
+    if (!plan_only && !q.colsum_accumulate) {
+      hipError_t e = hipMemsetAsync(q.colsum_out, 0, (size_t)cols * sizeof(float), stream);
+      if (e != hipSuccess) return (int)e;
+    }
+    if (!sink.add(c, GROUP_COLSUM, count)) return ASR_E_SHAPE;
+  }
+  return 0;
+}
+
+static int group_check(const AsrGemmJob* jobs, int njobs) {
+  if (!jobs || njobs <= 0) return ASR_E_ARG;
+  if (njobs > ASR_GEMM_GROUP_MAX) return ASR_E_SHAPE;
+  for (int j = 0; j < njobs; ++j) {
+    const AsrGemmJob& q = jobs[j];
+    if (!q.A || !q.B || !q.C || q.M <= 0 || q.N <= 0 || q.K <= 0 || q.batch <= 0) return ASR_E_ARG;
+    if (q.colsum < 0 || q.colsum > 2 || (q.colsum && !q.colsum_out)) return ASR_E_ARG;
+    if ((q.colsum == 1 && !q.transA) || (q.colsum == 2 && q.transB)) return ASR_E_SHAPE;
+    const int64_t sk = q.split_k > 1 ? q.split_k : 1;
+    if (q.batch * sk > 65535) return ASR_E_SHAPE;
+    const int64_t tiles = ((q.M + 63) / 64) * ((q.N + 63) / 64) * q.batch;
+    if (tiles > GROUP_MAX_WGS / 64 || q.K > ((int64_t)1 << 40)) return ASR_E_SHAPE;
+    if ((q.bias || q.relu) && q.accumulate && sk > 1) return ASR_E_SHAPE;
+  }
+  return 0;
+}
+
+extern "C" int asr_gemm_group_plan(const AsrGemmJob* jobs, int njobs, int arith, int* first, int* kinds, int cap) {
+  int rc = group_check(jobs, njobs);
+  if (rc) return rc;
+  GroupSink sink;
+  sink.jobs.n = 0; sink.wgs = 0; sink.plan_only = false;
+  rc = 0;
+  for (int j = 0; j < njobs && !rc; ++j) rc = group_fill(jobs[j], arith, sink, nullptr, true);
+  if (rc) return rc;
+  if (sink.jobs.n + 1 > cap) return ASR_E_ARG;
+  for (int s = 0; s < sink.jobs.n; ++s) { first[s] = sink.jobs.first[s]; kinds[s] = sink.jobs.kind[s]; }
+  first[sink.jobs.n] = (int)sink.wgs;
+  return sink.jobs.n;
+}
+
+extern "C" int asr_gemm_group_f32(const AsrGemmJob* jobs, int njobs, int arith, asr_stream_t stream_) {
+  hipStream_t stream = (hipStream_t)stream_;
+  int rc = group_check(jobs, njobs);
+  if (rc) return rc;
+  GroupSink sink;
+  sink.jobs.n = 0; sink.wgs = 0; sink.plan_only = false;
+  for (int j = 0; j < njobs; ++j) {
+    rc = group_fill(jobs[j], arith, sink, stream, false);
+    if (rc) return rc;
+  }
+  if (!sink.jobs.n) return 0;
+  sink.jobs.first[sink.jobs.n] = (int)sink.wgs;
+  for (int s = sink.jobs.n + 1; s <= GROUP_MAX_SLOTS; ++s) sink.jobs.first[s] = (int)sink.wgs;
+  return asr_gemm_group_launch(&sink.jobs, (int)sink.wgs, (arith & ASR_ARITH_MASK) == ASR_ARITH_BF16X3 ? 2 : 3, stream);
 }
 
 extern "C" int asr_gemm_drop_f32(int transA, int transB, int64_t M, int64_t N, int64_t K, const float* A, int64_t lda,
diff --git a/semi-supervised-asr_amd/csrc/gemm_bf3.h b/semi-supervised-asr_amd/csrc/gemm_bf3.h
--- /dev/null
+++ b/semi-supervised-asr_amd/csrc/gemm_bf3.h
@@ -0,0 +1,447 @@
+#pragma once
+#include "common.h"
+
+#ifndef ASR_GEMM_BF3_TOUCH
+#define ASR_GEMM_BF3_TOUCH 2
+#endif
+#ifndef ASR_GB_ABL
+#define ASR_GB_ABL 0
+#endif
+#ifndef ASR_GEMM_SMALL_OCC
+#define ASR_GEMM_SMALL_OCC 1
+#endif
+#ifndef ASR_GEMM_TOUCH
+#define ASR_GEMM_TOUCH 2
+#endif
+
+namespace {
+
+constexpr int BK = 32;
+
+struct MatView {
+  const float* p;
+  int64_t ld, R, Cn;
+  bool vec;
+};
+
+__device__ __forceinline__ float4 load4_guard(const MatView& m, int64_t r, int64_t c) {
+  float4 v = make_float4(0.f, 0.f, 0.f, 0.f);
+  if (r >= m.R) return v;
+  const float* q = m.p + r * m.ld + c;
+  if (m.vec && c + 3 < m.Cn) return *reinterpret_cast<const float4*>(q);
+  if (c < m.Cn) v.x = q[0];
+  if (c + 1 < m.Cn) v.y = q[1];
+  if (c + 2 < m.Cn) v.z = q[2];
+  if (c + 3 < m.Cn) v.w = q[3];
+  return v;
+}
+
+struct GemmArgs {
+  MatView A, B;
+  float* C;
+  int64_t ldc, M, N, K;
+  const float* bias;
+  int relu, accumulate, split_k;
+  int64_t sA, sB, sC;
+  int tiles_m, tiles_n;
+  unsigned* queue;
+  unsigned xcd_mask;
+};
+
+typedef __bf16 gbf16x8 __attribute__((ext_vector_type(8)));
+typedef __bf16 gbf16x2 __attribute__((ext_vector_type(2)));
+typedef unsigned gu32x4 __attribute__((ext_vector_type(4)));
+constexpr int BS = 40;
+
+__device__ __forceinline__ unsigned bf3g_hi2(float a, float b) {
+  return __builtin_amdgcn_perm(__float_as_uint(b), __float_as_uint(a), 0x07060302u);
+}
+__device__ __forceinline__ unsigned bf3g_lo2(float a, float b) {
+  const float la = a - __uint_as_float(__float_as_uint(a) & 0xffff0000u);
+  const float lb = b - __uint_as_float(__float_as_uint(b) & 0xffff0000u);
+  const gbf16x2 p = {(__bf16)la, (__bf16)lb};
+  return __builtin_bit_cast(unsigned, p);
+}
+
+template <int NT>
+__device__ __forceinline__ void bfn_split2(float x, float y, unsigned (&t)[NT]) {
+  if constexpr (NT == 2) {
+    t[0] = bf3g_hi2(x, y);
+    t[1] = bf3g_lo2(x, y);
+  } else {
+    const gbf16x2 pa = {(__bf16)x, (__bf16)y};
+    const unsigned ua = __builtin_bit_cast(unsigned, pa);
+    const float rx = x - __uint_as_float(ua << 16), ry = y - __uint_as_float(ua & 0xffff0000u);
+    const gbf16x2 pb = {(__bf16)rx, (__bf16)ry};
+    const unsigned ub = __builtin_bit_cast(unsigned, pb);
+    const float sx = rx - __uint_as_float(ub << 16), sy = ry - __uint_as_float(ub & 0xffff0000u);
+    t[0] = ua;
+    t[1] = ub;
+    t[2] = bf3g_hi2(sx, sy);
+  }
+}
+
+template <bool KC, int TS>
+__device__ __forceinline__ void tile_fetch_bf3(const MatView& m, int64_t row0, int64_t k0, float4 (&v)[TS / 32]) {
+  const int t = threadIdx.x;
+#pragma unroll
+  for (int i = 0; i < TS / 32; ++i) {
+    if (KC) {
+      const int f = t + 256 * i;
+      v[i] = load4_guard(m, row0 + (f >> 3), k0 + 4 * (f & 7));
+    } else if (TS == 128) {
+      v[i] = load4_guard(m, k0 + 4 * (t & 7) + i, row0 + 4 * (t >> 3));
+    } else {
+      v[i] = load4_guard(m, k0 + 4 * (t & 7) + 2 * (t >> 7) + i, row0 + 4 * ((t >> 3) & 15));
+    }
+  }
+}
+
+template <bool KC, int NT, int TS>
+__device__ __forceinline__ void tile_store_bf3(unsigned short* img, const float4 (&v)[TS / 32]) {
+  const int t = threadIdx.x;
+  if (KC) {
+#pragma unroll
+    for (int i = 0; i < TS / 32; ++i) {
+      const int f = t + 256 * i;
+      const int o = (f >> 3) * BS + 4 * (f & 7);
+      unsigned p0[NT], p1[NT];
+      bfn_split2<NT>(v[i].x, v[i].y, p0);
+      bfn_split2<NT>(v[i].z, v[i].w, p1);
+#pragma unroll
+      for (int k = 0; k < NT; ++k) *reinterpret_cast<uint2*>(img + k * TS * BS + o) = make_uint2(p0[k], p1[k]);
+    }
+  } else if constexpr (TS == 64) {
+    const int o = 4 * ((t >> 3) & 15) * BS + 4 * (t & 7) + 2 * (t >> 7);
+    const float r[4][2] = {{v[0].x, v[1].x}, {v[0].y, v[1].y}, {v[0].z, v[1].z}, {v[0].w, v[1].w}};
+#pragma unroll
+    for (int j = 0; j < 4; ++j) {
+      unsigned p0[NT];
+      bfn_split2<NT>(r[j][0], r[j][1], p0);
+#pragma unroll
+      for (int k = 0; k < NT; ++k) *reinterpret_cast<unsigned*>(img + k * TS * BS + o + j * BS) = p0[k];
+    }
+  } else {
+    const int o = 4 * (t >> 3) * BS + 4 * (t & 7);
+    const float r[4][4] = {{v[0].x, v[1].x, v[2].x, v[3].x}, {v[0].y, v[1].y, v[2].y, v[3].y},
+                           {v[0].z, v[1].z, v[2].z, v[3].z}, {v[0].w, v[1].w, v[2].w, v[3].w}};
+#pragma unroll
+    for (int j = 0; j < 4; ++j) {
+      unsigned p0[NT], p1[NT];
+      bfn_split2<NT>(r[j][0], r[j][1], p0);
+      bfn_split2<NT>(r[j][2], r[j][3], p1);
+#pragma unroll
+      for (int k = 0; k < NT; ++k) *reinterpret_cast<uint2*>(img + k * TS * BS + o + j * BS) = make_uint2(p0[k], p1[k]);
+    }
+  }
+}
+
+template <bool AKC, bool BKC, int NT, int TS, bool QUEUE>
+__device__ __forceinline__ void gemm_bf3_tile(const GemmArgs g, const int tid, const int z, unsigned short* smem) {
+  constexpr int BM = TS, BN = TS, NP = TS / 32, NB = TS / 64;
+  unsigned short* Ai = smem;
+  unsigned short* Bi = smem + NT * BM * BS;
+  const int tm = tid / g.tiles_n, tn = tid % g.tiles_n;
+  const int bz = z / g.split_k, kz = z % g.split_k;
+
+  MatView A = g.A, B = g.B;
+  A.p += bz * g.sA;
+  B.p += bz * g.sB;
+  float* C = g.C + bz * g.sC;
+
+  const int64_t m0 = (int64_t)tm * BM, n0 = (int64_t)tn * BN;
+  const int64_t ktiles = (g.K + BK - 1) / BK;
+  const int64_t per = (ktiles + g.split_k - 1) / g.split_k;
+  const int64_t kt_begin = kz * per;
+  const int64_t kt_end = kt_begin + per < ktiles ? kt_begin + per : ktiles;
+
+  const int lane = threadIdx.x & 63, wave = threadIdx.x >> 6;
+  const int wm = wave >> 1, wn = wave & 1;
+  const int l31 = lane & 31, kh = lane >> 5;
+
+  f32x16 acc[NB][NB];
+#pragma unroll
+  for (int i = 0; i < NB; ++i)
+#pragma unroll
+    for (int j = 0; j < NB; ++j)
+#pragma unroll
+      for (int e = 0; e < 16; ++e) acc[i][j][e] = 0.f;
+
+  const bool fast_a = A.vec && (AKC ? (m0 + BM <= A.R) : (m0 + BM <= A.Cn)) && A.R * A.ld < (int64_t)1 << 30;
+  const bool fast_b = B.vec && (BKC ? (n0 + BN <= B.R) : (n0 + BN <= B.Cn)) && B.R * B.ld < (int64_t)1 << 30;
+  const bool fast = fast_a && fast_b;
+  unsigned offa[NP], offb[NP];
+#pragma unroll
+  for (int i = 0; i < NP; ++i) {
+    const int f = threadIdx.x + 256 * i;
+    const int t = threadIdx.x;
+    const int krow = TS == 128 ? 4 * (t & 7) + i : 4 * (t & 7) + 2 * (t >> 7) + i, rq = TS == 128 ? (t >> 3) : ((t >> 3) & 15);
+    offa[i] = AKC ? (unsigned)((f >> 3) * A.ld + 4 * (f & 7)) : (unsigned)(krow * A.ld + 4 * rq);
+    offb[i] = BKC ? (unsigned)((f >> 3) * B.ld + 4 * (f & 7)) : (unsigned)(krow * B.ld + 4 * rq);
+  }
+  const float* basea = AKC ? A.p + m0 * A.ld : A.p + m0;
+  const float* baseb = BKC ? B.p + n0 * B.ld : B.p + n0;
+  float4 ra[NP], rb[NP];
+  auto fetch_fast = [&](int64_t kt2) {
+    const int64_t k0 = kt2 * BK;
+    const float* pa = basea + (AKC ? k0 : k0 * A.ld);
+    const float* pb = baseb + (BKC ? k0 : k0 * B.ld);
+#pragma unroll
+    for (int i = 0; i < NP; ++i) ra[i] = *reinterpret_cast<const float4*>(pa + offa[i]);
+#pragma unroll
+    for (int i = 0; i < NP; ++i) rb[i] = *reinterpret_cast<const float4*>(pb + offb[i]);
+  };
+  auto fetch_guard = [&](int64_t kt2) {
+    const int64_t k0 = kt2 * BK;
+    tile_fetch_bf3<AKC, TS>(A, m0, k0, ra);
+    tile_fetch_bf3<BKC, TS>(B, n0, k0, rb);
+  };
+  const int tt = threadIdx.x & 127;
+  const bool touch_a = threadIdx.x < 128;
+  float touched = 0.f;
+  const bool do_touch = TS == 128 && kt_end - kt_begin > 2 * ASR_GEMM_BF3_TOUCH;
+  auto touch_tile = [&](int64_t ktt) {
+    const MatView& m = touch_a ? A : B;
+    const bool kc = touch_a ? AKC : BKC;
+    const int64_t r0t = touch_a ? m0 : n0;
+    int64_t rr, cc;
+    if (kc) { rr = r0t + tt; cc = ktt * BK; }
+    else { rr = ktt * BK + (tt >> 2); cc = r0t + 32 * (tt & 3); }
+    rr = rr < m.R ? rr : m.R - 1;
+    cc = cc < m.Cn ? cc : m.Cn - 1;
+    touched = m.p[rr * m.ld + cc];
+  };
+  const int ao = (wm * (TS / 2) + l31) * BS + 8 * kh, bo = (wn * (TS / 2) + l31) * BS + 8 * kh;
+  auto multiply = [&]() {
+#pragma unroll
+    for (int ks = 0; ks < ((ASR_GB_ABL & 1) ? 0 : BK / 16); ++ks) {
+      gu32x4 af[NB][NT], bf[NB][NT];
+#pragma unroll
+      for (int i = 0; i < NB; ++i)
+#pragma unroll
+        for (int k = 0; k < NT; ++k) {
+          af[i][k] = *reinterpret_cast<const gu32x4*>(Ai + k * BM * BS + ao + 32 * i * BS + 16 * ks);
+          bf[i][k] = *reinterpret_cast<const gu32x4*>(Bi + k * BM * BS + bo + 32 * i * BS + 16 * ks);
+        }
+#define BF3G(a_, b_, c_) c_ = __builtin_amdgcn_mfma_f32_32x32x16_bf16(__builtin_bit_cast(gbf16x8, a_), __builtin_bit_cast(gbf16x8, b_), c_, 0, 0, 0)
+#pragma unroll
+      for (int o = 0; o < NT; ++o)
+#pragma unroll
+        for (int p = 0; p <= o; ++p)
+#pragma unroll
+          for (int i = 0; i < NB; ++i)
+#pragma unroll
+            for (int j = 0; j < NB; ++j) BF3G(af[i][p], bf[j][o - p], acc[i][j]);
+#undef BF3G
+    }
+  };
+  const int64_t kt_full = g.K / BK < kt_end ? g.K / BK : kt_end;
+  const int64_t kt_fast_end = (fast && kt_full > kt_begin) ? kt_full : kt_begin;
+  if constexpr (TS == 64) {
+    constexpr int PD = QUEUE ? 1 : 3;
+    float4 qa[PD][NP], qb[PD][NP];
+    auto fetch_set = [&](int64_t kt2, float4 (&xa)[NP], float4 (&xb)[NP]) __attribute__((always_inline)) {
+      const int64_t k0 = kt2 * BK;
+      const float* pa = basea + (AKC ? k0 : k0 * A.ld);
+      const float* pb = baseb + (BKC ? k0 : k0 * B.ld);
+#pragma unroll
+      for (int i = 0; i < NP; ++i) xa[i] = *reinterpret_cast<const float4*>(pa + offa[i]);
+#pragma unroll
+      for (int i = 0; i < NP; ++i) xb[i] = *reinterpret_cast<const float4*>(pb + offb[i]);
+    };
+    int64_t kt = kt_begin;
+    if (kt < kt_fast_end) {
+#pragma unroll
+      for (int d = 0; d < PD; ++d)
+        if (kt + d < kt_fast_end) fetch_set(kt + d, qa[d], qb[d]);
+      for (; kt + 2 * PD <= kt_fast_end; kt += PD) {
+#pragma unroll
+        for (int d = 0; d < PD; ++d) {
+          __builtin_amdgcn_sched_barrier(0);
+          tile_store_bf3<AKC, NT, TS>(Ai, qa[d]);
+          tile_store_bf3<BKC, NT, TS>(Bi, qb[d]);
+          __syncthreads();
+          fetch_set(kt + d + PD, qa[d], qb[d]);
+          multiply();
+          __syncthreads();
+          __builtin_amdgcn_sched_barrier(0);
+        }
+      }
+#pragma unroll
+      for (int d = 0; d < 2 * PD - 1; ++d) {
+        if (kt + d < kt_fast_end) {
+          tile_store_bf3<AKC, NT, TS>(Ai, qa[d % PD]);
+          tile_store_bf3<BKC, NT, TS>(Bi, qb[d % PD]);
+          __syncthreads();
+          if (kt + d + PD < kt_fast_end) fetch_set(kt + d + PD, qa[d % PD], qb[d % PD]);
+          multiply();
+          __syncthreads();
+        }
+      }
+    }
+  } else if (kt_begin < kt_fast_end) {
+    fetch_fast(kt_begin);
+    for (int64_t kt = kt_begin; kt < kt_fast_end; ++kt) {
+#if ASR_GB_ABL & 4
+      if (kt == kt_begin) {
+        tile_store_bf3<AKC, NT, TS>(Ai, ra);
+        tile_store_bf3<BKC, NT, TS>(Bi, rb);
+      } else {
+#pragma unroll
+        for (int i = 0; i < NP; ++i) asm volatile("" ::"v"(ra[i].x), "v"(ra[i].y), "v"(ra[i].z), "v"(ra[i].w), "v"(rb[i].x), "v"(rb[i].y), "v"(rb[i].z), "v"(rb[i].w));
+      }
+#else
+      tile_store_bf3<AKC, NT, TS>(Ai, ra);
+      tile_store_bf3<BKC, NT, TS>(Bi, rb);
+#endif
+      __syncthreads();
+      if (kt + 1 < kt_fast_end && !(ASR_GB_ABL & 2)) fetch_fast(kt + 1);
+#if ASR_GEMM_TOUCH
+      asm volatile("" ::"v"(touched));
+      if (do_touch && kt + ASR_GEMM_BF3_TOUCH < kt_end) touch_tile(kt + ASR_GEMM_BF3_TOUCH);
+#endif
+      multiply();
+      __syncthreads();
+    }
+  }
+  if (kt_fast_end < kt_end) {
+    fetch_guard(kt_fast_end);
+    for (int64_t kt = kt_fast_end; kt < kt_end; ++kt) {
+      tile_store_bf3<AKC, NT, TS>(Ai, ra);
+      tile_store_bf3<BKC, NT, TS>(Bi, rb);
+      __syncthreads();
+      if (kt + 1 < kt_end) fetch_guard(kt + 1);
+#if ASR_GEMM_TOUCH
+      asm volatile("" ::"v"(touched));
+      if (do_touch && kt + ASR_GEMM_BF3_TOUCH < kt_end) touch_tile(kt + ASR_GEMM_BF3_TOUCH);
+#endif
+      multiply();
+      __syncthreads();
+    }
+  }
+
+#if ASR_GB_ABL & 8
+  if (threadIdx.x + blockIdx.x + blockIdx.y != 0 || g.M != 1) {
+#pragma unroll
+    for (int i = 0; i < NB; ++i)
+#pragma unroll
+      for (int j = 0; j < NB; ++j)
+#pragma unroll
+        for (int e = 0; e < 16; ++e) asm volatile("" ::"v"(acc[i][j][e]));
+    return;
+  }
+#endif
+  if (m0 + BM <= g.M && n0 + BN <= g.N) {
+    const unsigned ldc = (unsigned)g.ldc;
+    const bool split = QUEUE || g.split_k > 1, accum = g.accumulate != 0, relu = g.relu != 0;
+#pragma unroll
+    for (int j = 0; j < NB; ++j) {
+      const int64_t n = n0 + wn * (TS / 2) + j * 32 + l31;
+      const float bv = g.bias ? g.bias[n] : 0.f;
+#pragma unroll
+      for (int i = 0; i < NB; ++i) {
+        float* base = C + (m0 + wm * (TS / 2) + i * 32 + 4 * kh) * g.ldc + n;
+        if (split) {
+#pragma unroll
+          for (int e = 0; e < 16; ++e) atomicAdd(base + (unsigned)((e & 3) + 8 * (e >> 2)) * ldc, acc[i][j][e]);
+        } else if (accum) {
+          float old[16];
+#pragma unroll
+          for (int e = 0; e < 16; ++e) old[e] = base[(unsigned)((e & 3) + 8 * (e >> 2)) * ldc];
+#pragma unroll
+          for (int e = 0; e < 16; ++e) {
+            float v = acc[i][j][e] + bv + old[e];
+            if (relu) v = fmaxf(v, 0.f);
+            base[(unsigned)((e & 3) + 8 * (e >> 2)) * ldc] = v;
+          }
+        } else {
+#pragma unroll
+          for (int e = 0; e < 16; ++e) {
+            float v = acc[i][j][e] + bv;
+            if (relu) v = fmaxf(v, 0.f);
+            base[(unsigned)((e & 3) + 8 * (e >> 2)) * ldc] = v;
+          }
+        }
+      }
+    }
+    return;
+  }
+#pragma unroll
+  for (int j = 0; j < NB; ++j) {
+    const int64_t n = n0 + wn * (TS / 2) + j * 32 + l31;
+    if (n >= g.N) continue;
+    const float bv = g.bias ? g.bias[n] : 0.f;
+#pragma unroll
+    for (int i = 0; i < NB; ++i) {
+#pragma unroll
+      for (int e = 0; e < 16; ++e) {
+        const int64_t m = m0 + wm * (TS / 2) + i * 32 + (e & 3) + 8 * (e >> 2) + 4 * kh;
+        if (m >= g.M) continue;
+        float v = acc[i][j][e];
+        float* dst = C + m * g.ldc + n;
+        if (QUEUE || g.split_k > 1) {
+          atomicAdd(dst, v);
+        } else {
+          v += bv;
+          if (g.accumulate) v += *dst;
+          if (g.relu) v = fmaxf(v, 0.f);
+          *dst = v;
+        }
+      }
+    }
+  }
+}
+
+__device__ __forceinline__ void colsum_body(int64_t M, int64_t N, const float* X, int64_t ldx, float* out, int bx, int by,
+                                            float (*part)[64]) {
+  const int cx = threadIdx.x & 63, ry = threadIdx.x >> 6;
+  const int64_t n = (int64_t)bx * 64 + cx;
+  const int64_t mbeg = (int64_t)by * 512;
+  const int64_t mend = mbeg + 512 < M ? mbeg + 512 : M;
+  float s = 0.f;
+  if (n < N)
+    for (int64_t m = mbeg + ry; m < mend; m += 4) s += X[m * ldx + n];
+  part[ry][cx] = s;
+  __syncthreads();
+  if (ry == 0 && n < N) atomicAdd(out + n, (part[0][cx] + part[1][cx]) + (part[2][cx] + part[3][cx]));
+}
+
+__device__ __forceinline__ void colsum4_body(int64_t M, int64_t N, const float* __restrict__ X, int64_t ldx, float* out, int bx,
+                                             int by, float4 (*part)[16]) {
+  const int cq = threadIdx.x & 15, ry = threadIdx.x >> 4;
+  const int64_t n = (int64_t)bx * 64 + 4 * cq;
+  const int64_t mbeg = (int64_t)by * 256;
+  const int64_t mend = mbeg + 256 < M ? mbeg + 256 : M;
+  float4 s = make_float4(0.f, 0.f, 0.f, 0.f);
+  if (n < N) {
+    const float* p = X + n;
+#pragma unroll 4
+    for (int64_t m = mbeg + ry; m < mend; m += 16) {
+      const float4 v = *reinterpret_cast<const float4*>(p + m * ldx);
+      s.x += v.x; s.y += v.y; s.z += v.z; s.w += v.w;
+    }
+  }
+  part[ry][cq] = s;
+  __syncthreads();
+  if (threadIdx.x < 64) {
+    const int q = threadIdx.x >> 2, e = threadIdx.x & 3;
+    float t = 0.f;
+#pragma unroll
+    for (int r = 0; r < 16; ++r) t += reinterpret_cast<const float*>(&part[r][q])[e];
+    const int64_t col = (int64_t)bx * 64 + threadIdx.x;
+    if (col < N) atomicAdd(out + col, t);
+  }
+}
+
+constexpr int GROUP_MAX_SLOTS = 16;
+constexpr int GROUP_COLSUM = 4;
+struct GroupJobs {
+  GemmArgs g[GROUP_MAX_SLOTS];
+  int first[GROUP_MAX_SLOTS + 1];
+  int kind[GROUP_MAX_SLOTS];
+  int n;
+};
+
+}
+
+int asr_gemm_group_launch(const void* group_jobs, int wgs, int nt, hipStream_t stream);
diff --git a/semi-supervised-asr_amd/csrc/gemm_group.hip b/semi-supervised-asr_amd/csrc/gemm_group.hip
--- /dev/null
+++ b/semi-supervised-asr_amd/csrc/gemm_group.hip
@@ -0,0 +1,46 @@
+#include "gemm_bf3.h"
+
+namespace {
+
+template <int NT>
+__global__ __launch_bounds__(256, ASR_GEMM_SMALL_OCC) void gemm_group_kernel(GroupJobs jobs) {
+  __shared__ __attribute__((aligned(16))) unsigned short smem[2 * NT * 64 * BS];
+  const int b = blockIdx.x;
+  int s = 0;
+  for (int i = 1; i < jobs.n; ++i)
+    if (b >= jobs.first[i]) s = i;
+  const GemmArgs& g = jobs.g[s];
+  const int local = b - jobs.first[s], kind = jobs.kind[s];
+  if (kind & GROUP_COLSUM) {
+    const int bx = local % g.tiles_m, r = local / g.tiles_m;
+    const int by = r % g.tiles_n, bz = r / g.tiles_n;
+    const float* X = g.A.p + bz * g.sA;
+    if (g.split_k) colsum4_body(g.A.R, g.A.Cn, X, g.A.ld, g.C, bx, by, reinterpret_cast<float4(*)[16]>(smem));
+    else colsum_body(g.A.R, g.A.Cn, X, g.A.ld, g.C, bx, by, reinterpret_cast<float(*)[64]>(smem));
+    return;
+  }
+  const int ntile = g.tiles_m * g.tiles_n;
+  const int z = local / ntile;
+  int tid = local - z * ntile;
+  {
+    const int q = ntile >> 3, rmd = ntile & 7, xcd = tid & 7, idx = tid >> 3;
+    tid = (xcd < rmd ? xcd * (q + 1) : rmd * (q + 1) + (xcd - rmd) * q) + idx;
+  }
+  switch (kind & 3) {
+    case 3: gemm_bf3_tile<true, true, NT, 64, false>(g, tid, z, smem); break;
+    case 1: gemm_bf3_tile<true, false, NT, 64, false>(g, tid, z, smem); break;
+    case 2: gemm_bf3_tile<false, true, NT, 64, false>(g, tid, z, smem); break;
+    default: gemm_bf3_tile<false, false, NT, 64, false>(g, tid, z, smem); break;
+  }
+}
+
+}
+
+int asr_gemm_group_launch(const void* group_jobs, int wgs, int nt, hipStream_t stream) {
+  const GroupJobs& jobs = *static_cast<const GroupJobs*>(group_jobs);
+  const dim3 grid((unsigned)wgs), block(256);
+  if (nt == 2) hipLaunchKernelGGL((gemm_group_kernel<2>), grid, block, 0, stream, jobs);
+  else hipLaunchKernelGGL((gemm_group_kernel<3>), grid, block, 0, stream, jobs);
+  ASR_CHECK_LAUNCH();
+  return 0;
+}
diff --git a/semi-supervised-asr_amd/hip_backend.py b/semi-supervised-asr_amd/hip_backend.py
--- a/semi-supervised-asr_amd/hip_backend.py
+++ b/semi-supervised-asr_amd/hip_backend.py
@@ -14,7 +14,7 @@
     "asr_dropout_mask_f32",
     "asr_dec_step_fwd", "asr_att_step_fwd", "asr_dec_seq_fwd", "asr_dec_seq_fwd_persist", "asr_dec_seq_fwd_persist_fault", "asr_dec_seq_fwd_persist_free", "asr_dec_step_bwd", "asr_dec_seq_bwd", "asr_dec_seq_bwd_persist", "asr_dec_seq_bwd_persist_free",
     "asr_lstm_pack_f32", "asr_lstm_unpack_f32", "asr_lstm_unpack2_f32", "asr_dec_prepare_f32", "asr_cell_pack_f32", "asr_cell_unpack_f32",
-    "asr_lstm_pack_multi_f32", "asr_lstm_unpack_multi_f32", "asr_dec_pack_f32", "asr_colsum_parts_f32", "asr_gemm_drop_f32", "asr_gemm_side_f32", "asr_embedding_grad_f32",
+    "asr_lstm_pack_multi_f32", "asr_lstm_unpack_multi_f32", "asr_dec_pack_f32", "asr_colsum_parts_f32", "asr_gemm_drop_f32", "asr_gemm_side_f32", "asr_gemm_group_f32", "asr_gemm_group_plan", "asr_embedding_grad_f32",
     "asr_label_logprob_fwd", "asr_label_logprob_bwd", "asr_dec_feedback_fwd", "asr_dec_feedback_bwd",
     "asr_adam_clip_f32", "asr_sumsq_f32", "asr_gather_sumsq_f32", "asr_graphs_create", "asr_graphs_destroy", "asr_graphs_stats",
     "asr_beam_select_f32", "asr_beam_reorder_f32", "asr_beam_backtrack",
@@ -28,6 +28,16 @@
 
 
 PACK_MAX_LAYERS = 4
+
+
+GEMM_GROUP_MAX = 8
+
+
+class GemmJob(ctypes.Structure):
+    _fields_ = [("transA", c_i), ("transB", c_i), ("M", c_i64), ("N", c_i64), ("K", c_i64), ("A", c_p), ("lda", c_i64),
+                ("B", c_p), ("ldb", c_i64), ("C", c_p), ("ldc", c_i64), ("bias", c_p), ("relu", c_i), ("accumulate", c_i),
+                ("batch", c_i), ("split_k", c_i), ("sA", c_i64), ("sB", c_i64), ("sC", c_i64), ("flags", c_i), ("colsum", c_i),
+                ("colsum_accumulate", c_i), ("reserved", c_i), ("colsum_out", c_p)]
 
 
 class LstmPackJob(ctypes.Structure):
@@ -177,6 +187,8 @@
     lib.asr_gemm_skinny_f32.argtypes = [c_i64, c_i64, c_i64, c_p, c_i64, c_p, c_i64, c_p, c_i64, c_p, c_i, c_p,
                                         c_i64, c_i64, c_p]
     lib.asr_colsum_f32.argtypes = [c_i64, c_i64, c_p, c_i64, c_p, c_i, c_p]
+    lib.asr_gemm_group_f32.argtypes = [ctypes.POINTER(GemmJob), c_i, c_i, c_p]
+    lib.asr_gemm_group_plan.argtypes = [ctypes.POINTER(GemmJob), c_i, c_i, ctypes.POINTER(c_i), ctypes.POINTER(c_i), c_i]
     lib.asr_lstm_seq_fwd.argtypes = [c_i, c_i, c_i, c_i, c_i, c_p, c_p, c_p, c_p, c_p, c_p, c_p, c_p, c_p]
     lib.asr_lstm_seq_fwd_persist.argtypes = [c_i, c_i, c_i, c_i, c_i, c_p, c_p, c_p, c_p, c_p, c_p, c_p, c_p, c_p, c_p, c_i, c_p]
     lib.asr_lstm_seq_bwd_persist.argtypes = [c_i, c_i, c_i, c_i, c_i, c_p, c_p, c_p, c_p, c_p, c_p, c_p, c_p, c_p, c_p, c_p, c_p, c_p,
@@ -382,6 +394,66 @@
     return True
 
 
+def _addr(t):
+    return None if t is None else t.data_ptr()
+
+
+def gemm_job(A, B, trans_a=False, trans_b=False, bias=None, relu=False, out=None, accumulate=False, split_k=None,
+             out_zeroed=False, colsum=None, colsum_out=None, colsum_accumulate=False):
+    A, lda = _rowmajor(_dev(A, "A"))
+    B, ldb = _rowmajor(_dev(B, "B"))
+    M, K = (A.shape[1], A.shape[0]) if trans_a else A.shape
+    K2, N = (B.shape[1], B.shape[0]) if trans_b else B.shape
+    assert K == K2, "inner dimensions differ: %d vs %d" % (K, K2)
+    if out is None:
+        out = torch.empty(M, N, device=A.device, dtype=torch.float32)
+    out, ldc = _rowmajor(_dev(out, "out"))
+    assert out.shape == (M, N)
+    cs = {None: 0, "a": 1, "b": 2}[colsum]
+    if cs and colsum_out is None:
+        colsum_out, colsum_accumulate = torch.empty(M if cs == 1 else N, device=A.device, dtype=torch.float32), False
+    job = GemmJob(int(trans_a), int(trans_b), M, N, K, A.data_ptr(), lda, B.data_ptr(), ldb, out.data_ptr(), ldc, _addr(bias),
+                  int(relu), int(accumulate), 1, 0 if split_k is None else int(split_k), 0, 0, 0, C_ZEROED if out_zeroed else 0,
+                  cs, int(colsum_accumulate), 0, _addr(colsum_out))
+    job.out, job.colsum_out_t, job.keep = out, colsum_out, (A, B, bias)
+    return job
+
+
+def gemm_job_batched(A, B, out, trans_a, trans_b, M, N, K, lda, ldb, ldc, batch, sA, sB, sC, accumulate=False, split_k=None,
+                     a_off=0, b_off=0, colsum=None, colsum_out=None, colsum_accumulate=False):
+    cs = {None: 0, "a": 1, "b": 2}[colsum]
+    job = GemmJob(int(trans_a), int(trans_b), M, N, K, _dev(A).data_ptr() + 4 * a_off, lda, _dev(B).data_ptr() + 4 * b_off, ldb,
+                  _dev(out).data_ptr(), ldc, None, 0, int(accumulate), batch, 0 if split_k is None else int(split_k), sA, sB, sC,
+                  0, cs, int(colsum_accumulate), 0, _addr(colsum_out))
+    job.out, job.colsum_out_t, job.keep = out, colsum_out, (A, B)
+    return job
+
+
+def _job_array(jobs):
+    arr = (GemmJob * len(jobs))()
+    for i, j in enumerate(jobs):
+        ctypes.memmove(ctypes.byref(arr[i]), ctypes.byref(j), ctypes.sizeof(GemmJob))
+    return arr
+
+
+def gemm_group(jobs, arith=None):
+    code = ARITH[0] if arith is None else _arith_code(arith)
+    for i in range(0, len(jobs), GEMM_GROUP_MAX):
+        part = jobs[i:i + GEMM_GROUP_MAX]
+        check(load().asr_gemm_group_f32(_job_array(part), len(part), code, stream()), "asr_gemm_group_f32")
+    return [j.out for j in jobs]
+
+
+def gemm_group_plan(jobs, arith=None):
+    code = ARITH[0] if arith is None else _arith_code(arith)
+    cap = 2 * GEMM_GROUP_MAX + 1
+    first, kinds = (c_i * cap)(), (c_i * cap)()
+    n = load().asr_gemm_group_plan(_job_array(jobs), len(jobs), code, first, kinds, cap)
+    if n < 0:
+        raise RuntimeError("asr_gemm_group_plan failed with code %d (ASR_E_*)" % n)
+    return list(first[:n + 1]), list(kinds[:n])
+
+
 def gemm_skinny(A, Bt, bias=None, out=None, accumulate=False):
     A, lda = _rowmajor(_dev(A, "A"))
     Bt, ldb = _rowmajor(_dev(Bt, "Bt"))
diff --git a/semi-supervised-asr_amd/ops.py b/semi-supervised-asr_amd/ops.py
--- a/semi-supervised-asr_amd/ops.py
+++ b/semi-supervised-asr_amd/ops.py
@@ -194,6 +194,13 @@
     return hb.gemm(A, B, trans_a=trans_a, trans_b=trans_b, out=out, accumulate=True)
 
 
+def _gemm_acc_job(A, B, shape, colsum=False):
+    out = _ARENA.take(shape, A.device)
+    cs = _ARENA.take((A.shape[1],), A.device) if colsum else None
+    return hb.gemm_job(A, B, trans_a=True, out=out, accumulate=out is not None, colsum="a" if colsum else None, colsum_out=cs,
+                       colsum_accumulate=cs is not None)
+
+
 def _colsum_acc(X):
     out = _ARENA.take((X.shape[1],), X.device)
     return hb.colsum(X) if out is None else hb.colsum(X, out=out, accumulate=True)
@@ -243,14 +250,19 @@
             dy2 = hb.relu_dropout_bwd(dy2, y, seed, p)
         elif ctx.relu:
             dy2 = dy2 * (y > 0).to(dy2.dtype)
-        dx = hb.gemm(dy2, weight).view(ctx.in_shape) if ctx.needs_input_grad[0] else None
+        jobs = [hb.gemm_job(dy2, weight)] if ctx.needs_input_grad[0] else []
+        db = None
         if _SIDE.may_defer(ctx, weight):
             dw = zeros_acc((dy2.shape[1], x2.shape[1]), dy2.device)
             queue = zeros_acc((1,), dy2.device)
             _SIDE.defer(dy2.device, _side_product(dy2, x2, dw.detach(), queue, ctx.side_mask), (dy2, x2, queue))
-        else:
-            dw = _gemm_acc(dy2, x2, trans_a=True, shape=(dy2.shape[1], x2.shape[1]))
-        db = _colsum_acc(dy2) if ctx.has_bias else None
+            if ctx.has_bias:
+                db = _colsum_acc(dy2)
+        else:
+            jobs.append(_gemm_acc_job(dy2, x2, (dy2.shape[1], x2.shape[1]), colsum=ctx.has_bias))
+            dw, db = jobs[-1].out, jobs[-1].colsum_out_t
+        hb.gemm_group(jobs)
+        dx = jobs[0].out.view(ctx.in_shape) if ctx.needs_input_grad[0] else None
         return dx, dw, db, None, None
 
 
@@ -637,9 +649,9 @@
             acc = buf.accumulators(zb)
         G = acc["G"]
         XO = X[1:].view(L * B, KX)[:, :D + O]
-        hb.gemm(dlog2, w_out, out=G[1:].view(L * B, KX)[:, :D + O])
-        dw_out = _gemm_acc(dlog2, XO, trans_a=True, shape=(V, D + O))
-        db_out = _colsum_acc(dlog2)
+        jw = _gemm_acc_job(dlog2, XO, (V, D + O), colsum=True)
+        hb.gemm_group([hb.gemm_job(dlog2, w_out, out=G[1:].view(L * B, KX)[:, :D + O]), jw])
+        dw_out, db_out = jw.out, jw.colsum_out_t
         if dws is not None:
             buf.dws.copy_(dws)
         demb_w = zeros_acc(tuple(emb_w.shape), dev)
@@ -658,15 +670,16 @@
                                   demb_w)
         dg2 = buf.dgates.view(L * B, 4 * D)
         Xin = X[:L] if Xd is None else Xd[:L]
-        dwcat = _gemm_acc(dg2, Xin.reshape(L * B, KX), trans_a=True, shape=(4 * D, KX))
-        dw_ih, dw_hh, dbias, dbias2 = hb.cell_unpack(dwcat, _colsum_acc(dg2), D, O, E)
-        dwdec = _gemm_acc(buf.dD.view(L * B, A), X[1:].view(L * B, KX)[:, :D], trans_a=True, shape=(A, D))
+        jcat = _gemm_acc_job(dg2, Xin.reshape(L * B, KX), (4 * D, KX), colsum=True)
+        jdec = _gemm_acc_job(buf.dD.view(L * B, A), X[1:].view(L * B, KX)[:, :D], (A, D))
+        dQ = torch.empty(B, Tp, O, device=dev, dtype=torch.float32)
+        dctx_base = G[1:]
+        jq = hb.gemm_job_batched(buf.ws, dctx_base[:, :, D:], dQ, True, False, Tp, O, L, B * Tp, B * KX, O, B, Tp, KX, Tp * O)
+        hb.gemm_group([jcat, jdec, jq])
+        dwdec = jdec.out
+        dw_ih, dw_hh, dbias, dbias2 = hb.cell_unpack(jcat.out, jcat.colsum_out_t, D, O, E)
         dgvec, dwatt, dconvw = hb.colsum_parts([acc["dgvec_part"], acc["dwatt_part"], acc["dconv_part"]])
         dgvec, dconvw = dgvec.view(1, A), dconvw.view(C, 1, 1, 2 * K + 1)
-        dQ = torch.empty(B, Tp, O, device=dev, dtype=torch.float32)
-        dctx_base = G[1:]
-        hb.gemm_batched(buf.ws, dctx_base[:, :, D:], dQ, True, False, Tp, O, L, B * Tp, B * KX, O, B, Tp, KX,
-                        Tp * O)
         dbo = _colsum_acc(dctx_base.view(L * B, KX)[:, D:D + O])
         demb_all = G[:L, :, D + O:]
         nsteps = 1 if torch.is_tensor(probs_saved) else L
```
